# ahuang73/HemoCell

Hardware: AMD Instinct MI355X
Metric: MLUPS + cell-vertex updates/s, 256^3 pipeflow 10% Hct (higher is better)
Workload: dtype f64

## Files before the change

hemocell_amd/capi.py:

```python
import ctypes as C
import os
import subprocess

_HERE = os.path.dirname(os.path.abspath(__file__))
LIB_PATH = os.path.join(_HERE, "lib", "libhemocell_amd.so")

c_double_p = C.POINTER(C.c_double)
c_long_p = C.POINTER(C.c_long)
c_int_p = C.POINTER(C.c_int)


class HcError(RuntimeError):
    pass


class Params(C.Structure):
    _fields_ = [(n, C.c_double) for n in
                ("dx", "dt", "nu_p", "rho_p", "kBT_p", "tau", "nu_lbm", "dm", "df", "f_limit", "kBT_lbm")]


class Material(C.Structure):
    _fields_ = [("kLink", C.c_double), ("kArea", C.c_double), ("kVolume", C.c_double), ("kBend", C.c_double),
                ("eta_m", C.c_double), ("radius", C.c_double), ("min_triangles", C.c_int),
                ("aspect_ratio", C.c_double), ("inner_edges", c_long_p), ("n_inner", C.c_int)]


class WbcMaterial(C.Structure):
    _fields_ = [("kInnerRigid", C.c_double), ("kCytoskeleton", C.c_double), ("coreRadius", C.c_double),
                ("radius", C.c_double)]


class CellTypeSpec(C.Structure):
    _fields_ = [("model", C.c_int), ("shape", C.c_int), ("material", Material), ("wbc", C.POINTER(WbcMaterial)),
                ("kInnerLink", C.c_double), ("stl_path", C.c_char_p)]


VP = C.c_void_p
SIGNATURES = {
    "hc_last_error": (C.c_char_p, []),
    "hc_init": (C.c_int, [C.c_int]),
    "hc_device_count": (C.c_int, [c_int_p]),
    "hc_set_stream": (C.c_int, [VP]),
    "hc_synchronize": (C.c_int, []),
    "hc_fork": (C.c_int, []),
    "hc_route": (C.c_int, [C.c_int]),
    "hc_join": (C.c_int, []),
    "hc_side_stream": (C.c_int, [C.POINTER(VP)]),
    "hc_set_overlap": (C.c_int, [C.c_int]),
    "hc_comm_init_env": (C.c_int, []),
    "hc_comm_init": (C.c_int, [C.c_int, C.c_int, C.c_int, C.c_char_p, C.c_int, C.c_int, C.c_int]),
    "hc_comm_finalize": (C.c_int, []),
    "hc_comm_info": (C.c_int, [c_int_p, c_int_p, c_int_p]),
    "hc_comm_barrier": (C.c_int, []),
    "hc_comm_allreduce": (C.c_int, [c_double_p, C.c_int, C.c_int]),
    "hc_comm_bcast": (C.c_int, [VP, C.c_size_t, C.c_int]),
    "hc_comm_allgather": (C.c_int, [VP, C.c_size_t, VP]),
    "hc_comm_exchange_host": (C.c_int, [C.c_int, VP, C.c_size_t, VP, C.c_size_t, VP, C.c_size_t, VP, C.c_size_t]),
    "hc_slab_stats": (C.c_int, [VP, c_double_p, C.c_int]),
    "hcl_slab_refresh_halos": (C.c_int, [VP, C.c_int]),
    "hcp_slab_sync_placement": (C.c_int, [VP, c_long_p]),
    "hcp_set_envelope": (C.c_int, [VP, C.c_double, c_double_p]),
    "hcp_envelope": (C.c_int, [VP, c_double_p, c_long_p]),
    "hcp_set_deletion_mode": (C.c_int, [VP, C.c_int]),
    "hcp_delete_incomplete_cells": (C.c_int, [VP, c_long_p]),
    "hcp_deletion_counts": (C.c_int, [VP, c_long_p, c_long_p, c_long_p, c_long_p]),
    "hcp_download_alive": (C.c_int, [VP, VP]),
    "hc_profile_enable": (C.c_int, [C.c_int]),
    "hc_profile_read": (C.c_int, [C.c_char_p, c_double_p, c_long_p]),
    "hc_profile_reset": (C.c_int, []),
    "hc_build_tag": (C.c_char_p, []),
    "hc_measure_copy_bandwidth": (C.c_int, [C.c_size_t, C.c_int, c_double_p]),
    "hcl_node_counts": (C.c_int, [VP, c_long_p]),
    "hc_debug_ibm_per_vertex": (C.c_int, [C.c_int]),
    "hc_set_reproducible_spread": (C.c_int, [C.c_int]),
    "hc_debug_force_plane_padding": (C.c_int, [C.c_int]),
    "hcl_create": (C.c_int, [C.POINTER(VP), C.c_int, C.c_int, C.c_int, c_int_p, C.c_double, C.c_int, C.c_int, C.c_int]),
    "hcl_destroy": (C.c_int, [VP]),
    "hcl_set_mask": (C.c_int, [VP, VP]),
    "hcl_init_equilibrium": (C.c_int, [VP, C.c_double, c_double_p]),
    "hcl_set_body_force_regions": (C.c_int, [VP, C.c_int, C.POINTER(C.c_int), c_double_p]),
    "hcl_set_body_force": (C.c_int, [VP, c_double_p]),
    "hcl_set_wall_velocity": (C.c_int, [VP, C.c_int, c_double_p]),
    "hcl_collide_stream": (C.c_int, [VP, C.c_int]),
    "hcl_set_lees_edwards": (C.c_int, [VP, C.c_double, C.c_double]),
    "hcl_set_lees_edwards_displacement": (C.c_int, [VP, C.c_double, C.c_double]),
    "hcl_lees_edwards_apply": (C.c_int, [VP]),
    "hcl_lees_edwards_state": (C.c_int, [VP, c_double_p]),
    "hcl_open_boundary_add": (C.c_int, [VP, C.c_int, C.c_int, c_int_p, C.c_int, c_int_p]),
    "hcl_open_boundary_add_box": (C.c_int, [VP, C.c_int, C.c_int, c_int_p, c_int_p, c_int_p]),
    "hcl_open_boundary_add_axis": (C.c_int, [VP, C.c_int, C.c_int, C.c_int, c_int_p, C.c_int, c_int_p]),
    "hcl_open_boundary_add_box_axis": (C.c_int, [VP, C.c_int, C.c_int, C.c_int, c_int_p, c_int_p, c_int_p]),
    "hcl_open_boundary_axes": (C.c_int, [VP, c_int_p, C.c_int, c_int_p]),
    "hcl_open_boundary_clear": (C.c_int, [VP]),
    "hcl_open_boundary_slots": (C.c_int, [VP, c_int_p, C.c_int, c_int_p]),
    "hcl_open_boundary_set_velocity": (C.c_int, [VP, C.c_int, C.c_int, VP, C.c_int]),
    "hcl_open_boundary_set_density": (C.c_int, [VP, C.c_int, C.c_int, VP, C.c_int]),
    "hcl_open_boundary_values": (C.c_int, [VP, C.c_int, C.c_int, c_double_p]),
    "hcl_plane_velocity": (C.c_int, [VP, C.c_int, c_int_p, C.c_int, VP, C.c_int]),
    "hcl_plane_velocity_axis": (C.c_int, [VP, C.c_int, C.c_int, c_int_p, C.c_int, VP, C.c_int]),
    "hcl_preinlet_create": (C.c_int, [C.POINTER(VP), VP, VP, C.c_int, C.c_int, c_int_p, C.c_int, C.c_int]),
    "hcl_preinlet_apply": (C.c_int, [VP]),
    "hcl_preinlet_iterate": (C.c_int, [VP, C.c_int]),
    "hcl_preinlet_destroy": (C.c_int, [VP]),
    "hcl_collide_stream_part": (C.c_int, [VP, C.c_int]),
    "hcl_step_end": (C.c_int, [VP]),
    "hcl_download_populations": (C.c_int, [VP, c_double_p]),
    "hcl_upload_populations": (C.c_int, [VP, c_double_p]),
    "hcl_download_rho_u": (C.c_int, [VP, c_double_p, c_double_p]),
    "hcl_download_pi_neq": (C.c_int, [VP, c_double_p]),
    "hcl_download_ibm_force": (C.c_int, [VP, c_double_p]),
    "hcl_zero_ibm_force": (C.c_int, [VP]),
    "hcl_halo_doubles": (C.c_size_t, [VP, C.c_int]),
    "hcl_halo_pack": (C.c_int, [VP, C.c_int, C.c_int, VP]),
    "hcl_halo_unpack": (C.c_int, [VP, C.c_int, C.c_int, VP]),
    "hcl_halo_pack_next": (C.c_int, [VP, C.c_int, C.c_int, VP]),
    "hcl_face_velocity_pack": (C.c_int, [VP, C.c_int, VP]),
    "hcl_face_velocity_pack_both": (C.c_int, [VP, VP, VP]),
    "hcl_halo_pack_both": (C.c_int, [VP, VP, VP, C.c_int]),
    "hcl_halo_unpack_both": (C.c_int, [VP, VP, VP]),
    "hcl_zero_force_halos": (C.c_int, [VP]),
    "hcl_download_face_velocity": (C.c_int, [VP, C.c_int, c_double_p]),
    "hcl_dims": (C.c_int, [VP, c_int_p]),
    "hcl_mlups_bytes_per_node": (C.c_double, [VP]),
    "hcl_interior_enable": (C.c_int, [VP, C.c_int, c_double_p]),
    "hcl_interior_info": (C.c_int, [VP, c_int_p, c_double_p]),
    "hcl_interior_upload_classes": (C.c_int, [VP, VP]),
    "hcl_interior_download_classes": (C.c_int, [VP, VP]),
    "hcl_scalar_create": (C.c_int, [VP, C.c_double, C.POINTER(VP)]),
    "hcl_scalar_destroy": (C.c_int, [VP]),
    "hcl_scalar_init_equilibrium": (C.c_int, [VP, c_int_p, C.c_double]),
    "hcl_scalar_set_source_box": (C.c_int, [VP, c_int_p, C.c_double]),
    "hcl_scalar_clear_sources": (C.c_int, [VP]),
    "hcl_scalar_step": (C.c_int, [VP]),
    "hcl_scalar_download": (C.c_int, [VP, c_double_p]),
    "hcl_scalar_download_populations": (C.c_int, [VP, c_double_p]),
    "hcl_scalar_upload_populations": (C.c_int, [VP, c_double_p]),
    "hcl_scalar_download_velocity": (C.c_int, [VP, c_double_p]),
    "hcl_scalar_stats": (C.c_int, [VP, c_double_p]),
    "hcp_sample_scalar": (C.c_int, [VP, VP, c_double_p]),
    "hcp_type_set_interior_viscosity": (C.c_int, [VP, C.c_int, C.c_double]),
    "hcp_set_interior_timescales": (C.c_int, [VP, C.c_int, C.c_int]),
    "hcp_interior_find": (C.c_int, [VP]),
    "hcp_interior_membrane": (C.c_int, [VP]),
    "hcp_interior_normals": (C.c_int, [VP, C.c_int, c_double_p]),
    "hc_debug_interior_block": (C.c_int, [C.c_int]),
    "hcl_binding_populate": (C.c_int, [VP, c_int_p]),
    "hcl_binding_clear": (C.c_int, [VP]),
    "hcl_binding_download": (C.c_int, [VP, VP]),
    "hcl_binding_upload": (C.c_int, [VP, VP]),
    "hcl_download_mask": (C.c_int, [VP, VP]),
    "hcl_download_tresca": (C.c_int, [VP, c_double_p]),
    "hcl_upload_solidified_mask": (C.c_int, [VP, VP]),
    "hcp_type_set_solidify": (C.c_int, [VP, C.c_int, C.c_double, C.c_double]),
    "hcp_set_solidify_timescale": (C.c_int, [VP, C.c_int]),
    "hcp_solidify_prepare": (C.c_int, [VP]),
    "hcp_solidify_flag": (C.c_int, [VP]),
    "hcp_solidify_flags_download": (C.c_int, [VP, VP]),
    "hcp_solidify_flags_upload": (C.c_int, [VP, VP]),
    "hcp_solidify_counts": (C.c_int, [VP, c_long_p]),
    "hc_debug_solidify_block": (C.c_int, [C.c_int]),
    "hc_params_base": (C.c_int, [C.POINTER(Params)] + [C.c_double] * 5),
    "hcp_celltype_create": (C.c_int, [C.POINTER(VP), C.c_int, C.c_int, C.POINTER(Params), C.POINTER(Material)]),
    "hcp_celltype_create_wbc": (C.c_int, [C.POINTER(VP), C.c_int, C.POINTER(Params), C.POINTER(Material),
                                          C.POINTER(WbcMaterial)]),
    "hcp_celltype_wbc_constants": (C.c_int, [VP, c_double_p]),
    "hcp_celltype_create_ex": (C.c_int, [C.POINTER(VP), C.POINTER(Params), C.POINTER(CellTypeSpec)]),
    "hcp_celltype_malaria_constants": (C.c_int, [VP, c_double_p]),
    "hcp_celltype_destroy": (C.c_int, [VP]),
    "hcp_celltype_sizes": (C.c_int, [VP, c_int_p]),
    "hcp_celltype_tables": (C.c_int, [VP, c_double_p, c_long_p, c_long_p, c_double_p, c_double_p, c_double_p,
                                      c_long_p, c_double_p, c_double_p]),
    "hcp_celltype_tables2": (C.c_int, [VP, c_long_p, c_long_p, c_long_p, c_double_p, c_int_p]),
    "hcp_create": (C.c_int, [C.POINTER(VP), VP, C.POINTER(Params)]),
    "hcp_destroy": (C.c_int, [VP]),
    "hcp_add_type": (C.c_int, [VP, VP, C.c_int, c_int_p]),
    "hcp_add_cell": (C.c_int, [VP, C.c_int, C.c_long, c_double_p, c_double_p, C.c_double, c_int_p]),
    "hcp_add_cell_unchecked": (C.c_int, [VP, C.c_int, C.c_long, c_double_p, c_double_p]),
    "hcp_counts": (C.c_int, [VP, c_long_p, c_long_p, c_long_p]),
    "hcp_type_range": (C.c_int, [VP, C.c_int, c_long_p, c_long_p]),
    "hcp_download": (C.c_int, [VP, C.c_int, c_double_p]),
    "hcp_upload": (C.c_int, [VP, C.c_int, c_double_p]),
    "hcp_download_cell_ids": (C.c_int, [VP, c_long_p]),
    "hcp_download_records": (C.c_int, [VP, C.c_void_p, C.c_long]),
    "hcp_upload_records": (C.c_int, [VP, C.c_void_p, C.c_long]),
    "hcp_add_vertex_force": (C.c_int, [VP, c_long_p, C.c_int, c_double_p]),
    "hcp_set_repulsion": (C.c_int, [VP, C.c_double, C.c_double, C.c_int]),
    "hcp_repulsion": (C.c_int, [VP]),
    "hcp_download_repulsion": (C.c_int, [VP, c_double_p]),
    "hcl_fluid_stats": (C.c_int, [VP, C.c_int, c_double_p, C.POINTER(C.c_long)]),
    "hcp_vertex_stats": (C.c_int, [VP, C.c_int, c_double_p, C.POINTER(C.c_long)]),
    "hcp_set_boundary_repulsion": (C.c_int, [VP, C.c_double, C.c_double, C.c_int]),
    "hcp_boundary_repulsion": (C.c_int, [VP]),
    "hcp_spread": (C.c_int, [VP, C.c_int]),
    "hcp_interpolate": (C.c_int, [VP]),
    "hcp_interpolate_cells": (C.c_int, [VP, C.c_int, c_int_p, C.c_int]),
    "hcp_advance": (C.c_int, [VP, C.c_int]),
    "hcp_mechanics": (C.c_int, [VP, C.c_long, C.c_int]),
    "hcp_mechanics_components": (C.c_int, [VP, C.c_int, c_double_p]),
    "hc_iterate": (C.c_int, [VP, VP, c_long_p, C.c_int, C.c_int, C.c_int, C.c_int]),
    "hcp_cell_extents": (C.c_int, [VP, C.c_int, c_double_p]),
    "hcp_cell_extents_begin": (C.c_int, [VP, C.c_int]),
    "hcp_cell_extents_end": (C.c_int, [VP, C.c_int, c_double_p]),
    "hcp_record_doubles": (C.c_size_t, [VP, C.c_int]),
    "hcp_pack_cells": (C.c_int, [VP, C.c_int, c_int_p, C.c_int, C.c_double, VP]),
    "hcp_unpack_cells": (C.c_int, [VP, C.c_int, c_int_p, c_long_p, c_int_p, C.c_int, VP]),
    "hcp_remove_cells": (C.c_int, [VP, C.c_int, c_int_p, C.c_int]),
    "hcp_owned_vertices": (C.c_int, [VP, c_long_p]),
    "hcp_preinlet_create": (C.c_int, [C.POINTER(VP), VP, VP, C.c_int, C.c_int, C.c_double, C.c_double, c_double_p, C.c_long]),
    "hcp_preinlet_create_slab": (C.c_int, [C.POINTER(VP), VP, VP, C.c_int, C.c_int, C.c_double, C.c_double, c_double_p, C.c_long]),
    "hcp_preinlet_set_sink": (C.c_int, [VP, C.c_int, C.c_double]),
    "hcp_preinlet_apply": (C.c_int, [VP, c_long_p, c_long_p]),
    "hcp_preinlet_counts": (C.c_int, [VP, c_long_p]),
    "hcp_preinlet_destroy": (C.c_int, [VP]),
    "hc_preinlet_iterate": (C.c_int, [VP, VP, c_long_p, C.c_int, C.c_int, C.c_int, C.c_int, C.c_int]),
    "hcp_cell_info": (C.c_int, [VP, C.c_int, c_double_p, c_double_p, c_double_p, c_double_p]),
}

_lib = None


def build():
    subprocess.check_call(["make", "-s", "-C", os.path.join(_HERE, "csrc")])


def lib():
    global _lib
    if _lib is None:
        if not os.path.exists(LIB_PATH):
            raise HcError("libhemocell_amd.so is not built (run `python -c 'import __graft_entry__ as g; g.build()'`); "
                          "the product path has no CPU fallback")
        L = C.CDLL(LIB_PATH)
        for name, (res, args) in SIGNATURES.items():
            fn = getattr(L, name)
            fn.restype = res
            fn.argtypes = args
        _lib = L
    return _lib


def check(rc):
    if rc != 0:
        raise HcError(lib().hc_last_error().decode("utf-8", "replace"))


def dptr(a):
    return a.ctypes.data_as(c_double_p)


def lptr(a):
    return a.ctypes.data_as(c_long_p)
```

hemocell_amd/csrc/cells.h:

```cpp
#pragma once
#include "common.h"
#include "host_cells.h"
#include "mesh.h"
#include <algorithm>
#include <cmath>
#include <cstring>

using namespace hc;

struct hc_celltype {
  CellTables host;
  DevBuf<int> d_tri, d_edge, d_ebt, d_ebo, d_iedge, d_vtri, d_vtri_k, d_vedge, d_vedge_s, d_bsrc, d_vouter, d_vinner, d_vinner_s, d_ring, d_nring;
  DevBuf<double> d_tri_area_eq, d_edge_len_eq, d_edge_angle_eq, d_patch_eq, d_iedge_len_eq;
};

struct hc_cells {
  hc_lattice *L = nullptr;
  hc_params P;
  int ntypes = 0;
  hc_celltype *types[8];
  int timescale[8];
  HostCells host[8];
  bool host_dirty = false;
  long nverts = 0, cap = 0;
  long ncells[8] = {0};
  long capc[8] = {0};
  long first[8] = {0};
  long cell0[8] = {0};
  DevBuf<double> pos[3], vel[3], frc[3];
  DevBuf<int> d_tag;
  long tag_cap = 0;
  DevBuf<unsigned char> d_vdead;
  MappedBuf<int> h_ntag;
  DevBuf<int> d_ntag;
  Event ntag_ev;
  bool ntag_pending = false, maybe_tagged = false;
  int del_mode = HC_DELETE_PARTICLE;
  DevBuf<int> d_vert_cell;
  DevBuf<double> rep[3];
  int rep_enabled = 0, rep_timescale = 1; double rep_const = 0, rep_cutoff = 0;
  int brep_enabled = 0, brep_timescale = 1; double brep_const = 0, brep_cutoff = 0; DevBuf<uint8_t> d_bflag;
  bool rep_on() const { return rep_enabled || brep_enabled; }
  DevBuf<unsigned int> d_keys[2]; DevBuf<int> d_vals[2]; DevBuf<char> d_sort_tmp; long sort_cap = 0;
  Staged<int> iscratch[19];
  MappedBuf<double> h_ext[8]; long ext_n[8] = {0}; Event ext_done[8]; bool ext_pending[8] = {false};
  Staged<char> vf;
  DevBuf<unsigned int> det_keys[2]; DevBuf<int> det_vals[2]; DevBuf<double> det_val[3]; DevBuf<char> det_tmp; long det_cap = 0;
  Staged<double> stat;
  Staged<double> info;
  std::vector<long> slab_gone[8];
  double e_share = 4.0;
  MappedBuf<int> h_env_viol;
  std::vector<long> slab_rejected;
  int visc_class[8] = {0};
  int visc_every = 1, visc_grid_every = 1;
  Staged<int> visc_rank; std::vector<long> visc_ids_seen;
  bool visc_on() const { for (int t = 0; t < ntypes; t++) if (visc_class[t]) return true; return false; }
  int solid_on[8] = {0}; double solid_dist[8] = {0}, solid_shear[8] = {0};
  int solid_every = 1;
  DevBuf<unsigned char> d_sflag;
  DevBuf<int> d_solid; MappedBuf<int> h_solid;
  long solid_nodes_seen = 0;
  bool solidify_on() const { for (int t = 0; t < ntypes; t++) if (solid_on[t]) return true; return false; }
  long n_deleted = 0;
  long n_particles_deleted = 0;
};

namespace hcc {

constexpr double E_SHARE_DEFAULT = 4.0, E_SHARE_MIN = 2.0;

struct LatView {
  const uint8_t *mask;
  int nx, ny, nz; long plane; long npad;
  int x0;
  int wrap_x, halo_x;
  int per_y, per_z;
  int nx_global;
  uint8_t *dirty; uint8_t epoch;
  const uint8_t *wallbrick; int nby, nbz;
  const double *halo_u[2];
  int ny_nz;
};

inline LatView make_view(const hc_lattice *L) {
  LatView v;
  v.mask = L->mask; v.nx = L->nx; v.ny = L->ny; v.nz = L->nz; v.plane = (long)L->xs; v.npad = (long)L->npad;
  v.x0 = L->x0; v.wrap_x = (L->n_slabs == 1 && L->periodic[0]) ? 1 : 0; v.halo_x = L->n_slabs > 1 ? 1 : 0;
  v.per_y = L->periodic[1]; v.per_z = L->periodic[2]; v.nx_global = L->nx_global;
  v.dirty = L->fdirty[L->fcur]; v.epoch = L->fepoch[L->fcur];
  v.wallbrick = L->wallbrick; v.nby = L->nby; v.nbz = L->nbz;
  v.halo_u[0] = L->halo_u_valid ? L->halo_u[0] : nullptr; v.halo_u[1] = L->halo_u_valid ? L->halo_u[1] : nullptr; v.ny_nz = (int)L->plane;
  return v;
}

__device__ __forceinline__ long pmod(long a, long n) { long r = a % n; return r < 0 ? r + n : r; }

__device__ __forceinline__ double phi2(double x) { x = fabs(x); x = 1.0 - x; return x > 0.0 ? x : 0.0; }

struct Stencil {
  long node[8];
  double w[8];
  int lx[8], ly[8], lz[8];
};

__device__ __forceinline__ long nearest_node(double x) { return (long)floor(x + 0.5); }

__device__ __forceinline__ void phi2_stencil(const LatView &v, double px, double py, double pz, Stencil &s) {
  const double p[3] = {px, py, pz};
  long c[3]; int d0[3];
#pragma unroll
  for (int a = 0; a < 3; a++) { c[a] = nearest_node(p[a]); d0[a] = (p[a] < (double)c[a]) ? -1 : 0; }
  double total = 0.0;
#pragma unroll
  for (int i = 0; i < 2; i++)
#pragma unroll
    for (int j = 0; j < 2; j++)
#pragma unroll
      for (int k = 0; k < 2; k++) {
        const int idx = i * 4 + j * 2 + k;
        const long gx = c[0] + d0[0] + i, gy = c[1] + d0[1] + j, gz = c[2] + d0[2] + k;
        long lx = gx - v.x0, ly = gy, lz = gz;
        bool ok = true;
        if (v.wrap_x) lx = pmod(lx, v.nx);
        else if (v.halo_x) ok = ok && (lx >= -HALO && lx < v.nx + HALO);
        else ok = ok && (lx >= 0 && lx < v.nx);
        if (gy < 0 || gy >= v.ny) { if (v.per_y) ly = pmod(gy, v.ny); else ok = false; }
        if (gz < 0 || gz >= v.nz) { if (v.per_z) lz = pmod(gz, v.nz); else ok = false; }
        double weight = 0.0; long node = -1;
        if (ok) {
          weight = phi2(p[0] - (double)gx) * phi2(p[1] - (double)gy) * phi2(p[2] - (double)gz);
          if (weight != 0.0) {
            node = (lx + HALO) * (long)v.plane + ly * v.nz + lz;
            if (v.mask[node] != 0) node = -1;
          }
        }
        if (node >= 0) total += weight;
        s.node[idx] = node; s.w[idx] = weight; s.lx[idx] = (int)lx; s.ly[idx] = (int)ly; s.lz[idx] = (int)lz;
      }
  const double coeff = 1.0 / total;
#pragma unroll
  for (int idx = 0; idx < 8; idx++) s.w[idx] *= coeff;
}

struct VertArrays { double *p[3], *v[3], *f[3], *r[3]; unsigned char *dead; int *tag; };
struct TypeArrays : VertArrays { const int *vert_cell; int *tag_all; };

template <typename T>
inline int upload_vec(DevBuf<T> &dst, const std::vector<T> &src) {
  const int rc = dst.reserve(src.size() ? src.size() : 1); if (rc != HC_OK) return rc;
  if (src.size()) HC_HIP(hipMemcpy(dst, src.data(), src.size() * sizeof(T), hipMemcpyHostToDevice));
  return HC_OK;
}
template <size_t N>
inline std::vector<int> flatten(const std::vector<std::array<long, N>> &v) {
  std::vector<int> o; o.reserve(v.size() * N);
  for (auto &a : v) for (long x : a) o.push_back((int)x);
  return o;
}

int sync_to_device(hc_cells *C);
int sync_to_host(hc_cells *C);
int settle(hc_cells *C);
TypeArrays vert_arrays(hc_cells *C, int t);
int ensure_sflag(hc_cells *C);
int solidify_refresh_mask(hc_cells *C);
int solidify_check(hc_cells *C);
const char *solidify_refusal(const hc_lattice *L);
int ensure_rep(hc_cells *C);
int stage_ints(hc_cells *C, int which, int **d, const int *h, int n);
int stage_ints(Staged<int> &s, int **d, const int *h, int n);
int upload_xyz(DevBuf<double> dst[3], long first, const double *src, long n);
int download_xyz(double *dst, const DevBuf<double> src[3], long first, long n);
int append_cells(hc_cells *C, int type, const long *cell_ids, const int *is_new, int n, long n_new);
int interpolate_cells_staged(hc_cells *C, int type, const int *slots, int n, int which);

}
using namespace hcc;
```

hemocell_amd/csrc/cells.hip:

```cpp
#include "cells.h"
#include <cstddef>
#include <memory>
#include <unordered_map>
#include <utility>
#include <vector>

namespace {

__global__ __launch_bounds__(256) void advance_kernel(LatView v, long n, double *px, double *py, double *pz, const double *vx,
                                                      const double *vy, const double *vz, const int *vert_cell, int *tag, unsigned char *dead,
                                                      int *counters, int whole_cell) {
  const long i = (long)blockIdx.x * 256 + threadIdx.x;
  if (i >= n) return;
  const int cell = vert_cell[i];
  if (dead[i] || tag[cell] == 1) return;
  const double x = px[i] + vx[i], y = py[i] + vy[i], z = pz[i] + vz[i];
  px[i] = x; py[i] = y; pz[i] = z;
  long gx = nearest_node(x) - v.x0, gy = nearest_node(y), gz = nearest_node(z);
  bool inside = true;
  if (v.wrap_x) gx = pmod(gx, v.nx); else inside = inside && (gx >= (v.halo_x ? -HALO : 0) && gx < (v.halo_x ? v.nx + HALO : v.nx));
  if (gy < 0 || gy >= v.ny) { if (v.per_y) gy = pmod(gy, v.ny); else inside = false; }
  if (gz < 0 || gz >= v.nz) { if (v.per_z) gz = pmod(gz, v.nz); else inside = false; }
  if (inside && v.mask[(gx + HALO) * (long)v.plane + gy * v.nz + gz] != 0) {
    if (whole_cell) {
      if (atomicExch(&tag[cell], 1) != 1) atomicAdd(&counters[0], 1);
    } else {
      dead[i] = 1;
      atomicAdd(&counters[2], 1);
      if (atomicCAS(&tag[cell], 0, 2) == 0) atomicAdd(&counters[1], 1);
    }
  }
}

__global__ void publish_counters_kernel(const int *counters, int *host_view) { for (int k = 0; k < 4; k++) host_view[k] = counters[k]; }
__global__ void sub_counters_kernel(int *counters, int a, int b, int c, int d) { atomicSub(&counters[0], a); atomicSub(&counters[1], b); atomicSub(&counters[2], c); if (d) atomicSub(&counters[3], d); }

__global__ void delete_incomplete_kernel(long ncells, int *tag, int *counters) {
  const long c = (long)blockIdx.x * 256 + threadIdx.x;
  if (c >= ncells) return;
  if (tag[c] == 2) { tag[c] = 1; atomicAdd(&counters[0], 1); }
}

__global__ void add_vertex_force_kernel(int n, const long *idx, const double *f, double *fx, double *fy, double *fz) {
  const int i = blockIdx.x * 256 + threadIdx.x;
  if (i >= n) return;
  const long v = idx[i];
  fx[v] += f[3 * i]; fy[v] += f[3 * i + 1]; fz[v] += f[3 * i + 2];
}

__global__ void fill_vert_cell_kernel(long n, int nv, int cell0, long first, int *vert_cell) {
  const long i = (long)blockIdx.x * 256 + threadIdx.x;
  if (i >= n) return;
  vert_cell[first + i] = cell0 + (int)(i / nv);
}

}

namespace hcc {

static void drop_regions(hc_cells *C) {
  for (int d = 0; d < 3; d++) { C->pos[d].reset(); C->vel[d].reset(); C->frc[d].reset(); C->rep[d].reset(); }
  C->d_tag.reset(); C->d_vdead.reset(); C->d_vert_cell.reset(); C->d_sflag.reset();
  C->cap = 0; C->tag_cap = 0;
  for (int t = 0; t < 8; t++) C->capc[t] = 0;
}

int ensure_rep(hc_cells *C) {
  if (C->rep[0] || C->cap <= 0) return HC_OK;
  for (int d = 0; d < 3; d++) {
    const int rc = C->rep[d].reserve((size_t)C->cap); if (rc != HC_OK) return rc;
    HC_HIP(hipMemset(C->rep[d], 0, C->cap * sizeof(double)));
  }
  return HC_OK;
}

int upload_xyz(DevBuf<double> dst[3], long first, const double *src, long n) {
  std::vector<double> tmp((size_t)n);
  for (int d = 0; d < 3; d++) {
    for (long i = 0; i < n; i++) tmp[(size_t)i] = src[(size_t)(3 * i + d)];
    HC_HIP(hipMemcpy(dst[d] + first, tmp.data(), (size_t)n * sizeof(double), hipMemcpyHostToDevice));
  }
  return HC_OK;
}
int download_xyz(double *dst, const DevBuf<double> src[3], long first, long n) {
  std::vector<double> tmp((size_t)n);
  for (int d = 0; d < 3; d++) {
    HC_HIP(hipMemcpy(tmp.data(), src[d] + first, (size_t)n * sizeof(double), hipMemcpyDeviceToHost));
    for (long i = 0; i < n; i++) dst[(size_t)(3 * i + d)] = tmp[(size_t)i];
  }
  return HC_OK;
}

int sync_to_device(hc_cells *C) {
  if (!C->host_dirty) return HC_OK;
  bool grow = false;
  long nverts = 0;
  int rc;
  for (int t = 0; t < C->ntypes; t++) {
    C->ncells[t] = (long)C->host[t].cells();
    nverts += C->ncells[t] * C->types[t]->host.nv;
    if (C->ncells[t] > C->capc[t]) grow = true;
  }
  if (grow || C->cap == 0) {
    drop_regions(C);
    long cap = 0, capcells = 0;
    for (int t = 0; t < C->ntypes; t++) {
      C->capc[t] = C->ncells[t] + C->ncells[t] / 4 + 64;
      C->first[t] = cap; C->cell0[t] = capcells;
      cap += C->capc[t] * C->types[t]->host.nv; capcells += C->capc[t];
    }
    C->cap = cap > 0 ? cap : 1;
    for (int d = 0; d < 3; d++)
      if ((rc = C->pos[d].reserve((size_t)C->cap)) != HC_OK || (rc = C->vel[d].reserve((size_t)C->cap)) != HC_OK || (rc = C->frc[d].reserve((size_t)C->cap)) != HC_OK) return rc;
    if ((rc = C->d_vert_cell.reserve((size_t)C->cap)) != HC_OK) return rc;
    if (C->rep_on() && (rc = ensure_rep(C)) != HC_OK) return rc;
    C->tag_cap = capcells + 1;
    if ((rc = C->d_tag.reserve((size_t)C->tag_cap)) != HC_OK || (rc = C->d_vdead.reserve((size_t)C->cap)) != HC_OK) return rc;
    for (int t = 0; t < C->ntypes; t++) {
      const long n = C->capc[t] * C->types[t]->host.nv;
      hipLaunchKernelGGL(fill_vert_cell_kernel, dim3((unsigned)((n + 255) / 256)), dim3(256), 0, hc::stream(), n, C->types[t]->host.nv, (int)C->cell0[t], C->first[t], C->d_vert_cell);
      HC_HIP(hipGetLastError());
    }
  }
  if (C->solidify_on() && (rc = ensure_sflag(C)) != HC_OK) return rc;
  C->nverts = nverts;
  for (int t = 0; t < C->ntypes; t++) {
    const long n = C->ncells[t] * C->types[t]->host.nv;
    if (n == 0) continue;
    const HostCells &H = C->host[t];
    if ((rc = upload_xyz(C->pos, C->first[t], H.pos.data(), n)) != HC_OK || (rc = upload_xyz(C->vel, C->first[t], H.vel.data(), n)) != HC_OK ||
        (rc = upload_xyz(C->frc, C->first[t], H.frc.data(), n)) != HC_OK) return rc;
  }
  HC_HIP(hipMemsetAsync(C->d_tag, 0, C->tag_cap * sizeof(int), hc::stream()));
  HC_HIP(hipMemsetAsync(C->d_vdead, 0, (size_t)C->cap, hc::stream()));
  if (C->d_sflag) HC_HIP(hipMemsetAsync(C->d_sflag, 0, (size_t)C->cap, hc::stream()));
  HC_HIP(hipStreamSynchronize(hc::stream()));
  for (int t = 0; t < C->ntypes; t++) {
    const long nc = C->ncells[t], n = nc * C->types[t]->host.nv;
    if (nc == 0) continue;
    const HostCells &H = C->host[t];
    HC_HIP(hipMemcpy(C->d_tag + C->cell0[t], H.tag.data(), (size_t)nc * sizeof(int), hipMemcpyHostToDevice));
    HC_HIP(hipMemcpy(C->d_vdead + C->first[t], H.dead.data(), (size_t)n, hipMemcpyHostToDevice));
    if (C->d_sflag) HC_HIP(hipMemcpy(C->d_sflag + C->first[t], H.sflag.data(), (size_t)n, hipMemcpyHostToDevice));
    if (H.has_rep && C->rep[0] && (rc = upload_xyz(C->rep, C->first[t], H.rep.data(), n)) != HC_OK) return rc;
  }
  C->host_dirty = false;
  return HC_OK;
}

int sync_to_host(hc_cells *C) {
  if (C->host_dirty) return HC_OK;
  HC_HIP(hipStreamSynchronize(hc::stream()));
  int rc;
  for (int t = 0; t < C->ntypes; t++) {
    const long n = C->ncells[t] * C->types[t]->host.nv;
    HostCells &H = C->host[t];
    H.size_payload(C->rep[0] != nullptr);
    if (n == 0) continue;
    if ((rc = download_xyz(H.pos.data(), C->pos, C->first[t], n)) != HC_OK || (rc = download_xyz(H.vel.data(), C->vel, C->first[t], n)) != HC_OK ||
        (rc = download_xyz(H.frc.data(), C->frc, C->first[t], n)) != HC_OK) return rc;
    if (C->d_tag) {
      HC_HIP(hipMemcpy(H.tag.data(), C->d_tag + C->cell0[t], (size_t)C->ncells[t] * sizeof(int), hipMemcpyDeviceToHost));
      HC_HIP(hipMemcpy(H.dead.data(), C->d_vdead + C->first[t], (size_t)n, hipMemcpyDeviceToHost));
    }
    if (C->d_sflag) HC_HIP(hipMemcpy(H.sflag.data(), C->d_sflag + C->first[t], (size_t)n, hipMemcpyDeviceToHost));
    if (H.has_rep && (rc = download_xyz(H.rep.data(), C->rep, C->first[t], n)) != HC_OK) return rc;
  }
  return HC_OK;
}

TypeArrays vert_arrays(hc_cells *C, int t) {
  TypeArrays a;
  for (int d = 0; d < 3; d++) {
    a.p[d] = C->pos[d] + C->first[t]; a.v[d] = C->vel[d] + C->first[t]; a.f[d] = C->frc[d] + C->first[t];
    a.r[d] = C->rep[d] ? C->rep[d] + C->first[t] : nullptr;
  }
  a.dead = C->d_vdead + C->first[t]; a.tag = C->d_tag + C->cell0[t];
  a.vert_cell = C->d_vert_cell + C->first[t]; a.tag_all = C->d_tag;
  return a;
}
int stage_ints(hc_cells *C, int which, int **d, const int *h, int n) { return stage_ints(C->iscratch[which], d, h, n); }
int stage_ints(Staged<int> &s, int **d, const int *h, int n) {
  if (!s.ev) { const int rc = s.ev.create(); if (rc != HC_OK) return rc; }
  else HC_HIP(hipEventSynchronize(s.ev));
  if ((size_t)n > s.cap()) {
    HC_HIP(hipDeviceSynchronize());
    const int rc = s.reserve((size_t)n * 2 + 256); if (rc != HC_OK) return rc;
  }
  if (n > 0) {
    std::memcpy(s.h, h, (size_t)n * sizeof(int));
    HC_HIP(hipMemcpyAsync(s.d, s.h, (size_t)n * sizeof(int), hipMemcpyHostToDevice, hc::stream()));
    HC_HIP(hipEventRecord(s.ev, hc::stream()));
  }
  *d = s.d;
  return HC_OK;
}

int celltype_create(const char *fn, hc_celltype **out, const hc_params *P, const hc_celltype_spec &S) {
  if (hc::stream() == nullptr) { hc::set_error(std::string(fn) + ": hc_init() has not been called"); return HC_ERR_STATE; }
  std::unique_ptr<hc_celltype> T(new hc_celltype());
  std::string err = build_cell_tables(T->host, *P, S);
  if (!err.empty()) { hc::set_error(std::string(fn) + ": " + err); return HC_ERR_ARG; }
  const CellTables &H = T->host;
  int rc = HC_OK;
  auto up_i = [&](DevBuf<int> &d, const std::vector<int> &v) { if (rc == HC_OK) rc = upload_vec(d, v); };
  auto up_d = [&](DevBuf<double> &d, const std::vector<double> &v) { if (rc == HC_OK) rc = upload_vec(d, v); };
  up_i(T->d_tri, flatten(H.triangles)); up_i(T->d_edge, flatten(H.edges));
  up_i(T->d_ebt, flatten(H.edge_bending_triangles)); up_i(T->d_ebo, flatten(H.edge_bending_outer));
  up_i(T->d_iedge, flatten(H.inner_edges));
  up_i(T->d_vtri, H.vtri); up_i(T->d_vtri_k, H.vtri_k); up_i(T->d_vedge, H.vedge); up_i(T->d_vedge_s, H.vedge_s);
  up_i(T->d_bsrc, H.bsrc); up_i(T->d_vouter, H.vouter); up_i(T->d_vinner, H.vinner); up_i(T->d_vinner_s, H.vinner_s);
  up_i(T->d_ring, flatten(H.vertex_vertexes)); up_i(T->d_nring, H.vertex_n_vertexes);
  up_d(T->d_tri_area_eq, H.triangle_area_eq); up_d(T->d_edge_len_eq, H.edge_length_eq);
  up_d(T->d_edge_angle_eq, H.edge_angle_eq); up_d(T->d_patch_eq, H.patch_dist_eq); up_d(T->d_iedge_len_eq, H.inner_edge_length_eq);
  if (rc != HC_OK) return rc;
  *out = T.release();
  return HC_OK;
}

}

extern "C" {

int hcp_celltype_create(hc_celltype **out, int model, int shape, const hc_params *P, const hc_material *M) {
  HC_REQUIRE(out && P && M, "hcp_celltype_create: null pointer");
  HC_REQUIRE(model != HC_MODEL_WBC_HO, "hcp_celltype_create: HC_MODEL_WBC_HO needs its inner-link constants: use hcp_celltype_create_wbc or hcp_celltype_create_ex");
  HC_REQUIRE(model != HC_MODEL_RBC_MALARIA, "hcp_celltype_create: HC_MODEL_RBC_MALARIA needs kInnerLink: use hcp_celltype_create_ex");
  HC_REQUIRE(shape != HC_SHAPE_MESH_FROM_STL, "hcp_celltype_create: HC_SHAPE_MESH_FROM_STL needs the STL file: use hcp_celltype_create_ex");
  hc_celltype_spec S{};
  S.model = model; S.shape = shape; S.material = *M;
  return hcc::celltype_create("hcp_celltype_create", out, P, S);
}

int hcp_celltype_create_wbc(hc_celltype **out, int shape, const hc_params *P, const hc_material *M, const hc_wbc_material *W) {
  HC_REQUIRE(out && P && M && W, "hcp_celltype_create_wbc: null pointer");
  HC_REQUIRE(shape != HC_SHAPE_MESH_FROM_STL, "hcp_celltype_create_wbc: HC_SHAPE_MESH_FROM_STL needs the STL file: use hcp_celltype_create_ex");
  hc_celltype_spec S{};
  S.model = HC_MODEL_WBC_HO; S.shape = shape; S.material = *M; S.wbc = W;
  return hcc::celltype_create("hcp_celltype_create_wbc", out, P, S);
}

int hcp_celltype_create_ex(hc_celltype **out, const hc_params *P, const hc_celltype_spec *S) {
  HC_REQUIRE(out && P && S, "hcp_celltype_create_ex: null pointer");
  return hcc::celltype_create("hcp_celltype_create_ex", out, P, *S);
}

int hcp_celltype_malaria_constants(const hc_celltype *T, double out[1]) {
  HC_REQUIRE(T && out, "hcp_celltype_malaria_constants: null pointer");
  out[0] = T->host.k_inner_link;
  return HC_OK;
}

int hcp_celltype_wbc_constants(const hc_celltype *T, double out[4]) {
  HC_REQUIRE(T && out, "hcp_celltype_wbc_constants: null pointer");
  const CellTables &H = T->host;
  out[0] = H.k_inner_rigid; out[1] = H.k_cytoskeleton; out[2] = H.core_radius; out[3] = H.wbc_radius;
  return HC_OK;
}

int hcp_celltype_destroy(hc_celltype *T) {
  delete T;
  return HC_OK;
}

int hcp_celltype_sizes(const hc_celltype *T, int out[4]) {
  HC_REQUIRE(T && out, "hcp_celltype_sizes: null pointer");
  out[0] = T->host.nv; out[1] = T->host.nt; out[2] = T->host.ne; out[3] = T->host.nie;
  return HC_OK;
}

int hcp_celltype_tables(const hc_celltype *T, double *vertices, long *triangles, long *edges, double *edge_length_eq,
                        double *edge_angle_eq, double *triangle_area_eq, long *vertex_vertexes, double *patch_dist_eq,
                        double scalars[9]) {
  HC_REQUIRE(T, "hcp_celltype_tables: null cell type");
  const CellTables &H = T->host;
  if (vertices) for (int i = 0; i < H.nv; i++) for (int d = 0; d < 3; d++) vertices[3 * i + d] = H.vertices[i][d];
  if (triangles) for (int i = 0; i < H.nt; i++) for (int d = 0; d < 3; d++) triangles[3 * i + d] = H.triangles[i][d];
  if (edges) for (int i = 0; i < H.ne; i++) for (int d = 0; d < 2; d++) edges[2 * i + d] = H.edges[i][d];
  if (edge_length_eq) std::copy(H.edge_length_eq.begin(), H.edge_length_eq.end(), edge_length_eq);
  if (edge_angle_eq) std::copy(H.edge_angle_eq.begin(), H.edge_angle_eq.end(), edge_angle_eq);
  if (triangle_area_eq) std::copy(H.triangle_area_eq.begin(), H.triangle_area_eq.end(), triangle_area_eq);
  if (vertex_vertexes) for (int i = 0; i < H.nv; i++) for (int d = 0; d < 6; d++) vertex_vertexes[6 * i + d] = H.vertex_vertexes[i][d];
  if (patch_dist_eq) std::copy(H.patch_dist_eq.begin(), H.patch_dist_eq.end(), patch_dist_eq);
  if (scalars) {
    const double s[9] = {H.volume_eq, H.area_mean_eq, H.edge_mean_eq, H.angle_mean_eq, H.k_volume, H.k_area, H.k_link, H.k_bend, H.eta_m};
    std::copy(s, s + 9, scalars);
  }
  return HC_OK;
}

int hcp_celltype_tables2(const hc_celltype *T, long *edge_bending_triangles, long *edge_bending_outer_points, long *inner_edges,
                         double *inner_edge_length_eq, int *vertex_n_vertexes) {
  HC_REQUIRE(T, "hcp_celltype_tables2: null cell type");
  const CellTables &H = T->host;
  if (edge_bending_triangles) for (int i = 0; i < H.ne; i++) for (int d = 0; d < 2; d++) edge_bending_triangles[2 * i + d] = H.edge_bending_triangles[i][d];
  if (edge_bending_outer_points) for (int i = 0; i < H.ne; i++) for (int d = 0; d < 2; d++) edge_bending_outer_points[2 * i + d] = H.edge_bending_outer[i][d];
  if (inner_edges) for (int i = 0; i < H.nie; i++) for (int d = 0; d < 2; d++) inner_edges[2 * i + d] = H.inner_edges[i][d];
  if (inner_edge_length_eq) std::copy(H.inner_edge_length_eq.begin(), H.inner_edge_length_eq.end(), inner_edge_length_eq);
  if (vertex_n_vertexes) std::copy(H.vertex_n_vertexes.begin(), H.vertex_n_vertexes.end(), vertex_n_vertexes);
  return HC_OK;
}

int hcp_create(hc_cells **out, hc_lattice *L, const hc_params *P) {
  HC_REQUIRE(out && L && P, "hcp_create: null pointer");
  std::unique_ptr<hc_cells> C(new hc_cells());
  C->L = L; C->P = *P;
  L->ibm = 1;
  int rc;
  if ((rc = C->h_ntag.reserve(4)) != HC_OK) return rc;
  for (int k = 0; k < 4; k++) C->h_ntag[k] = 0;
  if ((rc = C->d_ntag.reserve(4)) != HC_OK) return rc;
  HC_HIP(hipMemset(C->d_ntag, 0, 4 * sizeof(int)));
  if ((rc = C->ntag_ev.create()) != HC_OK || (rc = C->h_env_viol.reserve(1)) != HC_OK) return rc;
  *C->h_env_viol = 0;
  *out = C.release();
  return HC_OK;
}

int hcp_set_envelope(hc_cells *C, double particle_envelope_lu, double *share_in_use) {
  HC_REQUIRE(C, "hcp_set_envelope: null pointer");
  HC_REQUIRE(particle_envelope_lu > 0.0 && particle_envelope_lu < 1e6, "hcp_set_envelope: the envelope must be a positive number of lattice units");
  HC_REQUIRE(C->ntypes > 0, "hcp_set_envelope: add the cell types first (the envelope is measured against the largest cell)");
  for (int t = 0; t < C->ntypes; t++) HC_REQUIRE(C->host[t].cells() == 0, "hcp_set_envelope: set the envelope before the first cell is placed (placement already uses it)");
  double dmax = 0.0;
  for (int t = 0; t < C->ntypes; t++) dmax = std::max(dmax, C->types[t]->host.diameter);
  double share = std::max(particle_envelope_lu - dmax, E_SHARE_MIN);
  const hc_lattice *L = C->L;
  if (L->n_slabs > 1) {
    const double room = 0.5 * ((double)L->nx - 2.0 * dmax);
    if (room < E_SHARE_MIN) { hc::set_error("hcp_set_envelope: a slab of " + std::to_string(L->nx) + " planes cannot hold two cell diameters (" + std::to_string(2.0 * dmax) + " lu) and a particle envelope"); return HC_ERR_ARG; }
    share = std::min(share, std::floor(room * 16.0) / 16.0);
  }
  C->e_share = share;
  if (share_in_use) *share_in_use = share;
  return HC_OK;
}

int hcp_envelope(const hc_cells *C, double *share_in_use, long *late_copies) {
  HC_REQUIRE(C, "hcp_envelope: null pointer");
  if (share_in_use) *share_in_use = C->e_share;
  if (late_copies) *late_copies = C->h_env_viol ? (long)*C->h_env_viol : 0;
  return HC_OK;
}

int hcp_destroy(hc_cells *C) {
  if (!C) return HC_OK;
  (void)hipStreamSynchronize(hc::stream());
  delete C;
  return HC_OK;
}

int hcp_add_type(hc_cells *C, hc_celltype *T, int material_timescale, int *type_index) {
  HC_REQUIRE(C && T, "hcp_add_type: null pointer");
  HC_REQUIRE(C->ntypes < 8, "hcp_add_type: at most 8 cell types");
  HC_REQUIRE(material_timescale >= 1, "hcp_add_type: material timescale must be >= 1");
  C->types[C->ntypes] = T; C->timescale[C->ntypes] = material_timescale; C->host[C->ntypes].nv = T->host.nv;
  if (type_index) *type_index = C->ntypes;
  C->ntypes++;
  return HC_OK;
}

int hcp_add_cell(hc_cells *C, int type, long cell_id, const double centre_lu[3], const double angles[3], double min_dist_um, int *placed) {
  HC_REQUIRE(C && centre_lu && angles, "hcp_add_cell: null pointer");
  HC_REQUIRE(type >= 0 && type < C->ntypes, "hcp_add_cell: unknown cell type");
  int rc = settle(C); if (rc != HC_OK) return rc;
  rc = sync_to_host(C); if (rc != HC_OK) return rc;
  const CellTables &T = C->types[type]->host;
  const hc_lattice *L = C->L;
  const int nv = T.nv;
  auto bbox_centre = [&](const std::vector<Vec3> &v) {
    Vec3 lo = v[0], hi = v[0];
    for (auto &p : v) for (int d = 0; d < 3; d++) { lo[d] = std::min(lo[d], p[d]); hi[d] = std::max(hi[d], p[d]); }
    return Vec3{(hi[0] + lo[0]) * 0.5, (hi[1] + lo[1]) * 0.5, (hi[2] + lo[2]) * 0.5};
  };
  std::vector<Vec3> m = T.vertices;
  const Vec3 c0 = bbox_centre(m);
  for (auto &p : m) for (int d = 0; d < 3; d++) p[d] -= c0[d];
  const Vec3 mc = bbox_centre(m);
  double R[3][3];
  rotation_matrix_xyz(angles[0], angles[1], angles[2], R);
  for (auto &p : m) {
    const Vec3 x{p[0] + -1.0 * mc[0], p[1] + -1.0 * mc[1], p[2] + -1.0 * mc[2]};
    for (int a = 0; a < 3; a++) { double s = 0; for (int b = 0; b < 3; b++) s += R[a][b] * x[b]; p[a] = s + mc[a]; }
  }
  const std::vector<uint8_t> &mask = L->hmask;
  auto is_boundary = [&](long gx, long gy, long gz) -> bool {
    long lx = gx - L->x0, ly = gy, lz = gz;
    if (L->n_slabs == 1) { if (lx < 0 || lx >= L->nx) { if (L->periodic[0]) lx = ((lx % L->nx) + L->nx) % L->nx; else return false; } }
    else if (lx < -HALO || lx >= L->nx + HALO) return false;
    if (ly < 0 || ly >= L->ny) { if (L->periodic[1]) ly = ((ly % L->ny) + L->ny) % L->ny; else return false; }
    if (lz < 0 || lz >= L->nz) { if (L->periodic[2]) lz = ((lz % L->nz) + L->nz) % L->nz; else return false; }
    return mask[(size_t)(lx + HALO) * L->xs + (size_t)ly * L->nz + lz] != 0;
  };
  double cx = centre_lu[0];
  if (L->n_slabs > 1) {
    const double x0 = (double)L->x0, x1 = (double)(L->x0 + L->nx);
    const double shifts[3] = {0.0, -(double)L->nx_global, (double)L->nx_global};
    bool mine = false;
    for (int k = 0; k < (L->periodic[0] ? 3 : 1) && !mine; k++) {
      double lo = 1e300, hi = -1e300; bool own = false;
      for (int i = 0; i < nv; i++) {
        const double x = centre_lu[0] + shifts[k] + m[i][0];
        lo = std::min(lo, x); hi = std::max(hi, x);
        const double g = std::floor(x + 0.5);
        own = own || (g >= x0 && g < x1);
      }
      if (own || (hi >= x0 - C->e_share && lo < x1 + C->e_share)) { mine = true; cx = centre_lu[0] + shifts[k]; }
    }
    if (!mine) { if (placed) *placed = 0; return HC_OK; }
  }
  const int deny = (int)((min_dist_um * 1e-6) / C->P.dx);
  bool ok = true;
  for (int i = 0; i < nv && ok; i++) {
    const double v[3] = {cx + m[i][0], centre_lu[1] + m[i][1], centre_lu[2] + m[i][2]};
    const long n[3] = {(long)std::floor(v[0] + 0.5), (long)std::floor(v[1] + 0.5), (long)std::floor(v[2] + 0.5)};
    if (is_boundary(n[0], n[1], n[2])) { ok = false; break; }
    for (int a = -deny; a <= deny && ok; a++) for (int b = -deny; b <= deny && ok; b++) for (int c = -deny; c <= deny; c++)
      if (is_boundary(n[0] + a, n[1] + b, n[2] + c)) { ok = false; break; }
  }
  if (placed) *placed = ok ? 1 : 0;
  if (!ok) {
    if (L->n_slabs > 1) { C->slab_rejected.push_back(type); C->slab_rejected.push_back(cell_id); }
    return HC_OK;
  }
  double *p = C->host[type].append(cell_id, C->rep_on());
  for (int i = 0; i < nv; i++) { p[3 * i] = cx + m[i][0]; p[3 * i + 1] = centre_lu[1] + m[i][1]; p[3 * i + 2] = centre_lu[2] + m[i][2]; }
  C->host_dirty = true;
  return HC_OK;
}

int hcp_add_cell_unchecked(hc_cells *C, int type, long cell_id, const double centre_lu[3], const double angles[3]) {
  HC_REQUIRE(C && centre_lu && angles, "hcp_add_cell_unchecked: null pointer");
  HC_REQUIRE(type >= 0 && type < C->ntypes, "hcp_add_cell_unchecked: unknown cell type");
  int rc = settle(C); if (rc != HC_OK) return rc;
  rc = sync_to_host(C); if (rc != HC_OK) return rc;
  const CellTables &T = C->types[type]->host;
  (void)angles;
// ... 375 lines not shown
```

hemocell_amd/csrc/common.h:

```cpp
#pragma once
#include <hip/hip_runtime.h>
#include <stdint.h>
#include <string>
#include <utility>
#include <vector>
#include <type_traits>
#include "../../include/hemocell_amd.h"
#include "d3q19.h"

namespace hc {

void set_error(const std::string &msg);
int hip_fail(hipError_t e, const char *what, const char *file, int line);
hipStream_t stream();
hipStream_t comm_stream();
int fork();
void route(int side);
int join();
bool forked();

#define HC_HIP(call)                                                         \
  do {                                                                       \
    hipError_t e__ = (call);                                                 \
    if (e__ != hipSuccess) return hc::hip_fail(e__, #call, __FILE__, __LINE__); \
  } while (0)

#define HC_REQUIRE(cond, msg)                 \
  do {                                        \
    if (!(cond)) {                            \
      hc::set_error(std::string(msg));        \
      return HC_ERR_ARG;                      \
    }                                         \
  } while (0)

template <class T> struct DevBuf {
  T *p = nullptr; size_t cap = 0;
  DevBuf() = default;
  DevBuf(DevBuf &&o) noexcept { swap(o); }
  DevBuf &operator=(DevBuf &&o) noexcept { swap(o); return *this; }
  ~DevBuf() { reset(); }
  void swap(DevBuf &o) { std::swap(p, o.p); std::swap(cap, o.cap); }
  void reset() { if (p) (void)hipFree(p); p = nullptr; cap = 0; }
  operator T *() const { return p; }
  int reserve(size_t n) {
    if (n <= cap) return HC_OK;
    reset();
    const hipError_t e = hipMalloc((void **)&p, n * sizeof(T));
    if (e != hipSuccess) { p = nullptr; return hip_fail(e, "hipMalloc", __FILE__, __LINE__); }
    cap = n;
    return HC_OK;
  }
};
template <class T> struct PinBuf {
  T *p = nullptr, *dev = nullptr; size_t cap = 0; unsigned flags;
  explicit PinBuf(unsigned f = hipHostMallocDefault) : flags(f) {}
  PinBuf(PinBuf &&o) noexcept : flags(o.flags) { swap(o); }
  PinBuf &operator=(PinBuf &&o) noexcept { swap(o); return *this; }
  ~PinBuf() { reset(); }
  void swap(PinBuf &o) { std::swap(p, o.p); std::swap(dev, o.dev); std::swap(cap, o.cap); std::swap(flags, o.flags); }
  void reset() { if (p) (void)hipHostFree(p); p = dev = nullptr; cap = 0; }
  operator T *() const { return p; }
  int reserve(size_t n) {
    if (n <= cap) return HC_OK;
    reset();
    hipError_t e = hipHostMalloc((void **)&p, n * sizeof(T), flags);
    if (e != hipSuccess) p = nullptr;
    else if (flags & hipHostMallocMapped) e = hipHostGetDevicePointer((void **)&dev, p, 0);
    if (e != hipSuccess) { reset(); return hip_fail(e, "hipHostMalloc", __FILE__, __LINE__); }
    cap = n;
    return HC_OK;
  }
};
template <class T> struct MappedBuf : PinBuf<T> { MappedBuf() : PinBuf<T>(hipHostMallocMapped) {} };
struct Event {
  hipEvent_t e = nullptr;
  Event() = default;
  Event(Event &&o) noexcept { std::swap(e, o.e); }
  Event &operator=(Event &&o) noexcept { std::swap(e, o.e); return *this; }
  ~Event() { if (e) (void)hipEventDestroy(e); }
  operator hipEvent_t() const { return e; }
  int create() {
    if (e) return HC_OK;
    const hipError_t r = hipEventCreateWithFlags(&e, hipEventDisableTiming);
    if (r != hipSuccess) { e = nullptr; return hip_fail(r, "hipEventCreateWithFlags", __FILE__, __LINE__); }
    return HC_OK;
  }
};
template <class T> struct Staged {
  DevBuf<T> d; PinBuf<T> h; Event ev;
  size_t cap() const { return d.cap < h.cap ? d.cap : h.cap; }
  int reserve(size_t n) { const int rc = d.reserve(n); return rc != HC_OK ? rc : h.reserve(n); }
};

enum ProfKernel { PK_COLLIDE = 0, PK_SPREAD, PK_INTERP, PK_ADVANCE, PK_MECH, PK_COLLIDE_BESIDE, PK_LEES_EDWARDS, PK_COLLIDE_VISC, PK_INTERIOR_FIND, PK_INTERIOR_MEMBRANE, PK_SCALAR, PK_SOLIDIFY_PREPARE, PK_SOLIDIFY_FLAG, PK_COUNT };
void prof_count(int kernel);
struct ProfScope {
  int k; bool on;
  hipEvent_t a, b;
  explicit ProfScope(int kernel);
  ~ProfScope();
};

constexpr int HALO = 2;

constexpr int STAT_BLOCKS = 512;
struct StatAcc { double mn, mx, sum; long n; };
__device__ __forceinline__ void stat_add(StatAcc &a, double v) { a.mn = v < a.mn ? v : a.mn; a.mx = v > a.mx ? v : a.mx; a.sum += v; a.n++; }
__device__ __forceinline__ void stat_block_store(StatAcc a, double *partial ) {
  __shared__ double s_red[4][4];
#pragma unroll
  for (int off = 32; off > 0; off >>= 1) {
    const double mn = __shfl_xor(a.mn, off), mx = __shfl_xor(a.mx, off), sm = __shfl_xor(a.sum, off);
    const long n = __shfl_xor(a.n, off);
    a.mn = mn < a.mn ? mn : a.mn; a.mx = mx > a.mx ? mx : a.mx; a.sum += sm; a.n += n;
  }
  const int w = threadIdx.x >> 6;
  if ((threadIdx.x & 63) == 0) { s_red[w][0] = a.mn; s_red[w][1] = a.mx; s_red[w][2] = a.sum; s_red[w][3] = (double)a.n; }
  __syncthreads();
  if (threadIdx.x == 0) {
    double mn = s_red[0][0], mx = s_red[0][1], sm = s_red[0][2], n = s_red[0][3];
    for (int k = 1; k < (int)(blockDim.x >> 6); k++) { mn = s_red[k][0] < mn ? s_red[k][0] : mn; mx = s_red[k][1] > mx ? s_red[k][1] : mx; sm += s_red[k][2]; n += s_red[k][3]; }
    double *o = partial + 4 * blockIdx.x;
    o[0] = mn; o[1] = mx; o[2] = sm; o[3] = n;
  }
}
int stat_finish(const double *d_partial, double out[3], long *n, double *h_pinned = nullptr);

}

namespace hc {
struct BodyRegions { int n; int box[HC_MAX_FORCE_REGIONS][6]; double f[HC_MAX_FORCE_REGIONS][3]; };
#ifdef __HIPCC__
__device__ __forceinline__ void region_force(const BodyRegions &r, int xg, int y, int z, double &bx, double &by, double &bz) {
  for (int k = 0; k < r.n; k++) {
    const int *b = r.box[k];
    if (xg >= b[0] && xg <= b[1] && y >= b[2] && y <= b[3] && z >= b[4] && z <= b[5]) { bx = r.f[k][0]; by = r.f[k][1]; bz = r.f[k][2]; }
  }
}

constexpr int HC_OB_AXIS_SHIFT = 29;
constexpr int HC_OB_MAX_SLOTS = 1 << 27;
constexpr int ob_axis(int code) { return code >> HC_OB_AXIS_SHIFT; }
constexpr int ob_slot(int code) { return (code & ((1 << HC_OB_AXIS_SHIFT) - 1)) >> 2; }
constexpr bool ob_is_pressure(int code) { return (code & 2) != 0; }
__host__ __device__ constexpr int zh_perm(int axis, int i) {
  const int x = axis == 1 ? HC_CY[i] : axis == 2 ? HC_CZ[i] : HC_CX[i];
  const int y = axis == 1 ? HC_CX[i] : HC_CY[i];
  const int z = axis == 2 ? HC_CX[i] : HC_CZ[i];
  for (int j = 0; j < HC_Q; j++) if (HC_CX[j] == x && HC_CY[j] == y && HC_CZ[j] == z) return j;
  return -1;
}
template <int AXIS, int I> inline constexpr int ZH = zh_perm(AXIS, I);
static_assert(ZH<0, 7> == 7 && ZH<1, 1> == 2 && ZH<1, 5> == 14 && ZH<1, 15> == 17 && ZH<2, 1> == 3 && ZH<2, 7> == 16 && ZH<2, 13> == 17, "zh_perm");

template <int AXIS>
__device__ __forceinline__ void zou_he(double f[HC_Q], int code, const double *__restrict__ val) {
#define G(I) f[ZH<AXIS, I>]
  const int kind = code & 3;
  const long slot = code >> 2;
  const double s0 = G(0) + G(2) + G(3) + G(8) + G(9) + G(11) + G(12) + G(17) + G(18);
  const double sm = G(1) + G(4) + G(5) + G(6) + G(7);
  const double sp = G(10) + G(13) + G(14) + G(15) + G(16);
  const bool neg = (kind & 1) == 0;
  const double s_out = neg ? sm : sp;
  const double known = s0 + 2.0 * s_out + 1.0;
  double rho, ux, uy, uz;
  if (kind < 2) {
    ux = val[4 * slot + AXIS]; uy = val[4 * slot + (AXIS == 1 ? 0 : 1)]; uz = val[4 * slot + (AXIS == 2 ? 0 : 2)];
    rho = neg ? known / (1.0 - ux) : known / (1.0 + ux);
  } else {
    rho = val[4 * slot + 3];
    ux = neg ? 1.0 - known / rho : known / rho - 1.0;
    uy = 0.0; uz = 0.0;
  }
  const double ny = 0.5 * ((G(11) + G(17) + G(18)) - (G(2) + G(8) + G(9))) - rho * uy / 3.0;
  const double nz = 0.5 * ((G(12) + G(9) + G(17)) - (G(3) + G(8) + G(18))) - rho * uz / 3.0;
  if (neg) {
    G(10) = G(1) + rho * ux / 3.0;
    G(13) = G(4) + rho * (ux + uy) / 6.0 - ny;
    G(14) = G(5) + rho * (ux - uy) / 6.0 + ny;
    G(15) = G(6) + rho * (ux + uz) / 6.0 - nz;
    G(16) = G(7) + rho * (ux - uz) / 6.0 + nz;
  } else {
    G(1) = G(10) - rho * ux / 3.0;
    G(4) = G(13) - rho * (ux + uy) / 6.0 + ny;
    G(5) = G(14) - rho * (ux - uy) / 6.0 - ny;
    G(6) = G(15) - rho * (ux + uz) / 6.0 + nz;
    G(7) = G(16) - rho * (ux - uz) / 6.0 - nz;
  }
#undef G
}

__device__ __forceinline__ void zou_he_node(double f[HC_Q], int code, const double *__restrict__ val) {
  switch (code >> HC_OB_AXIS_SHIFT) {
    case 0: zou_he<0>(f, code, val); break;
    case 1: zou_he<1>(f, code & ((1 << HC_OB_AXIS_SHIFT) - 1), val); break;
    default: zou_he<2>(f, code & ((1 << HC_OB_AXIS_SHIFT) - 1), val); break;
  }
}
#endif
}

struct hc_lattice {
  int nx, ny, nz;
  int periodic[3];
  int x0, nx_global, n_slabs;
  double omega;
  size_t plane;
  size_t xs;
  size_t npad;
  size_t qstride;
  hc::DevBuf<double> f[2];
  int cur;
  hc::DevBuf<double> force[3];
  int fcur;
  int ibm;
  hc::DevBuf<uint8_t> fdirty[3];
  uint8_t fepoch[3];
  hc::DevBuf<uint8_t> wallbrick; int nbx, nby, nbz;
  hc::DevBuf<uint8_t> mask;
  std::vector<uint8_t> hmask;
  double body[3];
  hc::BodyRegions regions;
  double wall_u[4][3];
  hc::DevBuf<int> row_z0, row_cum, blk_row;
  int nblk, max_active;
  hc::DevBuf<double> scratch;
  hc::DevBuf<double> halo_u[2];
  bool halo_u_valid = false;
  bool le_on = false;
  double le_D = 0.0, le_d = 0.0, le_v_top = 0.0, le_v_bottom = 0.0;
  hc::DevBuf<double> le_buf;
  hc::DevBuf<int> ob_code;
  std::vector<int> ob_hcode;
  hc::DevBuf<double> ob_val;
  int ob_n = 0, ob_cap = 0;
  long ob_epoch = 0;
  hc::DevBuf<uint8_t> visc_class;
  int visc_n = 0; double visc_omega[HC_MAX_VISC_CLASSES];
  hc::DevBuf<unsigned long long> visc_vote;
  hc_scalar *scalar = nullptr;
  hc::DevBuf<uint8_t> binding;
  hc::DevBuf<int> ob_list;
  hc::DevBuf<double> ob_out;
};

namespace hc {
template <class Plain, class Launch>
inline void launch_open(const hc_lattice *L, const Plain &plain, Launch launch) {
  if (L->ob_n > 0) launch(std::true_type{}, open_of(L, plain));
  else launch(std::false_type{}, plain);
}
}

namespace hc {
int lees_edwards_step(hc_lattice *L);
void scalar_lattice_destroyed(hc_lattice *L);
void preinlet_pair_add(const void *owner, const hc_lattice *L);
void preinlet_pair_remove(const void *owner);
void preinlet_pair_forget(const hc_lattice *L);
bool in_preinlet_pair(const hc_lattice *L);
}

namespace hcs {
int iterate_slab(hc_lattice *L, hc_cells *C, long *iter, int n, int particle_timescale, int force_limit);
int collide_stream_slab(hc_lattice *L, int nsteps);
void lattice_destroyed(hc_lattice *L);
void halos_stale(hc_lattice *L);
void set_overlap(int on);
}
```

hemocell_amd/csrc/ibm.hip:

```cpp
#include "cells.h"
#include <type_traits>
#include <hipcub/hipcub.hpp>
#include <cstdlib>
#include <cstring>
#include <numeric>

namespace {

__global__ __launch_bounds__(256) void ibm_spread_kernel(LatView v, long n, const double *px, const double *py, const double *pz,
                                                         double *fx, double *fy, double *fz, const double *rx, const double *ry, const double *rz,
                                                         double *F, int limit_on, double f_limit, const int *vert_cell, const int *tag, const unsigned char *dead) {
  const long i = (long)blockIdx.x * 256 + threadIdx.x;
  if (i >= n) return;
  if (dead[i] || tag[vert_cell[i]] == 1) return;
  double f0 = fx[i], f1 = fy[i], f2 = fz[i];
  if (limit_on) {
    const double mag = sqrt((f0 * f0 + f1 * f1) + f2 * f2);
    if (mag > f_limit) {
      const double sc = f_limit / mag;
      f0 *= sc; f1 *= sc; f2 *= sc;
      fx[i] = f0; fy[i] = f1; fz[i] = f2;
    }
  }
  Stencil s;
  phi2_stencil(v, px[i], py[i], pz[i], s);
#pragma unroll
  for (int k = 0; k < 8; k++) {
    if (s.node[k] < 0) continue;
    v.dirty[s.node[k] >> 4] = v.epoch;
    double *Fn = F + 3 * s.node[k];
    unsafeAtomicAdd(Fn, ((rx ? rx[i] : 0.0) + f0) * s.w[k]);
    unsafeAtomicAdd(Fn + 1, ((ry ? ry[i] : 0.0) + f1) * s.w[k]);
    unsafeAtomicAdd(Fn + 2, ((rz ? rz[i] : 0.0) + f2) * s.w[k]);
  }
}

__global__ __launch_bounds__(256) void spread_emit_kernel(LatView v, int nv, long n, const int *order, long ebase, const double *px, const double *py,
                                                          const double *pz, double *fx, double *fy, double *fz, const double *rx, const double *ry,
                                                          const double *rz, int limit_on, double f_limit, const int *tag, const unsigned char *dead,
                                                          unsigned int *keys, int *vals, double *c0, double *c1, double *c2) {
  const long g = (long)blockIdx.x * 256 + threadIdx.x;
  if (g >= n) return;
  const int cell = order[g / nv];
  const long i = (long)cell * nv + (g % nv);
  const long e0 = (ebase + g) * 8;
  const bool live = tag[cell] != 1 && !dead[i];
  Stencil s;
  double f0 = 0.0, f1 = 0.0, f2 = 0.0;
  if (live) {
    f0 = fx[i]; f1 = fy[i]; f2 = fz[i];
    if (limit_on) {
      const double mag = sqrt((f0 * f0 + f1 * f1) + f2 * f2);
      if (mag > f_limit) { const double sc = f_limit / mag; f0 *= sc; f1 *= sc; f2 *= sc; fx[i] = f0; fy[i] = f1; fz[i] = f2; }
    }
    if (rx) { f0 = rx[i] + f0; f1 = ry[i] + f1; f2 = rz[i] + f2; }
    phi2_stencil(v, px[i], py[i], pz[i], s);
  }
#pragma unroll
  for (int k = 0; k < 8; k++) {
    const bool adm = live && s.node[k] >= 0;
    keys[e0 + k] = adm ? (unsigned int)s.node[k] : 0xffffffffu;
    vals[e0 + k] = (int)(e0 + k);
    c0[e0 + k] = adm ? f0 * s.w[k] : 0.0; c1[e0 + k] = adm ? f1 * s.w[k] : 0.0; c2[e0 + k] = adm ? f2 * s.w[k] : 0.0;
  }
}

__global__ __launch_bounds__(256) void spread_gather_kernel(LatView v, long n, const unsigned int *keys, const int *vals, const double *c0, const double *c1,
                                                            const double *c2, double *F) {
  const long s = (long)blockIdx.x * 256 + threadIdx.x;
  if (s >= n) return;
  const unsigned int key = keys[s];
  if (key == 0xffffffffu || (s > 0 && keys[s - 1] == key)) return;
  double a0 = 0.0, a1 = 0.0, a2 = 0.0;
  for (long q = s; q < n && keys[q] == key; q++) { const int e = vals[q]; a0 += c0[e]; a1 += c1[e]; a2 += c2[e]; }
  v.dirty[key >> 4] = v.epoch;
  double *Fn = F + 3 * (long)key;
  Fn[0] += a0; Fn[1] += a1; Fn[2] += a2;
}

struct PopView {
  const double *f; const double *F; double bx, by, bz; long qs;
  hc::BodyRegions reg;
};
struct OpenPopView : PopView { const int *ob_code; const double *ob_val; };
template <bool OPEN> using Pops = std::conditional_t<OPEN, OpenPopView, PopView>;

template <bool OPEN = false>
__device__ __forceinline__ void node_velocity(const LatView &v, const Pops<OPEN> &pv, int lx, int ly, int lz, long node, double u[3]) {
  if (v.halo_x && (lx <= -HALO || lx >= v.nx + HALO - 1)) { u[0] = u[1] = u[2] = 0.0; return; }
  if (v.halo_x && (lx == -1 || lx == v.nx)) {
    const double *hu = v.halo_u[lx < 0 ? 0 : 1];
    if (hu) { const long k = (long)ly * v.nz + lz; u[0] = hu[k]; u[1] = hu[v.ny_nz + k]; u[2] = hu[2L * v.ny_nz + k]; return; }
  }
  const hc::Nbr nb = hc::neighbours(v, v.plane, lx, ly, lz);
  double r = 0.0, jx = 0.0, jy = 0.0, jz = 0.0;
  [[maybe_unused]] double f[OPEN ? HC_Q : 1];
#define M(Q, CX, CY, CZ)                                                              \
  {                                                                                   \
    bool ok; const long off = hc::src_off<CX, CY, CZ>(nb, ok);                        \
    const double fq = ok ? pv.f[(long)Q * pv.qs + node + off] : 0.0;                 \
    if constexpr (OPEN) f[Q] = fq;                                                    \
    else {                                                                            \
      r += fq;                                                                        \
      if (CX == 1) jx += fq; else if (CX == -1) jx += -fq;                            \
      if (CY == 1) jy += fq; else if (CY == -1) jy += -fq;                            \
      if (CZ == 1) jz += fq; else if (CZ == -1) jz += -fq;                            \
    }                                                                                 \
  }
  FOR_Q(M)
#undef M
  if constexpr (OPEN) {
    if (v.mask[node] == 0) {
      const int code = pv.ob_code[node];
      if (code >= 0) hc::zou_he_node(f, code, pv.ob_val);
    }
    hc::moments(f, r, jx, jy, jz);
  }
  const double invRho = 1.0 / (1.0 + r);
  double bx = pv.bx, by = pv.by, bz = pv.bz;
  if (pv.reg.n) {
    int xg = v.x0 + lx;
    if (xg < 0) xg += v.nx_global; else if (xg >= v.nx_global) xg -= v.nx_global;
    region_force(pv.reg, xg, ly, lz, bx, by, bz);
  }
  u[0] = jx * invRho + (bx + pv.F[3 * node]) / 2.0;
  u[1] = jy * invRho + (by + pv.F[3 * node + 1]) / 2.0;
  u[2] = jz * invRho + (bz + pv.F[3 * node + 2]) / 2.0;
}

template <bool OPEN = false>
__global__ __launch_bounds__(256) void face_velocity_kernel(LatView v, Pops<OPEN> pv, int lx0, double *out0, int lx1, double *out1) {
  const int k = blockIdx.x * 256 + threadIdx.x;
  if (k >= v.ny_nz) return;
  const int lx = blockIdx.y ? lx1 : lx0;
  double *out = blockIdx.y ? out1 : out0;
  const int ly = k / v.nz, lz = k - ly * v.nz;
  const long node = (long)(lx + HALO) * v.plane + (long)ly * v.nz + lz;
  double u[3] = {0.0, 0.0, 0.0};
  if (v.mask[node] == 0) node_velocity<OPEN>(v, pv, lx, ly, lz, node, u);
  out[k] = u[0]; out[v.ny_nz + k] = u[1]; out[2L * v.ny_nz + k] = u[2];
}

template <bool OPEN = false>
__global__ __launch_bounds__(256) void ibm_interpolate_kernel(LatView v, Pops<OPEN> pv, long n, const double *px, const double *py,
                                                              const double *pz, double *vx, double *vy, double *vz, const int *vert_cell, const int *tag,
                                                              const unsigned char *dead) {
  const long i = (long)blockIdx.x * 256 + threadIdx.x;
  if (i >= n) return;
  if (dead[i] || tag[vert_cell[i]] == 1) return;
  Stencil s;
  phi2_stencil(v, px[i], py[i], pz[i], s);
  double a0 = 0.0, a1 = 0.0, a2 = 0.0;
#pragma unroll
  for (int k = 0; k < 8; k++) {
    if (s.node[k] < 0) continue;
    double u[3];
    node_velocity<OPEN>(v, pv, s.lx[k], s.ly[k], s.lz[k], s.node[k], u);
    a0 += (u[0] * s.w[k]); a1 += (u[1] * s.w[k]); a2 += (u[2] * s.w[k]);
  }
  vx[i] = a0; vy[i] = a1; vz[i] = a2;
}


constexpr int TILE_CAP = 5832;
constexpr int NODE_CAP = 1536;

struct Tile { int o[3]; int e[3]; int vol; int ow[3]; float r1, r2; };

__device__ __forceinline__ void tile_decode(const Tile &t, int i, int &tx, int &ty, int &tz) {
  const int q = (int)(((float)i + 0.5f) * t.r2);
  tz = i - q * t.e[2];
  tx = (int)(((float)q + 0.5f) * t.r1);
  ty = q - tx * t.e[1];
}

__device__ __forceinline__ int stencil_base(const LatView &v, double px, double py, double pz, int b[3]) {
  const double p[3] = {px, py, pz};
#pragma unroll
  for (int a = 0; a < 3; a++) { const long c = nearest_node(p[a]); b[a] = (int)c + ((p[a] < (double)c) ? -1 : 0); }
  return 0;
}

__device__ __forceinline__ long tile_node(const LatView &v, const Tile &t, int i, int &lx, int &ly, int &lz) {
  int tx, ty, tz;
  tile_decode(t, i, tx, ty, tz);
  lx = t.ow[0] + tx; ly = t.ow[1] + ty; lz = t.ow[2] + tz;
  if (v.wrap_x && lx >= v.nx) lx -= v.nx;
  if (v.per_y && ly >= v.ny) ly -= v.ny;
  if (v.per_z && lz >= v.nz) lz -= v.nz;
  return (long)(lx + HALO) * v.plane + ly * v.nz + lz;
}

__device__ __forceinline__ int xcd_contiguous(int b, int n) {
  const int per = n >> 3;
  const int main_n = per << 3;
  if (b >= main_n) return b;
  return (b & 7) * per + (b >> 3);
}

struct VStencil { double w[8]; int base; unsigned adm; };

constexpr int NVPT = 3;
constexpr int MAXW = 4;

#ifdef HC_IBM_PHASE_TIMES
__device__ unsigned long long g_phase[32];
#define PH_PARAM , long long &ph_last
#define PH_ARG , ph_last
#define PH_INIT long long ph_last = clock64();
#define STAMP(k) do { if (threadIdx.x == 0) { const long long ph_now = clock64(); atomicAdd(&g_phase[k], (unsigned long long)(ph_now - ph_last)); ph_last = ph_now; } } while (0)
#else
#define PH_PARAM
#define PH_ARG
#define PH_INIT
#define STAMP(k) do {} while (0)
#endif

__device__ __forceinline__ void block_bbox(int lo[3], int hi[3], int *s_red, Tile &t) {
  const int tid = threadIdx.x;
#pragma unroll
  for (int a = 0; a < 3; a++)
#pragma unroll
    for (int off = 32; off > 0; off >>= 1) { lo[a] = min(lo[a], __shfl_xor(lo[a], off)); hi[a] = max(hi[a], __shfl_xor(hi[a], off)); }
  if ((tid & 63) == 0) {
#pragma unroll
    for (int a = 0; a < 3; a++) { s_red[(tid >> 6) * 6 + a] = lo[a]; s_red[(tid >> 6) * 6 + 3 + a] = hi[a]; }
  }
  __syncthreads();
  const int nw = (blockDim.x + 63) >> 6;
#pragma unroll
  for (int a = 0; a < 3; a++) {
    int l = s_red[a], h = s_red[3 + a];
    for (int w = 1; w < nw; w++) { l = min(l, s_red[w * 6 + a]); h = max(h, s_red[w * 6 + 3 + a]); }
    t.o[a] = l; t.e[a] = h >= l ? h - l + 1 : 0;
  }
  const long vol = (long)t.e[0] * t.e[1] * t.e[2];
  t.vol = vol > 0x7fffffff ? 0x7fffffff : (int)vol;
}

__device__ __forceinline__ bool tile_finish(const LatView &v, Tile &t) {
  if (t.vol > TILE_CAP) return false;
  if ((v.wrap_x && t.e[0] > v.nx) || (v.per_y && t.e[1] > v.ny) || (v.per_z && t.e[2] > v.nz)) return false;
  t.ow[0] = v.wrap_x ? (int)pmod((long)t.o[0] - v.x0, v.nx) : t.o[0] - v.x0;
  t.ow[1] = v.per_y ? (int)pmod(t.o[1], v.ny) : t.o[1];
  t.ow[2] = v.per_z ? (int)pmod(t.o[2], v.nz) : t.o[2];
  t.r1 = 1.0f / (float)t.e[1]; t.r2 = 1.0f / (float)t.e[2];
  return true;
}

__device__ __forceinline__ unsigned char tile_mask(const LatView &v, const Tile &t, int i) {
  int tx, ty, tz;
  tile_decode(t, i, tx, ty, tz);
  int lx = t.ow[0] + tx, ly = t.ow[1] + ty, lz = t.ow[2] + tz;
  if (v.wrap_x) { if (lx >= v.nx) lx -= v.nx; }
  else if (v.halo_x) { if (lx < -HALO || lx >= v.nx + HALO) return 3; }
  else if (lx < 0 || lx >= v.nx) return 3;
  if (v.per_y) { if (ly >= v.ny) ly -= v.ny; } else if (ly < 0 || ly >= v.ny) return 3;
  if (v.per_z) { if (lz >= v.nz) lz -= v.nz; } else if (lz < 0 || lz >= v.nz) return 3;
  return v.mask[(long)(lx + HALO) * v.plane + ly * v.nz + lz];
}

__device__ __forceinline__ void tile_stencil(const Tile &t, const unsigned char *mt, double px, double py, double pz, const int b[3], VStencil &o) {
  const int sy = t.e[2], sx = t.e[1] * t.e[2];
  o.base = ((b[0] - t.o[0]) * t.e[1] + (b[1] - t.o[1])) * t.e[2] + (b[2] - t.o[2]);
  o.adm = 0;
  double total = 0.0;
#pragma unroll
  for (int i = 0; i < 2; i++)
#pragma unroll
    for (int j = 0; j < 2; j++)
#pragma unroll
      for (int k = 0; k < 2; k++) {
        const int idx = i * 4 + j * 2 + k;
        const double weight = phi2(px - (double)(b[0] + i)) * phi2(py - (double)(b[1] + j)) * phi2(pz - (double)(b[2] + k));
        const bool adm = (weight != 0.0) && (!mt || mt[o.base + i * sx + j * sy + k] == 0);
        if (adm) { total += weight; o.adm |= 1u << idx; }
        o.w[idx] = adm ? weight : 0.0;
      }
  const double coeff = 1.0 / total;
#pragma unroll
  for (int idx = 0; idx < 8; idx++) o.w[idx] *= coeff;
}

__device__ __forceinline__ bool tile_is_clear(const LatView &v, const Tile &t, int *s_near) {
  const int n[3] = {v.nx, v.ny, v.nz};
  bool inside = v.wallbrick != nullptr;
  int b0[3], nb[3];
#pragma unroll
  for (int a = 0; a < 3; a++) {
    const int lo = a == 0 ? t.ow[0] + HALO : t.ow[a], hi = lo + t.e[a] - 1, lim = a == 0 ? v.nx + 2 * HALO : n[a];
    inside = inside && lo >= 0 && hi < lim && (a != 0 || !v.wrap_x || (t.ow[0] >= 0 && t.ow[0] + t.e[0] <= v.nx));
    b0[a] = lo >> 3; nb[a] = (hi >> 3) - b0[a] + 1;
  }
  if (!inside) return false;
  if (nb[0] * nb[1] * nb[2] > 64) return false;
  if (threadIdx.x < 64) {
    const int l = threadIdx.x;
    bool near = false;
    if (l < nb[0] * nb[1] * nb[2]) {
      const int bz = l % nb[2], by = (l / nb[2]) % nb[1], bx = l / (nb[2] * nb[1]);
      near = v.wallbrick[((long)(b0[0] + bx) * v.nby + (b0[1] + by)) * v.nbz + (b0[2] + bz)] != 0;
    }
    const unsigned long long any = __ballot(near);
    if (l == 0) *s_near = any != 0ull;
  }
  __syncthreads();
  return *s_near == 0;
}

__device__ __forceinline__ bool cell_prologue(const LatView &v, int nv, long base, const double *px, const double *py, const double *pz,
                                              const unsigned char *dead, int *s_red, int *s_near, unsigned char *mt, Tile &t, VStencil vs[NVPT] PH_PARAM) {
  const int tid = threadIdx.x, nth = blockDim.x;
  double p[NVPT][3]; int b[NVPT][3]; bool live[NVPT];
  int lo[3] = {0x7fffffff, 0x7fffffff, 0x7fffffff}, hi[3] = {-0x7fffffff, -0x7fffffff, -0x7fffffff};
#pragma unroll
  for (int j = 0; j < NVPT; j++) {
    const int i = tid + j * nth;
    live[j] = i < nv && !(dead && dead[base + i]);
    if (live[j]) {
      p[j][0] = px[base + i]; p[j][1] = py[base + i]; p[j][2] = pz[base + i];
      stencil_base(v, p[j][0], p[j][1], p[j][2], b[j]);
#pragma unroll
      for (int a = 0; a < 3; a++) { lo[a] = min(lo[a], b[j][a]); hi[a] = max(hi[a], b[j][a] + 1); }
    }
  }
  block_bbox(lo, hi, s_red, t);
  STAMP(1);
  if (!tile_finish(v, t) || nv > NVPT * nth) return false;
  const bool clear = tile_is_clear(v, t, s_near);
  STAMP(2);
  if (!clear) {
#pragma unroll 4
    for (int i = tid; i < t.vol; i += nth) mt[i] = tile_mask(v, t, i);
    __syncthreads();
  }
  STAMP(3);
#pragma unroll
  for (int j = 0; j < NVPT; j++) {
    vs[j].adm = 0; vs[j].base = 0;
    if (live[j]) tile_stencil(t, clear ? nullptr : mt, p[j][0], p[j][1], p[j][2], b[j], vs[j]);
  }
  STAMP(4);
  return true;
}

constexpr unsigned short SLOT_FREE = 0xFFFF, SLOT_MARK = 0xFFFE;
__device__ __forceinline__ int compact_nodes(const Tile &t, const VStencil vs[NVPT], unsigned short *slot, unsigned short *list, int *s_count) {
  const int tid = threadIdx.x, nth = blockDim.x;
  const int sy = t.e[2], sx = t.e[1] * t.e[2];
  for (int i = tid; i < t.vol; i += nth) slot[i] = SLOT_FREE;
  if (tid == 0) *s_count = 0;
  __syncthreads();
#pragma unroll
  for (int j = 0; j < NVPT; j++)
#pragma unroll
    for (int k = 0; k < 8; k++) if (vs[j].adm & (1u << k)) slot[vs[j].base + (k >> 2) * sx + ((k >> 1) & 1) * sy + (k & 1)] = SLOT_MARK;
  __syncthreads();
  for (int i0 = 0; i0 < t.vol; i0 += nth) {
    const int i = i0 + tid;
    const bool marked = i < t.vol && slot[i] == SLOT_MARK;
    const unsigned long long b = __ballot(marked);
    int first = 0;
    if ((tid & 63) == 0 && b) first = atomicAdd(s_count, (int)__popcll(b));
    first = __shfl(first, 0);
    if (marked) {
      const int n = first + (int)__popcll(b & ((1ull << (tid & 63)) - 1ull));
      if (n < NODE_CAP) { slot[i] = (unsigned short)n; list[n] = (unsigned short)i; }
    }
  }
  __syncthreads();
  return *s_count;
}

__device__ void spread_direct(const LatView &v, int nv, long base, const double *px, const double *py, const double *pz, const double *fx,
                              const double *fy, const double *fz, const double *rx, const double *ry, const double *rz, double *F,
                              const unsigned char *dead) {
  for (int i = threadIdx.x; i < nv; i += blockDim.x) {
    if (dead && dead[base + i]) continue;
    Stencil s;
    phi2_stencil(v, px[base + i], py[base + i], pz[base + i], s);
    const double f0 = (rx ? rx[base + i] : 0.0) + fx[base + i], f1 = (ry ? ry[base + i] : 0.0) + fy[base + i], f2 = (rz ? rz[base + i] : 0.0) + fz[base + i];
#pragma unroll
    for (int k = 0; k < 8; k++) {
      if (s.node[k] < 0) continue;
      v.dirty[s.node[k] >> 4] = v.epoch;
      double *Fn = F + 3 * s.node[k];
      unsafeAtomicAdd(Fn, f0 * s.w[k]);
      unsafeAtomicAdd(Fn + 1, f1 * s.w[k]);
      unsafeAtomicAdd(Fn + 2, f2 * s.w[k]);
    }
  }
}

__global__ __launch_bounds__(256) void ibm_spread_cell_kernel(LatView v, int nv, const double *px, const double *py, const double *pz,
                                                              double *fx, double *fy, double *fz, const double *rx, const double *ry, const double *rz,
                                                              double *F, int limit_on, double f_limit, int xcd_ranges, const int *tag, const unsigned char *vdead) {
  __shared__ unsigned short slot[TILE_CAP];
  __shared__ __attribute__((aligned(16))) unsigned char raw[TILE_CAP > 2 * NODE_CAP ? TILE_CAP : 2 * NODE_CAP];
  unsigned char *mt = raw; unsigned short *list = reinterpret_cast<unsigned short *>(raw);
  __shared__ double acc[3 * NODE_CAP];
  __shared__ int s_red[6 * MAXW], s_count, s_near;
  const int tid = threadIdx.x, nth = blockDim.x;
  PH_INIT
  const int cell = xcd_ranges ? xcd_contiguous((int)blockIdx.x, (int)gridDim.x) : (int)blockIdx.x;
  const int state = tag[cell];
  if (state == 1) return;
  STAMP(0);
  const unsigned char *dead = state == 2 ? vdead : nullptr;
  const long base = (long)cell * nv;
  const bool in_regs = nv <= NVPT * nth;
  double f[NVPT][3];
  if (in_regs) {
#pragma unroll
    for (int j = 0; j < NVPT; j++) {
      const int i = tid + j * nth;
      f[j][0] = f[j][1] = f[j][2] = 0.0;
      if (i < nv) { f[j][0] = fx[base + i]; f[j][1] = fy[base + i]; f[j][2] = fz[base + i]; }
    }
  }
  Tile t; VStencil vs[NVPT];
  bool tiled = cell_prologue(v, nv, base, px, py, pz, dead, s_red, &s_near, mt, t, vs PH_ARG);
  if (limit_on) {
    if (in_regs) {
#pragma unroll
      for (int j = 0; j < NVPT; j++) {
        const int i = tid + j * nth;
        if (i < nv && !(dead && dead[base + i])) {
          const double mag = sqrt((f[j][0] * f[j][0] + f[j][1] * f[j][1]) + f[j][2] * f[j][2]);
          if (mag > f_limit) { const double sc = f_limit / mag; f[j][0] *= sc; f[j][1] *= sc; f[j][2] *= sc; fx[base + i] = f[j][0]; fy[base + i] = f[j][1]; fz[base + i] = f[j][2]; }
        }
      }
    } else {
      for (int i = tid; i < nv; i += nth) {
        if (dead && dead[base + i]) continue;
        const double f0 = fx[base + i], f1 = fy[base + i], f2 = fz[base + i];
        const double mag = sqrt((f0 * f0 + f1 * f1) + f2 * f2);
        if (mag > f_limit) { const double sc = f_limit / mag; fx[base + i] = f0 * sc; fy[base + i] = f1 * sc; fz[base + i] = f2 * sc; }
      }
    }
  }
  const int n = tiled ? compact_nodes(t, vs, slot, list, &s_count) : 0;
  STAMP(5);
  if (!tiled || n > NODE_CAP) { spread_direct(v, nv, base, px, py, pz, fx, fy, fz, rx, ry, rz, F, dead); return; }
  const int sy = t.e[2], sx = t.e[1] * t.e[2];
  for (int k = tid; k < 3 * n; k += nth) acc[k] = 0.0;
  __syncthreads();
#pragma unroll
  for (int j = 0; j < NVPT; j++) {
    const int i = tid + j * nth;
    if (i >= nv || !vs[j].adm) continue;
    double fv[3];
    fv[0] = (rx ? rx[base + i] : 0.0) + f[j][0]; fv[1] = (ry ? ry[base + i] : 0.0) + f[j][1]; fv[2] = (rz ? rz[base + i] : 0.0) + f[j][2];
#pragma unroll
    for (int k = 0; k < 8; k++) {
      if (!(vs[j].adm & (1u << k))) continue;
      double *a = &acc[3 * slot[vs[j].base + (k >> 2) * sx + ((k >> 1) & 1) * sy + (k & 1)]];
      atomicAdd(a, fv[0] * vs[j].w[k]); atomicAdd(a + 1, fv[1] * vs[j].w[k]); atomicAdd(a + 2, fv[2] * vs[j].w[k]);
    }
  }
  __syncthreads();
  STAMP(6);
  for (int k = tid; k < 3 * n; k += nth) {
    const double val = acc[k];
    if (val != 0.0) {
      const int q = k / 3;
      int lx, ly, lz; const long node = tile_node(v, t, list[q], lx, ly, lz); v.dirty[node >> 4] = v.epoch;
      unsafeAtomicAdd(&F[3 * node + (k - 3 * q)], val);
    }
  }
  STAMP(7);
}

template <bool OPEN = false>
__global__ __launch_bounds__(256) void ibm_interpolate_cell_kernel(LatView v, Pops<OPEN> pv, int nv, const double *px, const double *py,
                                                                   const double *pz, double *vx, double *vy, double *vz, const int *slots, int xcd_ranges,
                                                                   const int *tag, const unsigned char *vdead) {
  __shared__ unsigned short slot[TILE_CAP];
  __shared__ __attribute__((aligned(16))) unsigned char raw[TILE_CAP > 2 * NODE_CAP ? TILE_CAP : 2 * NODE_CAP];
  unsigned char *mt = raw; unsigned short *list = reinterpret_cast<unsigned short *>(raw);
  __shared__ double ux[NODE_CAP], uy[NODE_CAP], uz[NODE_CAP];
  __shared__ int s_red[6 * MAXW], s_count, s_near;
  const int tid = threadIdx.x, nth = blockDim.x;
  const int cell = slots ? slots[blockIdx.x] : (xcd_ranges ? xcd_contiguous((int)blockIdx.x, (int)gridDim.x) : (int)blockIdx.x);
  const int state = tag[cell];
  if (state == 1) return;
  const unsigned char *dead = state == 2 ? vdead : nullptr;
  const long base = (long)cell * nv;
  Tile t; VStencil vs[NVPT];
  PH_INIT
  bool tiled = cell_prologue(v, nv, base, px, py, pz, dead, s_red, &s_near, mt, t, vs PH_ARG);
  const int sy = t.e[2], sx = t.e[1] * t.e[2];
  if (tiled) {
    if (compact_nodes(t, vs, slot, list, &s_count) > NODE_CAP) tiled = false;
    STAMP(12);
  }
  if (tiled) {
    const int n = s_count;
    for (int k = tid; k < n; k += nth) {
      int lx, ly, lz;
      const long node = tile_node(v, t, list[k], lx, ly, lz);
      double u[3];
      node_velocity<OPEN>(v, pv, lx, ly, lz, node, u);
      ux[k] = u[0]; uy[k] = u[1]; uz[k] = u[2];
    }
    __syncthreads();
    STAMP(13);
#pragma unroll
    for (int j = 0; j < NVPT; j++) {
      const int i = tid + j * nth;
      if (i >= nv || (dead && dead[base + i])) continue;
      double a0 = 0.0, a1 = 0.0, a2 = 0.0;
#pragma unroll
      for (int k = 0; k < 8; k++) {
        if (!(vs[j].adm & (1u << k))) continue;
        const int q = slot[vs[j].base + (k >> 2) * sx + ((k >> 1) & 1) * sy + (k & 1)];
        a0 += (ux[q] * vs[j].w[k]); a1 += (uy[q] * vs[j].w[k]); a2 += (uz[q] * vs[j].w[k]);
      }
      vx[base + i] = a0; vy[base + i] = a1; vz[base + i] = a2;
    }
    STAMP(14);
    return;
  }
  for (int i = tid; i < nv; i += nth) {
    if (dead && dead[base + i]) continue;
    Stencil s;
    phi2_stencil(v, px[base + i], py[base + i], pz[base + i], s);
    double a0 = 0.0, a1 = 0.0, a2 = 0.0;
#pragma unroll
    for (int k = 0; k < 8; k++) {
      if (s.node[k] < 0) continue;
      double u[3];
      node_velocity<OPEN>(v, pv, s.lx[k], s.ly[k], s.lz[k], s.node[k], u);
      a0 += (u[0] * s.w[k]); a1 += (u[1] * s.w[k]); a2 += (u[2] * s.w[k]);
    }
    vx[base + i] = a0; vy[base + i] = a1; vz[base + i] = a2;
  }
}

PopView make_pops(const hc_lattice *L) {
  return PopView{L->f[L->cur], L->force[(L->fcur + 2) % 3], L->body[0], L->body[1], L->body[2], (long)L->qstride, L->regions};
}
OpenPopView open_of(const hc_lattice *L, const PopView &pv) {
  OpenPopView o;
  static_cast<PopView &>(o) = pv;
  o.ob_code = L->ob_code; o.ob_val = L->ob_val;
  return o;
}

}

#define HC_LAUNCH_POPS(K, grid, block, v, pv, ...)                                                                      \
  hc::launch_open(L, pv, [&](auto open, const auto &pops) {                                                             \
    hipLaunchKernelGGL(K<decltype(open)::value>, grid, block, 0, hc::stream(), v, pops, __VA_ARGS__);                   \
  })

static int g_ibm_per_vertex = 0;
extern "C" int hc_debug_ibm_per_vertex(int on) { g_ibm_per_vertex = on; return HC_OK; }
static int g_reproducible = -1;
static bool reproducible() {
  if (g_reproducible < 0) { const char *e = std::getenv("HEMOCELL_REPRODUCIBLE_SPREAD"); g_reproducible = (e && *e && *e != '0') ? 1 : 0; }
  return g_reproducible == 1;
}
extern "C" int hc_set_reproducible_spread(int on) { g_reproducible = on ? 1 : 0; return HC_OK; }

static int spread_reproducible(hc_cells *C, int force_limit) {
  const LatView v = make_view(C->L);
  HC_REQUIRE(v.npad * 3 < 0xffffffffL && C->nverts * 8 < 0x7fffffffL, "reproducible spread: lattice or vertex count beyond its 32-bit keys");
  const long n_e = C->nverts * 8;
  int rc;
  if (n_e > C->det_cap) {
    HC_HIP(hipDeviceSynchronize());
    const long cap = n_e + n_e / 4 + 4096;
    C->det_cap = 0;
    for (int k = 0; k < 2; k++) if ((rc = C->det_keys[k].reserve((size_t)cap)) != HC_OK || (rc = C->det_vals[k].reserve((size_t)cap)) != HC_OK) return rc;
    for (int k = 0; k < 3; k++) if ((rc = C->det_val[k].reserve((size_t)cap)) != HC_OK) return rc;
    size_t tmp_bytes = 0;
    HC_HIP(hipcub::DeviceRadixSort::SortPairs(nullptr, tmp_bytes, C->det_keys[0].p, C->det_keys[1].p, C->det_vals[0].p, C->det_vals[1].p, (int)cap, 0, 32, hc::stream()));
    if ((rc = C->det_tmp.reserve(tmp_bytes)) != HC_OK) return rc;
    C->det_cap = cap;
  }
  std::vector<int> order((size_t)0);
  std::vector<long> obase((size_t)C->ntypes, 0);
  for (int t = 0; t < C->ntypes; t++) {
    const size_t nc = (size_t)C->ncells[t], o = order.size();
    obase[(size_t)t] = (long)o;
    order.resize(o + nc);
    std::iota(order.begin() + (long)o, order.end(), 0);
    const std::vector<long> &ids = C->host[t].ids;
    std::stable_sort(order.begin() + (long)o, order.end(), [&](int a, int b) { return ids[(size_t)a] < ids[(size_t)b]; });
  }
  int *d_order = nullptr;
  rc = stage_ints(C, 2, &d_order, order.data(), (int)order.size()); if (rc != HC_OK) return rc;
  long ebase = 0;
  for (int t = 0; t < C->ntypes; t++) {
    const int nv = C->types[t]->host.nv;
    const long n = C->ncells[t] * nv;
    if (n == 0) continue;
    const TypeArrays a = vert_arrays(C, t);
    hipLaunchKernelGGL(spread_emit_kernel, dim3((unsigned)((n + 255) / 256)), dim3(256), 0, hc::stream(), v, nv, n, (const int *)(d_order + obase[(size_t)t]), ebase,
                       a.p[0], a.p[1], a.p[2], a.f[0], a.f[1], a.f[2], a.r[0], a.r[1], a.r[2], force_limit, C->P.f_limit, a.tag, a.dead, C->det_keys[0], C->det_vals[0],
                       C->det_val[0], C->det_val[1], C->det_val[2]);
    HC_HIP(hipGetLastError());
    ebase += n;
  }
  int bits = 1;
  while (bits < 32 && (1L << bits) <= v.npad) bits++;
  size_t tmp = C->det_tmp.cap;
  HC_HIP(hipcub::DeviceRadixSort::SortPairs(C->det_tmp.p, tmp, C->det_keys[0].p, C->det_keys[1].p, C->det_vals[0].p, C->det_vals[1].p, (int)n_e, 0, bits, hc::stream()));
  hipLaunchKernelGGL(spread_gather_kernel, dim3((unsigned)((n_e + 255) / 256)), dim3(256), 0, hc::stream(), v, n_e, (const unsigned int *)C->det_keys[1],
                     (const int *)C->det_vals[1], (const double *)C->det_val[0], (const double *)C->det_val[1], (const double *)C->det_val[2], C->L->force[C->L->fcur]);
  HC_HIP(hipGetLastError());
  return HC_OK;
}
#ifdef HC_IBM_PHASE_TIMES
extern "C" int hc_debug_phase_times(double *out) {
  unsigned long long h[32];
  if (hipMemcpyFromSymbol(h, HIP_SYMBOL(g_phase), sizeof(h)) != hipSuccess) return HC_ERR_HIP;
  for (int k = 0; k < 32; k++) out[k] = (double)h[k];
  std::memset(h, 0, sizeof(h));
  if (hipMemcpyToSymbol(HIP_SYMBOL(g_phase), h, sizeof(h)) != hipSuccess) return HC_ERR_HIP;
  return HC_OK;
}
#endif

extern "C" {

int hcp_spread(hc_cells *C, int force_limit) {
  HC_REQUIRE(C, "hcp_spread: null pointer");
  int rc = sync_to_device(C); if (rc != HC_OK) return rc;
  if (C->nverts == 0) return HC_OK;
  hc::ProfScope prof(hc::PK_SPREAD);
  if (reproducible()) return spread_reproducible(C, force_limit);
  const LatView v = make_view(C->L);
  for (int t = 0; t < C->ntypes; t++) {
    const long n = C->ncells[t] * C->types[t]->host.nv;
    if (n == 0) continue;
    const int nv = C->types[t]->host.nv;
    const TypeArrays a = vert_arrays(C, t);
    if (g_ibm_per_vertex)
      hipLaunchKernelGGL(ibm_spread_kernel, dim3((unsigned)((n + 255) / 256)), dim3(256), 0, hc::stream(), v, n, a.p[0], a.p[1], a.p[2], a.f[0], a.f[1], a.f[2],
                         a.r[0], a.r[1], a.r[2], C->L->force[C->L->fcur], force_limit, C->P.f_limit, a.vert_cell, a.tag_all, a.dead);
    else
      hipLaunchKernelGGL(ibm_spread_cell_kernel, dim3((unsigned)C->ncells[t]), dim3(nv > 128 ? 256 : 128), 0, hc::stream(), v, nv, a.p[0], a.p[1], a.p[2],
                         a.f[0], a.f[1], a.f[2], a.r[0], a.r[1], a.r[2], C->L->force[C->L->fcur], force_limit, C->P.f_limit, 1, a.tag, a.dead);
    HC_HIP(hipGetLastError());
  }
  return HC_OK;
}

int hcp_interpolate(hc_cells *C) {
  HC_REQUIRE(C, "hcp_interpolate: null pointer");
  int rc = sync_to_device(C); if (rc != HC_OK) return rc;
  if (C->nverts == 0) return HC_OK;
  hc::ProfScope prof(hc::PK_INTERP);
  const hc_lattice *L = C->L;
  const LatView v = make_view(L);
  const PopView pv = make_pops(L);
  for (int t = 0; t < C->ntypes; t++) {
    const long n = C->ncells[t] * C->types[t]->host.nv;
    if (n == 0) continue;
    const int nv = C->types[t]->host.nv;
    const TypeArrays a = vert_arrays(C, t);
    if (g_ibm_per_vertex)
      HC_LAUNCH_POPS(ibm_interpolate_kernel, dim3((unsigned)((n + 255) / 256)), dim3(256), v, pv, n, a.p[0], a.p[1], a.p[2], a.v[0], a.v[1], a.v[2],
                     a.vert_cell, a.tag_all, a.dead);
    else
      HC_LAUNCH_POPS(ibm_interpolate_cell_kernel, dim3((unsigned)C->ncells[t]), dim3(nv > 128 ? 256 : 128), v, pv, nv, a.p[0], a.p[1], a.p[2], a.v[0], a.v[1], a.v[2],
                     (const int *)nullptr, 1, a.tag, a.dead);
    HC_HIP(hipGetLastError());
  }
  return HC_OK;
}

int hcl_face_velocity_pack(hc_lattice *L, int side, double *dev_buf) {
  HC_REQUIRE(L && dev_buf && (side == 0 || side == 1), "hcl_face_velocity_pack: bad arguments");
  LatView v = make_view(L);
  v.halo_u[0] = v.halo_u[1] = nullptr;
  const PopView pv = make_pops(L);
  HC_LAUNCH_POPS(face_velocity_kernel, dim3((unsigned)((L->plane + 255) / 256), 1, 1), dim3(256), v, pv, side == 0 ? 0 : L->nx - 1, dev_buf, 0, (double *)nullptr);
  HC_HIP(hipGetLastError());
  return HC_OK;
}
int hcl_face_velocity_pack_both(hc_lattice *L, double *dev_lo, double *dev_hi) {
  HC_REQUIRE(L, "hcl_face_velocity_pack_both: null lattice");
  if (!dev_lo && !dev_hi) return HC_OK;
  if (!dev_lo || !dev_hi) return hcl_face_velocity_pack(L, dev_lo ? 0 : 1, dev_lo ? dev_lo : dev_hi);
  LatView v = make_view(L);
  v.halo_u[0] = v.halo_u[1] = nullptr;
  const PopView pv = make_pops(L);
  HC_LAUNCH_POPS(face_velocity_kernel, dim3((unsigned)((L->plane + 255) / 256), 2, 1), dim3(256), v, pv, 0, dev_lo, L->nx - 1, dev_hi);
  HC_HIP(hipGetLastError());
  return HC_OK;
}

int hcl_download_face_velocity(hc_lattice *L, int side, double *host_u) {
  HC_REQUIRE(L && host_u && (side == 0 || side == 1), "hcl_download_face_velocity: bad arguments");
  hc::DevBuf<double> d;
  int rc = d.reserve(3 * L->plane); if (rc != HC_OK) return rc;
  rc = hcl_face_velocity_pack(L, side, d);
  if (rc == HC_OK && hipMemcpyAsync(host_u, d, 3 * L->plane * sizeof(double), hipMemcpyDeviceToHost, hc::stream()) != hipSuccess) { hc::set_error("hcl_download_face_velocity: copy failed"); rc = HC_ERR_HIP; }
  if (rc == HC_OK && hipStreamSynchronize(hc::stream()) != hipSuccess) { hc::set_error("hcl_download_face_velocity: synchronise failed"); rc = HC_ERR_HIP; }
  return rc;
}

int hcp_interpolate_cells(hc_cells *C, int type, const int *slots, int n) { return hcc::interpolate_cells_staged(C, type, slots, n, 1); }

}

int hcc::interpolate_cells_staged(hc_cells *C, int type, const int *slots, int n, int which) {
  HC_REQUIRE(C && type >= 0 && type < C->ntypes && n >= 0 && which >= 0 && which < 19, "hcp_interpolate_cells: bad arguments");
  if (n == 0) return HC_OK;
  HC_REQUIRE(slots, "hcp_interpolate_cells: null pointer");
  int rc = sync_to_device(C); if (rc != HC_OK) return rc;
  for (int i = 0; i < n; i++) HC_REQUIRE(slots[i] >= 0 && slots[i] < C->ncells[type], "hcp_interpolate_cells: slot out of range");
  int *d_slots = nullptr;
  rc = stage_ints(C, which, &d_slots, slots, n); if (rc != HC_OK) return rc;
  hc::ProfScope prof(hc::PK_INTERP);
  const hc_lattice *L = C->L;
  const LatView v = make_view(L);
  const PopView pv = make_pops(L);
  const TypeArrays a = vert_arrays(C, type);
  const int nv = C->types[type]->host.nv;
  HC_LAUNCH_POPS(ibm_interpolate_cell_kernel, dim3((unsigned)n), dim3(nv > 128 ? 256 : 128), v, pv, nv, a.p[0], a.p[1], a.p[2], a.v[0], a.v[1], a.v[2],
                 (const int *)d_slots, 0, a.tag, a.dead);
  HC_HIP(hipGetLastError());
  return HC_OK;
}
```

hemocell_amd/csrc/mechanics.hip:

```cpp
#include "cells.h"

namespace {

struct MechArgs {
  int model, nv, nt, ne, nie;
  const int *tri, *edge, *ebt, *ebo, *iedge;
  const int *vtri, *vtri_k, *vedge, *vedge_s, *bsrc, *vouter, *vinner, *vinner_s, *ring, *nring;
  const double *tri_area_eq, *edge_len_eq, *edge_angle_eq, *patch_eq, *iedge_len_eq;
  double volume_eq, area_mean_eq, edge_mean_eq;
  double k_volume, k_area, k_link, k_bend, eta_m;
  const double *px, *py, *pz, *vx, *vy, *vz;
  double *fx, *fy, *fz;
  double *comp;
  long ncv;
  const int *tag;
  double k_inner_rigid, k_cytoskeleton, core_radius, radius;
  double k_inner_link;
};

#define MaxCellVolumetricChange 0.01
#define MaxCellSurfaceAreaChange 0.09
#define MaxCellBendingAngle 0.0555
#define MaxPLTBendingAngle 2.467
#define MaxCellPersistenceLength 9.0
// ... 62 lines not shown
    for (int t = 0; t < nt; t++) volume += tV[t];
    volume *= (1.0 / 6.0);
    const double vf = (volume - m.volume_eq) / m.volume_eq;
    s_volume_force = -m.k_volume * vf / fabs(MaxCellVolumetricChange - vf * vf);
  }

  if (!PLT) {
    double *Bx = ex, *By = ex + nv, *Bz = ex + 2 * nv;
    for (int i = tid; i < nv; i += nth) {
      const int nn = m.nring[i];
      const double x = xs[i], y = ys[i], z = zs[i];
      double sx = 0., sy = 0., sz = 0.;
      for (int j = 0; j < nn; j++) { const int r = m.ring[6 * i + j]; sx += xs[r]; sy += ys[r]; sz += zs[r]; }
      const double dvx = sx / nn - x, dvy = sy / nn - y, dvz = sz / nn - z;
      double pnx = 0., pny = 0., pnz = 0.;
      for (int j = 0; j < nn; j++) {
        const int ra = m.ring[6 * i + j], rb = m.ring[6 * i + (j + 1 == nn ? 0 : j + 1)];
        const double ax = xs[ra] - x, ay = ys[ra] - y, az = zs[ra] - z, bx = xs[rb] - x, by = ys[rb] - y, bz = zs[rb] - z;
        double cx = ay * bz - az * by, cy = az * bx - ax * bz, cz = ax * by - ay * bx;
        const double l = norm3(cx, cy, cz);
        cx /= l; cy /= l; cz /= l;
        pnx += cx; pny += cy; pnz += cz;
      }
      const double l = norm3(pnx, pny, pnz);
      pnx /= l; pny /= l; pnz /= l;
      const double ndev = dot3(pnx, pny, pnz, dvx, dvy, dvz);
      const double dDev = (ndev - m.patch_eq[i]) / m.edge_mean_eq;
      const double mag = m.k_bend * (dDev + dDev / fabs(MaxCellBendingAngle - dDev * dDev));
      Bx[i] = mag * pnx; By[i] = mag * pny; Bz[i] = mag * pnz;
    }
  } else {
    double *Lx = ex, *Ly = ex + ne, *Lz = ex + 2 * ne, *Vx = ex + 3 * ne, *Vy = ex + 4 * ne, *Vz = ex + 5 * ne,
           *Gx = ex + 6 * ne, *Gy = ex + 7 * ne, *Gz = ex + 8 * ne;
    for (int e = tid; e < ne; e += nth) {
      const int e0 = m.edge[2 * e], e1 = m.edge[2 * e + 1];
      const double evx = xs[e1] - xs[e0], evy = ys[e1] - ys[e0], evz = zs[e1] - zs[e0];
      const double el = sqrt(evx * evx + evy * evy + evz * evz);
      const double ux = evx / el, uy = evy / el, uz = evz / el;
      const double leq = m.edge_len_eq[e];
      const double ef = (el - leq) / leq;
      const double fs = m.k_link * (ef + ef / fabs(MaxCellPersistenceLength - ef * ef));
      Lx[e] = ux * fs; Ly[e] = uy * fs; Lz[e] = uz * fs;
      const double rvx = m.vx[base + e1] - m.vx[base + e0], rvy = m.vy[base + e1] - m.vy[base + e0], rvz = m.vz[base + e1] - m.vz[base + e0];
      const double pr = dot3(rvx, rvy, rvz, ux, uy, uz);
      double wx = m.eta_m * (pr * ux), wy = m.eta_m * (pr * uy), wz = m.eta_m * (pr * uz);
      const double wm = norm3(wx, wy, wz);
      if (wm > FORCE_LIMIT_PN / 4.0) { const double sc = (FORCE_LIMIT_PN / 4.0) / wm; wx *= sc; wy *= sc; wz *= sc; }
      Vx[e] = wx; Vy[e] = wy; Vz[e] = wz;
      const int b0 = m.ebt[2 * e], b1 = m.ebt[2 * e + 1];
      const double a = tNx[b0] + tNx[b1], b = tNy[b0] + tNy[b1], c = tNz[b0] + tNz[b1];
      const double crx = tNy[b0] * tNz[b1] - tNz[b0] * tNy[b1], cry = tNz[b0] * tNx[b1] - tNx[b0] * tNz[b1], crz = tNx[b0] * tNy[b1] - tNy[b0] * tNx[b1];
      const double angle = atan2(dot3(crx, cry, crz, ux, uy, uz), dot3(tNx[b0], tNy[b0], tNz[b0], tNx[b1], tNy[b1], tNz[b1]));
      const double af = angle - m.edge_angle_eq[e];
      const double fm = m.k_bend * (af + af / fabs(MaxPLTBendingAngle - af * af));
      Gx[e] = (fm * a) * 0.5; Gy[e] = (fm * b) * 0.5; Gz[e] = (fm * c) * 0.5;
    }
  }
  __syncthreads();
  const double volume_force = s_volume_force;

  for (int i = tid; i < nv; i += nth) {
    double acc[SEPARATE ? 6 : 1][3];
#pragma unroll
    for (int c = 0; c < (SEPARATE ? 6 : 1); c++) acc[c][0] = acc[c][1] = acc[c][2] = 0.0;
#define ACC(C) acc[SEPARATE ? (C) : 0]
    const double x = xs[i], y = ys[i], z = zs[i];
    for (int k = 0; k < MD; k++) {
      const int t = m.vtri[MD * i + k];
      if (t < 0) break;
      const int i0 = m.tri[3 * t], i1 = m.tri[3 * t + 1], i2 = m.tri[3 * t + 2];
      const double cx = (xs[i0] + xs[i1] + xs[i2]) / 3.0, cy = (ys[i0] + ys[i1] + ys[i2]) / 3.0, cz = (zs[i0] + zs[i1] + zs[i2]) / 3.0;
      double afm;
      if (PLT) afm = tAfm[t];
      else {
        const TriGeom g = tri_geom(xs, ys, zs, i0, i1, i2);
        const double aeq = m.tri_area_eq[t];
        const double areaRatio = (g.area - aeq) / aeq;
        afm = m.k_area * (areaRatio + areaRatio / fabs(MaxCellSurfaceAreaChange - areaRatio * areaRatio));
      }
      ACC(1)[0] += afm * (cx - x); ACC(1)[1] += afm * (cy - y); ACC(1)[2] += afm * (cz - z);
    }
    for (int k = 0; k < MD; k++) {
      const int t = m.vtri[MD * i + k];
      if (t < 0) break;
      TriGeom g;
      if (PLT) { g.area = tA[t]; g.nx = tNx[t]; g.ny = tNy[t]; g.nz = tNz[t]; }
      else g = tri_geom(xs, ys, zs, m.tri[3 * t], m.tri[3 * t + 1], m.tri[3 * t + 2]);
      const double sc = g.area / m.area_mean_eq;
      ACC(0)[0] += (volume_force * g.nx) * sc; ACC(0)[1] += (volume_force * g.ny) * sc; ACC(0)[2] += (volume_force * g.nz) * sc;
    }
    if (!PLT) {
      const double *Bx = ex, *By = ex + nv, *Bz = ex + 2 * nv;
      for (int k = 0; k < MD; k++) {
        const int src = m.bsrc[MD * i + k];
        if (src < 0) break;
        if (src == i) { ACC(2)[0] += Bx[i]; ACC(2)[1] += By[i]; ACC(2)[2] += Bz[i]; }
        else { const int nn = m.nring[src]; ACC(2)[0] += -Bx[src] / nn; ACC(2)[1] += -By[src] / nn; ACC(2)[2] += -Bz[src] / nn; }
      }
      for (int k = 0; k < MD; k++) {
        const int e = m.vedge[MD * i + k];
        if (e < 0) break;
        const int e0 = m.edge[2 * e], e1 = m.edge[2 * e + 1];
        const double evx = xs[e1] - xs[e0], evy = ys[e1] - ys[e0], evz = zs[e1] - zs[e0];
        const double el = norm3(evx, evy, evz);
        const double ux = evx / el, uy = evy / el, uz = evz / el;
        const double leq = m.edge_len_eq[e];
        const double ef = (el - leq) / leq;
        const double fs = m.k_link * (ef + ef / fabs(MaxCellPersistenceLength - ef * ef));
        const double frx = ux * fs, fry = uy * fs, frz = uz * fs;
        const bool first = m.vedge_s[MD * i + k] > 0;
        if (first) { ACC(3)[0] += frx; ACC(3)[1] += fry; ACC(3)[2] += frz; } else { ACC(3)[0] -= frx; ACC(3)[1] -= fry; ACC(3)[2] -= frz; }
        if (WBC || MAL || m.eta_m != 0.0) {
          const double rvx = m.vx[base + e1] - m.vx[base + e0], rvy = m.vy[base + e1] - m.vy[base + e0], rvz = m.vz[base + e1] - m.vz[base + e0];
          const double pr = dot3(rvx, rvy, rvz, ux, uy, uz);
          double wx = m.eta_m * (pr * ux), wy = m.eta_m * (pr * uy), wz = m.eta_m * (pr * uz);
          const double wm = norm3(wx, wy, wz);
          if (wm > FORCE_LIMIT_PN / 4.0) { const double sc = (FORCE_LIMIT_PN / 4.0) / wm; wx *= sc; wy *= sc; wz *= sc; }
          if (first) { ACC(4)[0] += wx; ACC(4)[1] += wy; ACC(4)[2] += wz; } else { ACC(4)[0] -= wx; ACC(4)[1] -= wy; ACC(4)[2] -= wz; }
        }
      }
      if (WBC) {
        const double d_cyto = 2 * m.radius, d_core = 2 * m.core_radius;
        for (int k = 0; k < MD; k++) {
          const int e = m.vinner[MD * i + k];
          if (e < 0) break;
          const int e0 = m.iedge[2 * e], e1 = m.iedge[2 * e + 1];
          const double evx = xs[e1] - xs[e0], evy = ys[e1] - ys[e0], evz = zs[e1] - zs[e0];
          const double el = norm3(evx, evy, evz);
          const double ux = evx / el, uy = evy / el, uz = evz / el;
          const bool first = m.vinner_s[MD * i + k] > 0;
          for (int term = 0; term < 2; term++) {
            const double d = term == 0 ? d_cyto : d_core, kk = term == 0 ? m.k_cytoskeleton : m.k_inner_rigid;
            if (!(el < d)) continue;
            const double s = 1.0 - (el / d);
            const double frx = (ux * s) * kk, fry = (uy * s) * kk, frz = (uz * s) * kk;
            if (first) { ACC(5)[0] -= frx; ACC(5)[1] -= fry; ACC(5)[2] -= frz; } else { ACC(5)[0] += frx; ACC(5)[1] += fry; ACC(5)[2] += frz; }
          }
        }
      }
      if (MAL) {
        for (int k = 0; k < MD; k++) {
          const int e = m.vinner[MD * i + k];
          if (e < 0) break;
          const int e0 = m.iedge[2 * e], e1 = m.iedge[2 * e + 1];
          const double evx = xs[e1] - xs[e0], evy = ys[e1] - ys[e0], evz = zs[e1] - zs[e0];
          const double el = sqrt(evx * evx + evy * evy + evz * evz);
          const double ux = evx / el, uy = evy / el, uz = evz / el;
          const double leq = m.iedge_len_eq[e];
          const double ef = (el - leq) / leq;
          const double fs = m.k_inner_link * 5.0 * ef;
          if (m.vinner_s[MD * i + k] > 0) { ACC(5)[0] += ux * fs; ACC(5)[1] += uy * fs; ACC(5)[2] += uz * fs; }
          else { ACC(5)[0] -= ux * fs; ACC(5)[1] -= uy * fs; ACC(5)[2] -= uz * fs; }
        }
      }
    } else {
      const double *Lx = ex, *Ly = ex + ne, *Lz = ex + 2 * ne, *Vx = ex + 3 * ne, *Vy = ex + 4 * ne, *Vz = ex + 5 * ne,
                   *Gx = ex + 6 * ne, *Gy = ex + 7 * ne, *Gz = ex + 8 * ne;
      int ka = 0, kb = 0;
      while (true) {
        const int ea = ka < MD ? m.vedge[MD * i + ka] : -1, eb = kb < MD ? m.vouter[MD * i + kb] : -1;
        if (ea < 0 && eb < 0) break;
        if (eb < 0 || (ea >= 0 && ea < eb)) {
          const bool first = m.vedge_s[MD * i + ka] > 0;
          if (first) { ACC(3)[0] += Lx[ea]; ACC(3)[1] += Ly[ea]; ACC(3)[2] += Lz[ea]; ACC(4)[0] += Vx[ea]; ACC(4)[1] += Vy[ea]; ACC(4)[2] += Vz[ea]; }
          else { ACC(3)[0] -= Lx[ea]; ACC(3)[1] -= Ly[ea]; ACC(3)[2] -= Lz[ea]; ACC(4)[0] -= Vx[ea]; ACC(4)[1] -= Vy[ea]; ACC(4)[2] -= Vz[ea]; }
          ACC(2)[0] += Gx[ea]; ACC(2)[1] += Gy[ea]; ACC(2)[2] += Gz[ea];
          ka++;
        } else {
          ACC(2)[0] -= Gx[eb]; ACC(2)[1] -= Gy[eb]; ACC(2)[2] -= Gz[eb];
          kb++;
        }
      }
      for (int k = 0; k < MD; k++) {
        const int e = m.vinner[MD * i + k];
        if (e < 0) break;
        const int e0 = m.iedge[2 * e], e1 = m.iedge[2 * e + 1];
        const double evx = xs[e1] - xs[e0], evy = ys[e1] - ys[e0], evz = zs[e1] - zs[e0];
        const double el = sqrt(evx * evx + evy * evy + evz * evz);
        const double ux = evx / el, uy = evy / el, uz = evz / el;
        const double leq = m.iedge_len_eq[e];
        const double ef = (el - leq) / leq;
        const double fs = m.k_link * 5.0 * ef;
        if (m.vinner_s[MD * i + k] > 0) { ACC(5)[0] += ux * fs; ACC(5)[1] += uy * fs; ACC(5)[2] += uz * fs; }
        else { ACC(5)[0] -= ux * fs; ACC(5)[1] -= uy * fs; ACC(5)[2] -= uz * fs; }
      }
    }
#undef ACC
    if (SEPARATE) {
#pragma unroll
      for (int c = 0; c < 6; c++)
        for (int d = 0; d < 3; d++) m.comp[((long)c * m.ncv + base + i) * 3 + d] = acc[c][d];
    } else {
      m.fx[base + i] = acc[0][0]; m.fy[base + i] = acc[0][1]; m.fz[base + i] = acc[0][2];
    }
  }
}

__global__ __launch_bounds__(256) void cell_info_kernel(int nv, int nt, const int *tri, const double *px, const double *py, const double *pz,
                                                        const int *tag, const unsigned char *dead, double *volume, double *area, double *bbox,
                                                        double *centroid) {
  __shared__ double red[256][12];
  const int tid = threadIdx.x;
  const long base = (long)blockIdx.x * nv;
  const bool incomplete = tag[blockIdx.x] == 2;
  double vol = 0, ar = 0, lo[3] = {1e300, 1e300, 1e300}, hi[3] = {-1e300, -1e300, -1e300}, cs[3] = {0, 0, 0}, cnt = 0;
  for (int t = tid; t < nt; t += 256) {
    const long i0 = base + tri[3 * t], i1 = base + tri[3 * t + 1], i2 = base + tri[3 * t + 2];
    const double v0x = px[i0], v0y = py[i0], v0z = pz[i0], v1x = px[i1], v1y = py[i1], v1z = pz[i1], v2x = px[i2], v2y = py[i2], v2z = pz[i2];
    vol += (-v2x * v1y * v0z + v1x * v2y * v0z + v2x * v0y * v1z - v0x * v2y * v1z - v1x * v0y * v2z + v0x * v1y * v2z);
    const double e1x = v1x - v0x, e1y = v1y - v0y, e1z = v1z - v0z, e2x = v2x - v0x, e2y = v2y - v0y, e2z = v2z - v0z;
    const double nx = e1y * e2z - e1z * e2y, ny = e1z * e2x - e1x * e2z, nz = e1x * e2y - e1y * e2x;
    ar += 0.5 * sqrt(nx * nx + ny * ny + nz * nz);
  }
  for (int i = tid; i < nv; i += 256) {
    if (incomplete && dead[base + i]) continue;
    const double p[3] = {px[base + i], py[base + i], pz[base + i]};
    for (int d = 0; d < 3; d++) { lo[d] = fmin(lo[d], p[d]); hi[d] = fmax(hi[d], p[d]); cs[d] += p[d]; }
    cnt += 1.0;
  }
  red[tid][0] = vol; red[tid][1] = ar; red[tid][11] = cnt;
  for (int d = 0; d < 3; d++) { red[tid][2 + d] = lo[d]; red[tid][5 + d] = hi[d]; red[tid][8 + d] = cs[d]; }
  __syncthreads();
  for (int s = 128; s > 0; s >>= 1) {
    if (tid < s) {
      red[tid][0] += red[tid + s][0]; red[tid][1] += red[tid + s][1]; red[tid][11] += red[tid + s][11];
      for (int d = 0; d < 3; d++) {
        red[tid][2 + d] = fmin(red[tid][2 + d], red[tid + s][2 + d]);
        red[tid][5 + d] = fmax(red[tid][5 + d], red[tid + s][5 + d]);
        red[tid][8 + d] += red[tid + s][8 + d];
      }
    }
    __syncthreads();
  }
  if (tid == 0) {
    const long c = blockIdx.x;
    volume[c] = red[0][0] / 6.0; area[c] = red[0][1];
    for (int d = 0; d < 3; d++) { bbox[6 * c + 2 * d] = red[0][2 + d]; bbox[6 * c + 2 * d + 1] = red[0][5 + d]; centroid[3 * c + d] = red[0][8 + d] / red[0][11]; }
  }
}

}

static MechArgs mech_args(const hc_cells *C, int t) {
  const hc_celltype *T = C->types[t];
  MechArgs m;
  m.model = T->host.model; m.nv = T->host.nv; m.nt = T->host.nt; m.ne = T->host.ne; m.nie = T->host.nie;
  m.tri = T->d_tri; m.edge = T->d_edge; m.ebt = T->d_ebt; m.ebo = T->d_ebo; m.iedge = T->d_iedge;
  m.vtri = T->d_vtri; m.vtri_k = T->d_vtri_k; m.vedge = T->d_vedge; m.vedge_s = T->d_vedge_s; m.bsrc = T->d_bsrc;
  m.vouter = T->d_vouter; m.vinner = T->d_vinner; m.vinner_s = T->d_vinner_s; m.ring = T->d_ring; m.nring = T->d_nring;
  m.tri_area_eq = T->d_tri_area_eq; m.edge_len_eq = T->d_edge_len_eq; m.edge_angle_eq = T->d_edge_angle_eq;
  m.patch_eq = T->d_patch_eq; m.iedge_len_eq = T->d_iedge_len_eq;
  m.volume_eq = T->host.volume_eq; m.area_mean_eq = T->host.area_mean_eq; m.edge_mean_eq = T->host.edge_mean_eq;
  m.k_volume = T->host.k_volume; m.k_area = T->host.k_area; m.k_link = T->host.k_link; m.k_bend = T->host.k_bend; m.eta_m = T->host.eta_m;
  const long f = C->first[t];
  m.px = C->pos[0] + f; m.py = C->pos[1] + f; m.pz = C->pos[2] + f;
  m.vx = C->vel[0] + f; m.vy = C->vel[1] + f; m.vz = C->vel[2] + f;
  m.fx = C->frc[0] + f; m.fy = C->frc[1] + f; m.fz = C->frc[2] + f;
  m.comp = nullptr; m.ncv = C->ncells[t] * T->host.nv;
  m.tag = C->d_tag + C->cell0[t];
  m.k_inner_rigid = T->host.k_inner_rigid; m.k_cytoskeleton = T->host.k_cytoskeleton; m.core_radius = T->host.core_radius; m.radius = T->host.wbc_radius;
  m.k_inner_link = T->host.k_inner_link;
  return m;
}

static size_t mech_lds_bytes(const CellTables &T) {
  if (T.model != HC_MODEL_PLT_SIMPLE) return (6 * (size_t)T.nv + (size_t)T.nt) * sizeof(double);
  return (3 * (size_t)T.nv + 6 * (size_t)T.nt + 9 * (size_t)T.ne) * sizeof(double);
}

static int launch_mechanics(hc_cells *C, int t, double *comp) {
  if (C->ncells[t] == 0) return HC_OK;
  MechArgs m = mech_args(C, t);
  m.comp = comp;
  const CellTables &T = C->types[t]->host;
  const size_t lds = mech_lds_bytes(T);
  HC_REQUIRE(lds <= 160 * 1024 - 64, "mechanics: cell type does not fit the 160 KiB LDS of a CU");
  const int threads = T.nv > 128 ? 256 : 128;
  const dim3 grid((unsigned)C->ncells[t]);
  HC_REQUIRE(T.md == CellTables::MAXD || T.md == CellTables::MAXD_WIDE, "mechanics: unsupported per-vertex table width");
#define LAUNCH1(MODEL, SEP, W)                                                                                    \
  do {                                                                                                            \
    HC_HIP(hipFuncSetAttribute((const void *)mechanics_kernel<MODEL, SEP, W>, hipFuncAttributeMaxDynamicSharedMemorySize, (int)lds)); \
    hipLaunchKernelGGL((mechanics_kernel<MODEL, SEP, W>), grid, dim3(threads), lds, hc::stream(), m);             \
  } while (0)
#define LAUNCH(MODEL, SEP)                                                                                        \
  do {                                                                                                            \
    if (T.md == CellTables::MAXD) LAUNCH1(MODEL, SEP, CellTables::MAXD); else LAUNCH1(MODEL, SEP, CellTables::MAXD_WIDE); \
  } while (0)
  if (T.model == HC_MODEL_RBC_HO) { if (comp) LAUNCH(HC_MODEL_RBC_HO, true); else LAUNCH(HC_MODEL_RBC_HO, false); }
  else if (T.model == HC_MODEL_WBC_HO) { if (comp) LAUNCH(HC_MODEL_WBC_HO, true); else LAUNCH(HC_MODEL_WBC_HO, false); }
  else if (T.model == HC_MODEL_RBC_MALARIA) { if (comp) LAUNCH(HC_MODEL_RBC_MALARIA, true); else LAUNCH(HC_MODEL_RBC_MALARIA, false); }
  else { if (comp) LAUNCH(HC_MODEL_PLT_SIMPLE, true); else LAUNCH(HC_MODEL_PLT_SIMPLE, false); }
#undef LAUNCH
#undef LAUNCH1
  HC_HIP(hipGetLastError());
  return HC_OK;
}

extern "C" {

int hcp_mechanics(hc_cells *C, long iter, int forced) {
  HC_REQUIRE(C, "hcp_mechanics: null pointer");
  int rc = sync_to_device(C); if (rc != HC_OK) return rc;
  hc::ProfScope prof(hc::PK_MECH);
  for (int t = 0; t < C->ntypes; t++) {
    if (!(iter % C->timescale[t] == 0 || forced)) continue;
    rc = launch_mechanics(C, t, nullptr);
    if (rc != HC_OK) return rc;
  }
  return HC_OK;
}

static int info_scratch(hc_cells *C, size_t doubles) {
  if (C->info.cap() >= doubles) return HC_OK;
  HC_HIP(hipStreamSynchronize(hc::stream()));
  return C->info.reserve(doubles + doubles / 4 + 1024);
}

int hcp_mechanics_components(hc_cells *C, int type, double *comp) {
  HC_REQUIRE(C && comp && type >= 0 && type < C->ntypes, "hcp_mechanics_components: bad arguments");
  int rc = settle(C); if (rc != HC_OK) return rc;
  rc = sync_to_device(C); if (rc != HC_OK) return rc;
  const long n = C->ncells[type] * C->types[type]->host.nv;
  if (n == 0) return HC_OK;
  rc = info_scratch(C, (size_t)(18 * n)); if (rc != HC_OK) return rc;
  rc = launch_mechanics(C, type, C->info.d); if (rc != HC_OK) return rc;
  HC_HIP(hipMemcpyAsync(C->info.h, C->info.d, (size_t)(18 * n) * sizeof(double), hipMemcpyDeviceToHost, hc::stream()));
  HC_HIP(hipStreamSynchronize(hc::stream()));
  std::memcpy(comp, C->info.h, (size_t)(18 * n) * sizeof(double));
  return HC_OK;
}

int hcp_cell_info(hc_cells *C, int type, double *volume, double *area, double *bbox, double *centroid) {
  HC_REQUIRE(C && volume && area && bbox && centroid && type >= 0 && type < C->ntypes, "hcp_cell_info: bad arguments");
  int rc = settle(C); if (rc != HC_OK) return rc;
  rc = sync_to_device(C); if (rc != HC_OK) return rc;
  const long nc = C->ncells[type];
  if (nc == 0) return HC_OK;
  const CellTables &T = C->types[type]->host;
  rc = info_scratch(C, (size_t)(11 * nc)); if (rc != HC_OK) return rc;
  double *d = C->info.d;
  const double *h = C->info.h;
  const TypeArrays a = vert_arrays(C, type);
  hipLaunchKernelGGL(cell_info_kernel, dim3((unsigned)nc), dim3(256), 0, hc::stream(), T.nv, T.nt, C->types[type]->d_tri, a.p[0], a.p[1], a.p[2], a.tag, a.dead,
                     d, d + nc, d + 2 * nc, d + 8 * nc);
  HC_HIP(hipGetLastError());
  HC_HIP(hipMemcpyAsync(C->info.h, d, (size_t)(11 * nc) * sizeof(double), hipMemcpyDeviceToHost, hc::stream()));
  HC_HIP(hipStreamSynchronize(hc::stream()));
  std::memcpy(volume, h, (size_t)nc * sizeof(double));
  std::memcpy(area, h + nc, (size_t)nc * sizeof(double));
  std::memcpy(bbox, h + 2 * nc, (size_t)(6 * nc) * sizeof(double));
  std::memcpy(centroid, h + 8 * nc, (size_t)(3 * nc) * sizeof(double));
  return HC_OK;
}

}
```

hemocell_amd/csrc/solidify.hip:

```cpp
#include "raycast.h"
#include <memory>

namespace {

__global__ __launch_bounds__(256) void binding_populate_kernel(LatView v, uint8_t *binding, int x0, int y0, int z0, int ex, int ey, int ez) {
  const long k = (long)blockIdx.x * 256 + threadIdx.x;
  if (k >= (long)ex * ey * ez) return;
  const int ix = (int)(k / ((long)ey * ez)), r = (int)(k - (long)ix * ey * ez), iy = r / ez, iz = r - iy * ez;
  const long gx = (long)v.x0 + x0 + ix, gy = y0 + iy, gz = z0 + iz;
  const long node = lattice_node(v, gx, gy, gz);
  if (node < 0 || v.mask[node] == 0) return;
  for (int a = -1; a <= 1; a++)
    for (int b = -1; b <= 1; b++)
      for (int c = -1; c <= 1; c++) {
        const long nb = lattice_node(v, gx + a, gy + b, gz + c);
        if (nb >= 0 && v.mask[nb] == 0) { binding[node] = 1; return; }
      }
}

__device__ __forceinline__ void jacobi_rotate(double &app, double &aqq, double &apq, double &arp, double &arq) {
  if (apq == 0.0) return;
  const double theta = (aqq - app) / (2.0 * apq);
  double t;
  if (fabs(theta) > 1.0e150) t = 0.5 / theta;
  else { t = 1.0 / (fabs(theta) + sqrt(theta * theta + 1.0)); if (theta < 0.0) t = -t; }
  const double c = 1.0 / sqrt(t * t + 1.0), s = t * c;
  app = app - t * apq; aqq = aqq + t * apq; apq = 0.0;
  const double rp = c * arp - s * arq, rq = s * arp + c * arq;
  arp = rp; arq = rq;
}

constexpr int JACOBI_SWEEPS = 6;
__device__ __forceinline__ double tresca_of(double xx, double xy, double xz, double yy, double yz, double zz) {
#pragma unroll 1
  for (int sweep = 0; sweep < JACOBI_SWEEPS; sweep++) {
    jacobi_rotate(xx, yy, xy, xz, yz);
    jacobi_rotate(xx, zz, xz, xy, yz);
    jacobi_rotate(yy, zz, yz, xy, xz);
  }
  const double hi = fmax(xx, fmax(yy, zz)), lo = fmin(xx, fmin(yy, zz));
  return (hi - lo) / 2.0;
}

__device__ __forceinline__ double tresca_at(const LatView &v, const double *__restrict__ fin, long qs, double omega, int lx, int ly, int lz, long node) {
  double f[HC_Q];
  pull(fin, qs, node, hc::neighbours(v, v.plane, lx, ly, lz), f);
  double rhoBar, j0, j1, j2;
  moments(f, rhoBar, j0, j1, j2);
  const double invRho = 1.0 / (1.0 + rhoBar);
  double xx = 0, xy = 0, xz = 0, yy = 0, yz = 0, zz = 0;
#define M(Q, CX, CY, CZ)                       \
  if (CX * CX) xx += f[Q];                     \
  if (CX * CY == 1) xy += f[Q]; else if (CX * CY == -1) xy += -f[Q]; \
  if (CX * CZ == 1) xz += f[Q]; else if (CX * CZ == -1) xz += -f[Q]; \
  if (CY * CY) yy += f[Q];                     \
  if (CY * CZ == 1) yz += f[Q]; else if (CY * CZ == -1) yz += -f[Q]; \
  if (CZ * CZ) zz += f[Q];
  FOR_Q(M)
#undef M
  const double cs2 = 1.0 / 3.0;
  const double pre = (-omega * 3.0) / (2.0 * (1.0 + rhoBar));
  return tresca_of(pre * (xx - invRho * j0 * j0 - cs2 * rhoBar), pre * (xy - invRho * j0 * j1), pre * (xz - invRho * j0 * j2),
                   pre * (yy - invRho * j1 * j1 - cs2 * rhoBar), pre * (yz - invRho * j1 * j2), pre * (zz - invRho * j2 * j2 - cs2 * rhoBar));
}

__global__ __launch_bounds__(256) void tresca_kernel(LatView v, const double *fin, long qs, double omega, double *out) {
  const int p = blockIdx.x * 256 + threadIdx.x;
  const int ny_nz = v.ny * v.nz;
  if (p >= ny_nz) return;
  const int x = blockIdx.y, y = p / v.nz, z = p - y * v.nz;
  const long node = (long)(x + HALO) * v.plane + p;
  out[(long)x * ny_nz + p] = v.mask[node] == 0 ? tresca_at(v, fin, qs, omega, x, y, z, node) : 0.0;
}

struct PrepareArgs {
  LatView v;
  uint8_t *mask, *binding, *wallbrick;
  int nv, nt;
  const int *tri;
  const double *px, *py, *pz;
  int *tag;
  const unsigned char *sflag;
  int *ntag;
  int *solid;
};

__global__ void solidify_prepare_kernel(PrepareArgs a) {
  extern __shared__ double lds[];
  __shared__ int s_any;
  const int nv = a.nv;
  double *xs = lds, *ys = xs + nv, *zs = ys + nv;
  if (a.tag[blockIdx.x] != 0) return;
  if (threadIdx.x == 0) s_any = 0;
  int lo[3], hi[3];
  stage_cell(a, xs, ys, zs, lo, hi);
  const long base = (long)blockIdx.x * nv;
  bool any = false;
  for (int i = threadIdx.x; i < nv; i += blockDim.x) any = any || a.sflag[base + i] != 0;
  if (any) s_any = 1;
  __syncthreads();
  if (!s_any) return;
  int converted = 0;
  const bool sweep = !(hi[0] < lo[0] || hi[1] < lo[1] || hi[2] < lo[2]) &&
                     !((long)hi[0] - lo[0] >= 4L * a.v.nx || (long)hi[1] - lo[1] >= 4L * a.v.ny || (long)hi[2] - lo[2] >= 4L * a.v.nz);
  if (sweep) {
    const long ey = (long)hi[1] - lo[1] + 1, ez = (long)hi[2] - lo[2] + 1;
    const long count = ((long)hi[0] - lo[0] + 1) * ey * ez;
    for (long k = threadIdx.x; k < count; k += blockDim.x) {
      const long ix = k / (ey * ez), r = k - ix * ey * ez, iy = r / ez, iz = r - iy * ez;
      const long gx = lo[0] + ix, gy = lo[1] + iy, gz = lo[2] + iz;
      const long node = lattice_node(a.v, gx, gy, gz);
      if (node < 0 || a.mask[node] != 0) continue;
      if (ray_crossings(xs, ys, zs, a.tri, a.nt, (double)gx, (double)gy, (double)gz) % 2 == 0) continue;
      const unsigned bit = 1u << (8 * (unsigned)(node & 3));
      const unsigned old = atomicOr(reinterpret_cast<unsigned *>(a.mask + (node & ~3L)), bit);
      if (((old >> (8 * (unsigned)(node & 3))) & 0xffu) == 0) converted++;
      a.binding[node] = 1;
      const long xp = node / a.v.plane, rem = node - xp * a.v.plane;
      const long y = rem / a.v.nz, z = rem - y * a.v.nz;
      a.wallbrick[((xp >> 3) * a.v.nby + (y >> 3)) * a.v.nbz + (z >> 3)] = 1;
    }
  }
  if (converted) atomicAdd(&a.solid[1], converted);
  if (threadIdx.x == 0 && atomicExch(&a.tag[blockIdx.x], 1) != 1) {
    atomicAdd(&a.ntag[0], 1); atomicAdd(&a.ntag[3], 1);
    atomicAdd(&a.solid[0], 1);
  }
}

__global__ __launch_bounds__(256) void solidify_flag_kernel(LatView v, long n, const uint8_t *binding, const double *fin, long qs, double omega,
                                                            const double *px, const double *py, const double *pz, unsigned char *sflag,
                                                            const int *vert_cell, const int *tag, const unsigned char *dead, double dist_max, double shear_min) {
  const long i = (long)blockIdx.x * 256 + threadIdx.x;
  if (i >= n) return;
  if (dead[i] || tag[vert_cell[i]] == 1) return;
  const double x = px[i], y = py[i], z = pz[i];
  const long cx = nearest_node(x), cy = nearest_node(y), cz = nearest_node(z);
  const long node = lattice_node(v, cx, cy, cz);
  if (node < 0) return;
  bool near = false;
  for (int dx = -1; dx <= 1; dx++)
    for (int dy = -1; dy <= 1; dy++)
      for (int dz = -1; dz <= 1; dz++) {
        const long gx = cx + dx, gy = cy + dy, gz = cz + dz;
        const long b = lattice_node(v, gx, gy, gz);
        if (b < 0 || !binding[b]) continue;
        const double d0 = x - (double)gx, d1 = y - (double)gy, d2 = z - (double)gz;
        if (sqrt(d0 * d0 + d1 * d1 + d2 * d2) <= dist_max) near = true;
      }
  if (!near || v.mask[node] != 0) return;
  const long xp = node / v.plane, rem = node - xp * v.plane;
  const int ly = (int)(rem / v.nz), lz = (int)(rem - (long)ly * v.nz);
  const double tresca = tresca_at(v, fin, qs, omega, (int)xp - HALO, ly, lz, node);
  if (fabs(tresca / 1e-7) > shear_min) sflag[i] = 1;
}

__global__ __launch_bounds__(256) void add_walls_kernel(LatView v, long npad, const uint8_t *add, uint8_t *mask, uint8_t *wallbrick) {
  const long node = (long)blockIdx.x * 256 + threadIdx.x;
  if (node >= npad || !add[node] || mask[node] != 0) return;
  mask[node] = 1;
  const long xp = node / v.plane, rem = node - xp * v.plane;
  const long y = rem / v.nz, z = rem - y * v.nz;
  wallbrick[((xp >> 3) * v.nby + (y >> 3)) * v.nbz + (z >> 3)] = 1;
}

__global__ void publish_solid_kernel(const int *solid, int *host_view) { host_view[0] = solid[0]; host_view[1] = solid[1]; }

int g_block = 256;

int ensure_binding(hc_lattice *L) {
  if (L->binding) return HC_OK;
  const int rc = L->binding.reserve(L->npad); if (rc != HC_OK) return rc;
  HC_HIP(hipMemsetAsync(L->binding, 0, L->npad, hc::stream()));
  return HC_OK;
}

void to_bulk(const hc_lattice *L, const std::vector<uint8_t> &pad, uint8_t *out) {
  for (int x = 0; x < L->nx; x++) std::memcpy(out + (size_t)x * L->plane, pad.data() + (size_t)(x + HALO) * L->xs, L->plane);
}

int refuse(const char *who, const hc_lattice *L) {
  const char *why = solidify_refusal(L);
  if (!why) return HC_OK;
  hc::set_error(std::string(who) + ": " + why);
  return HC_ERR_ARG;
}

}

namespace hcc {

const char *solidify_refusal(const hc_lattice *L) {
  if (L->n_slabs > 1) return "solidify mechanics run on one domain (n_slabs = 1)";
  if (L->ob_n > 0) return "solidify mechanics do not combine with open boundaries";
  if (L->le_on) return "solidify mechanics do not combine with a Lees-Edwards boundary";
  if (L->visc_n > 0) return "solidify mechanics do not combine with interior viscosity";
  if (hc::in_preinlet_pair(L)) return "solidify mechanics do not combine with a pre-inlet";
  return nullptr;
}

int ensure_sflag(hc_cells *C) {
  if (C->d_sflag || C->cap <= 0) return HC_OK;
  const int rc = C->d_sflag.reserve((size_t)C->cap); if (rc != HC_OK) return rc;
  HC_HIP(hipMemset(C->d_sflag, 0, (size_t)C->cap));
  return HC_OK;
}

static int launch_prepare(hc_cells *C) {
  hc_lattice *L = C->L;
  hc::ProfScope prof(hc::PK_SOLIDIFY_PREPARE);
  for (int t = 0; t < C->ntypes; t++) {
    if (!C->solid_on[t] || C->ncells[t] == 0) continue;
    const hc_celltype *T = C->types[t];
    const TypeArrays va = vert_arrays(C, t);
    PrepareArgs a;
    a.v = make_view(L);
    a.mask = L->mask; a.binding = L->binding; a.wallbrick = L->wallbrick;
    a.nv = T->host.nv; a.nt = T->host.nt; a.tri = T->d_tri;
    a.px = va.p[0]; a.py = va.p[1]; a.pz = va.p[2]; a.tag = va.tag;
    a.sflag = C->d_sflag + C->first[t];
    a.ntag = C->d_ntag; a.solid = C->d_solid;
    hipLaunchKernelGGL(solidify_prepare_kernel, dim3((unsigned)C->ncells[t]), dim3(g_block), 3 * (size_t)T->host.nv * sizeof(double), hc::stream(), a);
    HC_HIP(hipGetLastError());
  }
  C->maybe_tagged = true;
  return HC_OK;
}

static int launch_flag(hc_cells *C) {
  hc_lattice *L = C->L;
  hc::ProfScope prof(hc::PK_SOLIDIFY_FLAG);
  const LatView v = make_view(L);
  for (int t = 0; t < C->ntypes; t++) {
    const long n = C->ncells[t] * C->types[t]->host.nv;
    if (!C->solid_on[t] || n == 0) continue;
    const TypeArrays a = vert_arrays(C, t);
    hipLaunchKernelGGL(solidify_flag_kernel, dim3((unsigned)((n + 255) / 256)), dim3(256), 0, hc::stream(), v, n, (const uint8_t *)L->binding,
                       (const double *)L->f[L->cur], (long)L->qstride, L->omega, a.p[0], a.p[1], a.p[2], C->d_sflag + C->first[t], a.vert_cell,
                       (const int *)a.tag_all, (const unsigned char *)a.dead, C->solid_dist[t], C->solid_shear[t]);
    HC_HIP(hipGetLastError());
  }
  return HC_OK;
}

static int ready(hc_cells *C, const char *who) {
  if (!C->solidify_on()) { hc::set_error(std::string(who) + ": no cell type has solidify mechanics (hcp_type_set_solidify)"); return HC_ERR_STATE; }
  int rc = refuse(who, C->L); if (rc != HC_OK) return rc;
  if ((rc = sync_to_device(C)) != HC_OK || (rc = ensure_binding(C->L)) != HC_OK) return rc;
  return ensure_sflag(C);
}

int solidify_check(hc_cells *C) {
  int rc = ready(C, "hc_iterate"); if (rc != HC_OK) return rc;
  if (C->nverts == 0) return HC_OK;
  if ((rc = launch_prepare(C)) != HC_OK) return rc;
  return launch_flag(C);
}

int solidify_refresh_mask(hc_cells *C) {
  hc_lattice *L = C->L;
  if (!C->d_solid) return HC_OK;
  hipLaunchKernelGGL(publish_solid_kernel, dim3(1), dim3(1), 0, hc::stream(), (const int *)C->d_solid, C->h_solid.dev);
  HC_HIP(hipGetLastError());
  HC_HIP(hipStreamSynchronize(hc::stream()));
  if ((long)C->h_solid[1] == C->solid_nodes_seen) return HC_OK;
  HC_HIP(hipMemcpy(L->hmask.data(), L->mask, L->npad, hipMemcpyDeviceToHost));
  C->solid_nodes_seen = (long)C->h_solid[1];
  return HC_OK;
}

}

extern "C" {

int hc_debug_solidify_block(int threads) {
  HC_REQUIRE(threads == 64 || threads == 128 || threads == 256 || threads == 512, "hc_debug_solidify_block: 64, 128, 256 or 512 threads");
  g_block = threads;
  return HC_OK;
}

int hcl_binding_populate(hc_lattice *L, const int box[6]) {
  HC_REQUIRE(L && box, "hcl_binding_populate: null pointer");
  int rc = refuse("hcl_binding_populate", L); if (rc != HC_OK) return rc;
  if ((rc = ensure_binding(L)) != HC_OK) return rc;
  const int b[6] = {std::max(box[0], 0), std::min(box[1], L->nx - 1), std::max(box[2], 0), std::min(box[3], L->ny - 1), std::max(box[4], 0), std::min(box[5], L->nz - 1)};
  if (b[0] > b[1] || b[2] > b[3] || b[4] > b[5]) return HC_OK;
  const int ex = b[1] - b[0] + 1, ey = b[3] - b[2] + 1, ez = b[5] - b[4] + 1;
  const long n = (long)ex * ey * ez;
  hipLaunchKernelGGL(binding_populate_kernel, dim3((unsigned)((n + 255) / 256)), dim3(256), 0, hc::stream(), make_view(L), L->binding.p, b[0], b[2], b[4], ex, ey, ez);
  HC_HIP(hipGetLastError());
  return HC_OK;
}

int hcl_binding_clear(hc_lattice *L) {
  HC_REQUIRE(L, "hcl_binding_clear: null pointer");
  int rc = refuse("hcl_binding_clear", L); if (rc != HC_OK) return rc;
  if (!L->binding) return ensure_binding(L);
  HC_HIP(hipMemsetAsync(L->binding, 0, L->npad, hc::stream()));
  return HC_OK;
}

int hcl_binding_download(hc_lattice *L, uint8_t *out) {
  HC_REQUIRE(L && out, "hcl_binding_download: null pointer");
  if (!L->binding) { std::memset(out, 0, (size_t)L->nx * L->plane); return HC_OK; }
  std::vector<uint8_t> pad(L->npad);
  HC_HIP(hipMemcpyAsync(pad.data(), L->binding, L->npad, hipMemcpyDeviceToHost, hc::stream()));
  HC_HIP(hipStreamSynchronize(hc::stream()));
  to_bulk(L, pad, out);
  return HC_OK;
}

int hcl_binding_upload(hc_lattice *L, const uint8_t *in) {
  HC_REQUIRE(L && in, "hcl_binding_upload: null pointer");
  int rc = refuse("hcl_binding_upload", L); if (rc != HC_OK) return rc;
  if ((rc = ensure_binding(L)) != HC_OK) return rc;
  std::vector<uint8_t> pad(L->npad, 0);
  for (int x = 0; x < L->nx; x++)
    for (size_t p = 0; p < L->plane; p++) pad[(size_t)(x + HALO) * L->xs + p] = in[(size_t)x * L->plane + p] ? 1 : 0;
  HC_HIP(hipMemcpyAsync(L->binding, pad.data(), L->npad, hipMemcpyHostToDevice, hc::stream()));
  HC_HIP(hipStreamSynchronize(hc::stream()));
  return HC_OK;
}

int hcl_download_mask(hc_lattice *L, uint8_t *out) {
  HC_REQUIRE(L && out, "hcl_download_mask: null pointer");
  std::vector<uint8_t> pad(L->npad);
  HC_HIP(hipMemcpyAsync(pad.data(), L->mask, L->npad, hipMemcpyDeviceToHost, hc::stream()));
  HC_HIP(hipStreamSynchronize(hc::stream()));
  to_bulk(L, pad, out);
  return HC_OK;
}

int hcl_upload_solidified_mask(hc_lattice *L, const uint8_t *in) {
  HC_REQUIRE(L && in, "hcl_upload_solidified_mask: null pointer");
  int rc = refuse("hcl_upload_solidified_mask", L); if (rc != HC_OK) return rc;
  std::vector<uint8_t> pad(L->npad, 0);
  for (int x = 0; x < L->nx; x++)
    for (size_t p = 0; p < L->plane; p++) pad[(size_t)(x + HALO) * L->xs + p] = in[(size_t)x * L->plane + p] ? 1 : 0;
  hc::DevBuf<uint8_t> d;
  if ((rc = d.reserve(L->npad)) != HC_OK) return rc;
  HC_HIP(hipMemcpyAsync(d, pad.data(), L->npad, hipMemcpyHostToDevice, hc::stream()));
  hipLaunchKernelGGL(add_walls_kernel, dim3((unsigned)((L->npad + 255) / 256)), dim3(256), 0, hc::stream(), make_view(L), (long)L->npad, (const uint8_t *)d.p, L->mask.p, L->wallbrick.p);
  HC_HIP(hipGetLastError());
  HC_HIP(hipMemcpyAsync(L->hmask.data(), L->mask, L->npad, hipMemcpyDeviceToHost, hc::stream()));
  HC_HIP(hipStreamSynchronize(hc::stream()));
  return HC_OK;
}

int hcl_download_tresca(hc_lattice *L, double *out) {
  HC_REQUIRE(L && out, "hcl_download_tresca: null pointer");
  HC_REQUIRE(L->n_slabs == 1 && L->ob_n == 0 && L->visc_n == 0, "hcl_download_tresca: one domain without open boundaries and without interior viscosity (the value is formed with the lattice's one omega)");
  const size_t n = (size_t)L->nx * L->plane;
  int rc = L->scratch.reserve(n); if (rc != HC_OK) return rc;
  hipLaunchKernelGGL(tresca_kernel, dim3((unsigned)((L->plane + 255) / 256), (unsigned)L->nx), dim3(256), 0, hc::stream(), make_view(L),
                     (const double *)L->f[L->cur], (long)L->qstride, L->omega, L->scratch.p);
  HC_HIP(hipGetLastError());
  HC_HIP(hipMemcpyAsync(out, L->scratch, n * sizeof(double), hipMemcpyDeviceToHost, hc::stream()));
  HC_HIP(hipStreamSynchronize(hc::stream()));
  return HC_OK;
}

int hcp_type_set_solidify(hc_cells *C, int type, double distance_threshold_lu, double shear_threshold) {
  HC_REQUIRE(C && type >= 0 && type < C->ntypes, "hcp_type_set_solidify: unknown cell type");
  HC_REQUIRE(C->types[type]->host.model == HC_MODEL_PLT_SIMPLE, "hcp_type_set_solidify: only HC_MODEL_PLT_SIMPLE (PltSimpleModel) implements solidifyMechanics");
  HC_REQUIRE(distance_threshold_lu >= 0.0 && shear_threshold >= 0.0, "hcp_type_set_solidify: the thresholds must not be negative");
  HC_REQUIRE(3 * (size_t)C->types[type]->host.nv * sizeof(double) <= 60 * 1024, "hcp_type_set_solidify: the positions of one cell of the type exceed 60 KiB of LDS");
  int rc = refuse("hcp_type_set_solidify", C->L); if (rc != HC_OK) return rc;
  if (!C->d_solid) {
    std::unique_ptr<int[]> zero(new int[2]());
    if ((rc = C->d_solid.reserve(2)) != HC_OK || (rc = C->h_solid.reserve(2)) != HC_OK) return rc;
    HC_HIP(hipMemcpy(C->d_solid, zero.get(), 2 * sizeof(int), hipMemcpyHostToDevice));
    C->h_solid[0] = C->h_solid[1] = 0;
  }
  C->solid_on[type] = 1; C->solid_dist[type] = distance_threshold_lu; C->solid_shear[type] = shear_threshold;
  if (!C->host_dirty) return ensure_sflag(C);
  return HC_OK;
}

int hcp_set_solidify_timescale(hc_cells *C, int every) {
  HC_REQUIRE(C && every >= 1, "hcp_set_solidify_timescale: the timescale must be >= 1");
  C->solid_every = every;
  return HC_OK;
}

int hcp_solidify_prepare(hc_cells *C) {
  HC_REQUIRE(C, "hcp_solidify_prepare: null pointer");
  int rc = ready(C, "hcp_solidify_prepare"); if (rc != HC_OK) return rc;
  if (C->nverts > 0 && (rc = launch_prepare(C)) != HC_OK) return rc;
  return solidify_refresh_mask(C);
}

int hcp_solidify_flag(hc_cells *C) {
  HC_REQUIRE(C, "hcp_solidify_flag: null pointer");
  int rc = ready(C, "hcp_solidify_flag"); if (rc != HC_OK) return rc;
  if (C->nverts > 0 && (rc = launch_flag(C)) != HC_OK) return rc;
  return solidify_refresh_mask(C);
}

int hcp_solidify_flags_download(hc_cells *C, unsigned char *out) {
  HC_REQUIRE(C && out, "hcp_solidify_flags_download: null pointer");
  int rc = settle(C); if (rc != HC_OK) return rc;
  rc = sync_to_host(C); if (rc != HC_OK) return rc;
  size_t o = 0;
  for (int t = 0; t < C->ntypes; t++) { const std::vector<unsigned char> &f = C->host[t].sflag; std::copy(f.begin(), f.end(), out + o); o += f.size(); }
  return HC_OK;
}

int hcp_solidify_flags_upload(hc_cells *C, const unsigned char *in) {
  HC_REQUIRE(C && in, "hcp_solidify_flags_upload: null pointer");
  if (!C->solidify_on()) { hc::set_error("hcp_solidify_flags_upload: no cell type has solidify mechanics (hcp_type_set_solidify)"); return HC_ERR_STATE; }
  int rc = settle(C); if (rc != HC_OK) return rc;
  rc = sync_to_host(C); if (rc != HC_OK) return rc;
  size_t o = 0;
  for (int t = 0; t < C->ntypes; t++) {
    std::vector<unsigned char> &f = C->host[t].sflag;
    for (size_t i = 0; i < f.size(); i++) f[i] = in[o + i] ? 1 : 0;
    o += f.size();
  }
  C->host_dirty = true;
  return HC_OK;
}

int hcp_solidify_counts(hc_cells *C, long out[3]) {
  HC_REQUIRE(C && out, "hcp_solidify_counts: null pointer");
  int rc = settle(C); if (rc != HC_OK) return rc;
  rc = sync_to_host(C); if (rc != HC_OK) return rc;
  if ((rc = solidify_refresh_mask(C)) != HC_OK) return rc;
  out[0] = C->d_solid ? (long)C->h_solid[0] : 0; out[1] = C->d_solid ? (long)C->h_solid[1] : 0; out[2] = 0;
  for (int t = 0; t < C->ntypes; t++) for (unsigned char f : C->host[t].sflag) out[2] += f ? 1 : 0;
  return HC_OK;
}

}
```

hemocell_amd/host.py:

```python
import ctypes as C
import math
import os
import xml.etree.ElementTree as ET

import numpy as np

from . import capi
from .capi import CellTypeSpec, HcError, Material, Params, WbcMaterial, check, dptr, lptr

HALO = 2

MODEL_RBC_HO = 0
MODEL_PLT_SIMPLE = 1
MODEL_WBC_HO = 2
MODEL_RBC_MALARIA = 3
WBC_SPHERE = 0
RBC_FROM_SPHERE = 1
MESH_FROM_STL = 2
ELLIPSOID_FROM_SPHERE = 6

WBC_HO_XML = os.path.join(os.path.dirname(os.path.dirname(os.path.abspath(__file__))), "tests", "golden", "wbc_case",
                          "WBC_HO.xml")
MALARIA_XML = os.path.join(os.path.dirname(os.path.dirname(os.path.abspath(__file__))), "tests", "golden", "malaria_case",
                           "RBC_MALARIA.xml")

PLT_INNER_EDGES = np.array([[60, 65], [62, 64], [37, 42], [54, 56], [34, 40], [25, 46], [50, 59], [29, 47],
                            [61, 63], [26, 45], [33, 43], [27, 35], [32, 39], [49, 51], [0, 4], [48, 52],
                            [6, 10], [53, 55], [19, 21], [57, 58], [15, 13]], dtype=np.int64)

_initialised = False


def _iptr(array):
    return array.ctypes.data_as(C.POINTER(C.c_int))


def read_material(path):
    mm = ET.parse(path).getroot().find("MaterialModel")
    if mm is None:
        raise HcError("%s has no <MaterialModel>" % path)
    out = {}
    for el in mm:
        if el.tag == "InnerEdges":
            out["inner_edges"] = np.array([[int(v) for v in e.text.split()] for e in el.iter("Edge")], np.int64).reshape(-1, 2)
            continue
        try:
            out[el.tag] = float(el.text)
        except (TypeError, ValueError):
            pass
    return out


def read_stl_file_tag(path):
    el = ET.parse(path).getroot().find("MaterialModel/StlFile")
    return None if el is None or not (el.text or "").strip() else el.text.strip()


def init(device=0):
    global _initialised
    check(capi.lib().hc_init(device))
    _initialised = True


def ensure_init():
    if not _initialised:
        init(0)


def base_parameters(dx=5e-7, dt=1e-7, nuP=1.1e-6, rhoP=1025.0, kBT=4.100531391e-21):
    P = Params()
    check(capi.lib().hc_params_base(C.byref(P), dx, dt, nuP, rhoP, kBT))
    return P


class Lattice:

    def __init__(self, nx, ny, nz, periodic=(False, False, False), omega=1.0, x0=0, nx_global=None, n_slabs=1):
        ensure_init()
        self.lib = capi.lib()
        self.nx, self.ny, self.nz = int(nx), int(ny), int(nz)
        self.x0 = int(x0)
        self.nx_global = int(nx_global if nx_global is not None else nx)
        self.n_slabs = int(n_slabs)
        self.periodic = tuple(bool(p) for p in periodic)
        per = (C.c_int * 3)(*[int(p) for p in periodic])
        self.ptr = C.c_void_p()
        check(self.lib.hcl_create(C.byref(self.ptr), self.nx, self.ny, self.nz, per, float(omega),
                                  self.x0, self.nx_global, self.n_slabs))
        self.n = self.nx * self.ny * self.nz

    def defineBounceBack(self, mask_global):
        m = np.ascontiguousarray(mask_global, dtype=np.uint8)
        if m.shape != (self.nx_global, self.ny, self.nz):
            raise HcError("mask must have the global shape %s, got %s" % ((self.nx_global, self.ny, self.nz), m.shape))
        xs = np.arange(self.x0 - HALO, self.x0 + self.nx + HALO)
        if self.periodic[0]:
            local = m[np.mod(xs, self.nx_global)]
        else:
            local = np.ones((len(xs), self.ny, self.nz), np.uint8)
            ok = (xs >= 0) & (xs < self.nx_global)
            local[ok] = m[xs[ok]]
        local = np.ascontiguousarray(local)
        check(self.lib.hcl_set_mask(self.ptr, local.ctypes.data))

    def latticeEquilibrium(self, rho=1.0, u=(0.0, 0.0, 0.0)):
        uu = np.array(u, dtype=np.float64)
        check(self.lib.hcl_init_equilibrium(self.ptr, float(rho), dptr(uu)))

    def setExternalVector(self, F):
        ff = np.array(F, dtype=np.float64)
        check(self.lib.hcl_set_body_force(self.ptr, dptr(ff)))

    def setExternalVectorBoxes(self, boxes, forces):
        bb = np.ascontiguousarray(boxes, dtype=np.int32).reshape(-1, 6)
        ff = np.ascontiguousarray(forces, dtype=np.float64).reshape(-1, 3)
        assert len(bb) == len(ff)
        check(self.lib.hcl_set_body_force_regions(self.ptr, len(bb), _iptr(bb), dptr(ff)))

    def setBoundaryVelocity(self, wall_class, u):
        if isinstance(wall_class, (int, np.integer)):
            uu = np.array(u, dtype=np.float64)
            check(self.lib.hcl_set_wall_velocity(self.ptr, int(wall_class), dptr(uu)))
            return
        self._set_open(wall_class, u, 3, self.lib.hcl_open_boundary_set_velocity)

    def setBoundaryDensity(self, where, rho):
        self._set_open(where, rho, 1, self.lib.hcl_open_boundary_set_density)

    def addVelocityBoundary0N(self, box):
        return self._add_open_box(0, -1, box)

    def addVelocityBoundary0P(self, box):
        return self._add_open_box(0, 1, box)

    def addPressureBoundary0N(self, box):
        return self._add_open_box(1, -1, box)

    def addPressureBoundary0P(self, box):
        return self._add_open_box(1, 1, box)

    def addVelocityBoundary1N(self, box):
        return self._add_open_box(0, -1, box, 1)

    def addVelocityBoundary1P(self, box):
        return self._add_open_box(0, 1, box, 1)

    def addPressureBoundary1N(self, box):
        return self._add_open_box(1, -1, box, 1)

    def addPressureBoundary1P(self, box):
        return self._add_open_box(1, 1, box, 1)

    def addVelocityBoundary2N(self, box):
        return self._add_open_box(0, -1, box, 2)

    def addVelocityBoundary2P(self, box):
        return self._add_open_box(0, 1, box, 2)

    def addPressureBoundary2N(self, box):
        return self._add_open_box(1, -1, box, 2)

    def addPressureBoundary2P(self, box):
        return self._add_open_box(1, 1, box, 2)

    def addOpenBoundaryNodes(self, kind, orientation, nodes, axis=0):
        nn = np.ascontiguousarray(nodes, dtype=np.int32).reshape(-1, 3)
        first = C.c_int()
        check(self.lib.hcl_open_boundary_add_axis(self.ptr, int(kind), int(axis), int(orientation),
                                                  _iptr(nn), len(nn), C.byref(first)))
        return first.value

    def openBoundaryAxes(self, nodes):
        nn = np.ascontiguousarray(nodes, dtype=np.int32).reshape(-1, 3)
        out = np.empty(len(nn), np.int32)
        check(self.lib.hcl_open_boundary_axes(self.ptr, _iptr(nn), len(nn), _iptr(out)))
        return out

    def clearOpenBoundaries(self):
        check(self.lib.hcl_open_boundary_clear(self.ptr))

    def openBoundarySlots(self, nodes):
        nn = np.ascontiguousarray(nodes, dtype=np.int32).reshape(-1, 3)
        out = np.empty(len(nn), np.int32)
        check(self.lib.hcl_open_boundary_slots(self.ptr, _iptr(nn), len(nn), _iptr(out)))
        return out

    def setOpenBoundaryVelocitySlots(self, first_slot, u):
        uu = np.ascontiguousarray(u, dtype=np.float64).reshape(-1, 3)
        check(self.lib.hcl_open_boundary_set_velocity(self.ptr, int(first_slot), len(uu), uu.ctypes.data, 0))

    def setOpenBoundaryDensitySlots(self, first_slot, rho):
        rr = np.ascontiguousarray(rho, dtype=np.float64).reshape(-1)
        check(self.lib.hcl_open_boundary_set_density(self.ptr, int(first_slot), len(rr), rr.ctypes.data, 0))

    def openBoundaryValues(self, first_slot, n):
        out = np.empty((int(n), 4))
        check(self.lib.hcl_open_boundary_values(self.ptr, int(first_slot), int(n), dptr(out)))
        return out

    def planeVelocity(self, x, yz):
        ii = np.ascontiguousarray(yz, dtype=np.int32).reshape(-1)
        out = np.empty((len(ii), 3))
        check(self.lib.hcl_plane_velocity(self.ptr, int(x), _iptr(ii), len(ii), out.ctypes.data, 0))
        return out

    def planeVelocityAxis(self, axis, plane, idx):
        ii = np.ascontiguousarray(idx, dtype=np.int32).reshape(-1)
        out = np.empty((len(ii), 3))
        check(self.lib.hcl_plane_velocity_axis(self.ptr, int(axis), int(plane), _iptr(ii), len(ii),
                                               out.ctypes.data, 0))
        return out

    def _add_open_box(self, kind, orientation, box, axis=0):
        bb = (C.c_int * 6)(*[int(v) for v in box])
        first, n = C.c_int(), C.c_int()
        check(self.lib.hcl_open_boundary_add_box_axis(self.ptr, int(kind), int(axis), int(orientation), bb, C.byref(first), C.byref(n)))
        return first.value, n.value

    def _set_open(self, where, values, nc, fn):
        w = np.asarray(where)
        if w.shape == (6,):
            x0, x1, y0, y1, z0, z1 = [int(v) for v in w]
            g = np.mgrid[x0:x1 + 1, y0:y1 + 1, z0:z1 + 1].reshape(3, -1).T
        else:
            g = w.reshape(-1, 3)
        slots = self.openBoundarySlots(g)
        if (slots < 0).any():
            raise HcError("node %s is not an open-boundary node" % (tuple(g[np.argmax(slots < 0)]),))
        v = np.asarray(values, dtype=np.float64)
        v = np.broadcast_to(v.reshape(-1, nc) if v.size != nc else v.reshape(1, nc), (len(g), nc))
        order = np.argsort(slots, kind="stable")
        s, vv = slots[order], np.ascontiguousarray(v[order])
        cut = np.flatnonzero(np.diff(s) != 1) + 1
        for a, b in zip(np.r_[0, cut], np.r_[cut, len(s)]):
            blk = np.ascontiguousarray(vv[a:b])
            check(fn(self.ptr, int(s[a]), int(b - a), blk.ctypes.data, 0))

    def collideAndStream(self, steps=1):
        check(self.lib.hcl_collide_stream(self.ptr, int(steps)))

    def setLeesEdwards(self, v_top, v_bottom):
        check(self.lib.hcl_set_lees_edwards(self.ptr, float(v_top), float(v_bottom)))

    def setLeesEdwardsDisplacement(self, D, d_per_iteration=0.0):
        check(self.lib.hcl_set_lees_edwards_displacement(self.ptr, float(D), float(d_per_iteration)))

    def applyLeesEdwards(self):
        check(self.lib.hcl_lees_edwards_apply(self.ptr))

    def leesEdwardsState(self):
        o = np.zeros(4)
        check(self.lib.hcl_lees_edwards_state(self.ptr, dptr(o)))
        return tuple(float(v) for v in o)

    def collide_part(self, part):
        check(self.lib.hcl_collide_stream_part(self.ptr, int(part)))

    def fluid_stats(self, what=0):
        o = np.zeros(3); n = C.c_long()
        check(self.lib.hcl_fluid_stats(self.ptr, int(what), dptr(o), C.byref(n)))
        return o[0], o[1], (o[2] / n.value if n.value else 0.0), n.value

    def step_end(self):
        check(self.lib.hcl_step_end(self.ptr))

    def populations(self):
        out = np.empty((self.n, 19), dtype=np.float64)
        check(self.lib.hcl_download_populations(self.ptr, dptr(out)))
        return out

    def set_populations(self, f):
        f = np.ascontiguousarray(f, dtype=np.float64)
        if f.shape != (self.n, 19):
            raise HcError("populations must have shape (%d, 19), got %s" % (self.n, f.shape))
        check(self.lib.hcl_upload_populations(self.ptr, dptr(f)))

    def rho_u(self):
        rho = np.empty(self.n, dtype=np.float64)
        u = np.empty((self.n, 3), dtype=np.float64)
        check(self.lib.hcl_download_rho_u(self.ptr, dptr(rho), dptr(u)))
        return rho, u

    def pi_neq(self):
        pi = np.empty((self.n, 6), dtype=np.float64)
        check(self.lib.hcl_download_pi_neq(self.ptr, dptr(pi)))
        return pi

    def ibm_force(self):
        F = np.empty((self.n, 3), dtype=np.float64)
        check(self.lib.hcl_download_ibm_force(self.ptr, dptr(F)))
        return F

    def halo_doubles(self, width):
        return int(self.lib.hcl_halo_doubles(self.ptr, int(width)))

    def halo_pack(self, side, width, dev_ptr, next=False):
        fn = self.lib.hcl_halo_pack_next if next else self.lib.hcl_halo_pack
        check(fn(self.ptr, int(side), int(width), C.c_void_p(dev_ptr)))

    def halo_unpack(self, side, width, dev_ptr):
        check(self.lib.hcl_halo_unpack(self.ptr, int(side), int(width), C.c_void_p(dev_ptr)))

    def bytes_per_node(self):
        return float(self.lib.hcl_mlups_bytes_per_node(self.ptr))

    def enableInteriorViscosity(self, omegas):
        oo = np.ascontiguousarray(omegas, dtype=np.float64).reshape(-1)
        check(self.lib.hcl_interior_enable(self.ptr, len(oo), dptr(oo)))

    def interiorViscosityOmegas(self):
        n = C.c_int()
        oo = np.zeros(7)
        check(self.lib.hcl_interior_info(self.ptr, C.byref(n), dptr(oo)))
        return oo[:n.value].copy()

    def setInteriorClasses(self, classes):
        cc = np.ascontiguousarray(classes, dtype=np.uint8)
        if cc.size != self.n:
            raise HcError("classes must have %d entries, got %d" % (self.n, cc.size))
        check(self.lib.hcl_interior_upload_classes(self.ptr, cc.ctypes.data))

    def interiorClasses(self):
        out = np.empty((self.nx, self.ny, self.nz), dtype=np.uint8)
        check(self.lib.hcl_interior_download_classes(self.ptr, out.ctypes.data))
        return out

    def populateBindingSites(self, box):
        b = [int(v) for v in box]
        if len(b) != 6:
            raise HcError("a box is (x0, x1, y0, y1, z0, z1), got %r" % (box,))
        check(self.lib.hcl_binding_populate(self.ptr, (C.c_int * 6)(*b)))

    def bindingSites(self):
        out = np.empty((self.nx, self.ny, self.nz), dtype=np.uint8)
        check(self.lib.hcl_binding_download(self.ptr, out.ctypes.data))
        return out

    def setBindingSites(self, sites):
        ss = np.ascontiguousarray(sites, dtype=np.uint8)
        if ss.size != self.n:
            raise HcError("the binding field must have %d entries, got %d" % (self.n, ss.size))
        check(self.lib.hcl_binding_upload(self.ptr, ss.ctypes.data))

    def clearBindingSites(self):
        check(self.lib.hcl_binding_clear(self.ptr))

    def mask(self):
        out = np.empty((self.nx, self.ny, self.nz), dtype=np.uint8)
        check(self.lib.hcl_download_mask(self.ptr, out.ctypes.data))
        return out

    def node_counts(self):
        o = (C.c_long * 3)()
        check(self.lib.hcl_node_counts(self.ptr, o))
        return tuple(int(v) for v in o)

    def tresca(self):
        out = np.empty(self.n, dtype=np.float64)
        check(self.lib.hcl_download_tresca(self.ptr, dptr(out)))
        return out

    def createCEPACfield(self, tau):
        if not tau > 0.0:
            raise HcError("createCEPACfield: tau must be positive, got %r" % (tau,))
        self.scalar = Scalar(self, 1.0 / float(tau))
        return self.scalar

    def destroy(self):
        if self.ptr:
# ... 640 lines not shown
```

include/hemocell_amd.h:

```cpp
#ifndef HEMOCELL_AMD_H
#define HEMOCELL_AMD_H

#include <stddef.h>
#include <stdint.h>

#ifdef __cplusplus
extern "C" {
#endif

#define HC_OK 0
#define HC_ERR_HIP 1
#define HC_ERR_ARG 2
#define HC_ERR_STATE 3

#define HC_Q 19

typedef struct hc_lattice hc_lattice;
typedef struct hc_celltype hc_celltype;
typedef struct hc_cells hc_cells;

const char *hc_last_error(void);
int hc_init(int device);
int hc_device_count(int *count);
int hc_set_stream(void *hip_stream);
int hc_synchronize(void);
int hc_fork(void);
int hc_route(int side);
int hc_join(void);
int hc_side_stream(void **hip_stream);
int hc_set_overlap(int on);
int hc_profile_enable(int on);
int hc_profile_read(const char *kernel, double *total_ms, long *launches);
int hc_profile_reset(void);
const char *hc_build_tag(void);
int hc_measure_copy_bandwidth(size_t bytes, int repeats, double *gbytes_per_s);
int hc_set_reproducible_spread(int on);
int hc_debug_ibm_per_vertex(int on);
int hc_debug_force_plane_padding(int on);

#define HC_TRANSPORT_NONE 0
#define HC_TRANSPORT_RCCL 1
#define HC_TRANSPORT_TCP 2
#define HC_TRANSPORT_AUTO 3
int hc_comm_init_env(void);
int hc_comm_init(int rank, int world, int local_rank, const char *master_addr, int port, int transport, int init_device);
int hc_comm_finalize(void);
int hc_comm_info(int *rank, int *world, int *transport);
int hc_comm_barrier(void);
int hc_comm_allreduce(double *v, int n, int op);
int hc_comm_bcast(void *buf, size_t bytes, int root);
int hc_comm_allgather(const void *mine, size_t bytes, void *all);
int hc_comm_exchange_host(int periodic, const void *send_lo, size_t n_lo, const void *send_hi, size_t n_hi,
                          void *recv_lo, size_t m_lo, void *recv_hi, size_t m_hi);
int hc_slab_stats(hc_lattice *L, double out[8], int reset);

int hcl_create(hc_lattice **out, int nx, int ny, int nz, const int periodic[3], double omega,
               int x0, int nx_global, int n_slabs);
int hcl_destroy(hc_lattice *L);
int hcl_set_mask(hc_lattice *L, const uint8_t *mask_with_halo);
int hcl_init_equilibrium(hc_lattice *L, double rho, const double u[3]);
int hcl_set_body_force(hc_lattice *L, const double F[3]);
#define HC_MAX_FORCE_REGIONS 4
int hcl_set_body_force_regions(hc_lattice *L, int n, const int *boxes, const double *forces);
int hcl_set_wall_velocity(hc_lattice *L, int wall_class, const double u[3]);
int hcl_collide_stream(hc_lattice *L, int nsteps);
int hcl_set_lees_edwards(hc_lattice *L, double v_top, double v_bottom);
int hcl_set_lees_edwards_displacement(hc_lattice *L, double D, double d_per_iteration);
int hcl_lees_edwards_apply(hc_lattice *L);
int hcl_lees_edwards_state(const hc_lattice *L, double out[4]);
#define HC_OB_VELOCITY 0
#define HC_OB_PRESSURE 1
int hcl_open_boundary_add(hc_lattice *L, int kind, int orientation, const int *nodes, int n, int *first_slot);
int hcl_open_boundary_add_box(hc_lattice *L, int kind, int orientation, const int box[6], int *first_slot, int *n_nodes);
int hcl_open_boundary_add_axis(hc_lattice *L, int kind, int axis, int orientation, const int *nodes, int n, int *first_slot);
int hcl_open_boundary_add_box_axis(hc_lattice *L, int kind, int axis, int orientation, const int box[6], int *first_slot, int *n_nodes);
int hcl_open_boundary_clear(hc_lattice *L);
int hcl_open_boundary_slots(const hc_lattice *L, const int *nodes, int n, int *slots);
int hcl_open_boundary_axes(const hc_lattice *L, const int *nodes, int n, int *axes);
int hcl_open_boundary_set_velocity(hc_lattice *L, int first_slot, int n, const double *u, int on_device);
int hcl_open_boundary_set_density(hc_lattice *L, int first_slot, int n, const double *rho, int on_device);
int hcl_open_boundary_values(hc_lattice *L, int first_slot, int n, double *out);
int hcl_plane_velocity(hc_lattice *L, int x, const int *yz, int n, double *out, int on_device);
int hcl_plane_velocity_axis(hc_lattice *L, int axis, int plane, const int *idx, int n, double *out, int on_device);
typedef struct hc_preinlet hc_preinlet;
int hcl_preinlet_create(hc_preinlet **out, hc_lattice *pre, hc_lattice *domain, int axis, int pre_plane,
                        const int *pre_idx, int n, int domain_first_slot);
int hcl_preinlet_apply(hc_preinlet *P);
int hcl_preinlet_iterate(hc_preinlet *P, int n);
int hcl_preinlet_destroy(hc_preinlet *P);
int hcl_slab_refresh_halos(hc_lattice *L, int width);
int hcl_collide_stream_part(hc_lattice *L, int part);
int hcl_zero_force_halos(hc_lattice *L);
int hcl_step_end(hc_lattice *L);
int hcl_download_populations(hc_lattice *L, double *f_aos);
int hcl_upload_populations(hc_lattice *L, const double *f_aos);
int hcl_download_rho_u(hc_lattice *L, double *rho, double *u);
int hcl_download_pi_neq(hc_lattice *L, double *pi);
int hcl_fluid_stats(hc_lattice *L, int what, double out[3], long *n_nodes);
int hcl_download_ibm_force(hc_lattice *L, double *F);
int hcl_zero_ibm_force(hc_lattice *L);
size_t hcl_halo_doubles(const hc_lattice *L, int width);
int hcl_halo_pack(hc_lattice *L, int side, int width, double *dev_buf);
int hcl_halo_unpack(hc_lattice *L, int side, int width, const double *dev_buf);
int hcl_halo_pack_next(hc_lattice *L, int side, int width, double *dev_buf);
int hcl_halo_pack_both(hc_lattice *L, double *dev_lo, double *dev_hi, int next);
int hcl_halo_unpack_both(hc_lattice *L, const double *dev_lo, const double *dev_hi);
int hcl_face_velocity_pack(hc_lattice *L, int side, double *dev_buf);
int hcl_face_velocity_pack_both(hc_lattice *L, double *dev_lo, double *dev_hi);
int hcl_download_face_velocity(hc_lattice *L, int side, double *host_u );
int hcl_dims(const hc_lattice *L, int dims[3]);
int hcl_node_counts(const hc_lattice *L, long counts[3]);
double hcl_mlups_bytes_per_node(const hc_lattice *L);
#define HC_MAX_VISC_CLASSES 7
int hcl_interior_enable(hc_lattice *L, int n_classes, const double *omega );
int hcl_interior_info(const hc_lattice *L, int *n_classes , double *omega );
int hcl_interior_upload_classes(hc_lattice *L, const uint8_t *classes);
int hcl_interior_download_classes(hc_lattice *L, uint8_t *classes);

typedef struct hc_scalar hc_scalar;
#define HC_MAX_SCALAR_SOURCES 8
int hcl_scalar_create(hc_lattice *L, double omega, hc_scalar **out);
int hcl_scalar_destroy(hc_scalar *S);
int hcl_scalar_init_equilibrium(hc_scalar *S, const int box[6] , double C);
int hcl_scalar_set_source_box(hc_scalar *S, const int box[6], double C);
int hcl_scalar_clear_sources(hc_scalar *S);
int hcl_scalar_step(hc_scalar *S);
int hcl_scalar_download(hc_scalar *S, double *C_out);
int hcl_scalar_download_populations(hc_scalar *S, double *g_aos);
int hcl_scalar_upload_populations(hc_scalar *S, const double *g_aos);
int hcl_scalar_download_velocity(hc_scalar *S, double *u_out);
int hcl_scalar_stats(hc_scalar *S, double out3[3]);
int hcp_sample_scalar(hc_cells *C, hc_scalar *S, double *out_per_vertex);

#define HC_MODEL_RBC_HO 0
#define HC_MODEL_PLT_SIMPLE 1
#define HC_MODEL_WBC_HO 2
#define HC_MODEL_RBC_MALARIA 3
#define HC_SHAPE_WBC_SPHERE 0
#define HC_SHAPE_RBC_FROM_SPHERE 1
#define HC_SHAPE_MESH_FROM_STL 2
#define HC_SHAPE_ELLIPSOID_FROM_SPHERE 6

typedef struct hc_params {
  double dx, dt, nu_p, rho_p, kBT_p;
  double tau, nu_lbm, dm, df, f_limit, kBT_lbm;
} hc_params;
int hc_params_base(hc_params *P, double dx, double dt, double nu_p, double rho_p, double kBT_p);

typedef struct hc_material {
  double kLink, kArea, kVolume, kBend, eta_m;
  double radius;
  int min_triangles;
  double aspect_ratio;
  const long *inner_edges;
  int n_inner;
} hc_material;

int hcp_celltype_create(hc_celltype **out, int model, int shape, const hc_params *P, const hc_material *M);

typedef struct hc_wbc_material {
  double kInnerRigid;
  double kCytoskeleton;
  double coreRadius;
  double radius;
} hc_wbc_material;
int hcp_celltype_create_wbc(hc_celltype **out, int shape, const hc_params *P, const hc_material *M, const hc_wbc_material *W);
int hcp_celltype_wbc_constants(const hc_celltype *T, double out[4]);

typedef struct hc_celltype_spec {
  int model;
  int shape;
  hc_material material;
  const hc_wbc_material *wbc;
  double kInnerLink;
  const char *stl_path;
} hc_celltype_spec;
int hcp_celltype_create_ex(hc_celltype **out, const hc_params *P, const hc_celltype_spec *S);
int hcp_celltype_malaria_constants(const hc_celltype *T, double out[1]);
int hcp_celltype_destroy(hc_celltype *T);
int hcp_celltype_sizes(const hc_celltype *T, int out[4]);
int hcp_celltype_tables(const hc_celltype *T, double *vertices , long *triangles ,
                        long *edges , double *edge_length_eq, double *edge_angle_eq,
                        double *triangle_area_eq, long *vertex_vertexes , double *patch_dist_eq,
                        double scalars[9] );

int hcp_celltype_tables2(const hc_celltype *T, long *edge_bending_triangles , long *edge_bending_outer_points ,
                         long *inner_edges , double *inner_edge_length_eq , int *vertex_n_vertexes );

int hcp_create(hc_cells **out, hc_lattice *L, const hc_params *P);
int hcp_destroy(hc_cells *C);
int hcp_add_type(hc_cells *C, hc_celltype *T, int material_timescale , int *type_index);
int hcp_add_cell(hc_cells *C, int type, long cell_id, const double centre_lu[3], const double angles[3],
                 double min_dist_um, int *placed);
int hcp_add_cell_unchecked(hc_cells *C, int type, long cell_id, const double centre_lu[3], const double angles[3]);
int hcp_slab_sync_placement(hc_cells *C, long *global_cells_per_type );
int hcp_set_envelope(hc_cells *C, double particle_envelope_lu, double *share_in_use);
int hcp_envelope(const hc_cells *C, double *share_in_use, long *late_copies);
int hcp_counts(hc_cells *C, long *n_vertices, long *n_cells, long *n_deleted);
int hcp_type_range(hc_cells *C, int type, long *first_vertex, long *n_cells);
#define HC_DELETE_PARTICLE 0
#define HC_DELETE_CELL 1
int hcp_set_deletion_mode(hc_cells *C, int mode);
int hcp_delete_incomplete_cells(hc_cells *C, long *n_cells_removed);
int hcp_deletion_counts(hc_cells *C, long *cells_removed, long *particles_removed, long *incomplete_cells, long *missing_particles);
int hcp_download_alive(hc_cells *C, unsigned char *alive);
int hcp_download(hc_cells *C, int what, double *out);
int hcp_upload(hc_cells *C, int what, const double *in);
int hcp_download_cell_ids(hc_cells *C, long *ids);
int hcp_download_records(hc_cells *C, void *records, long n_records);
int hcp_upload_records(hc_cells *C, const void *records, long n_records);
int hcp_add_vertex_force(hc_cells *C, const long *vertex_index, int n, const double *f );
int hcp_vertex_stats(hc_cells *C, int what, double out[3], long *n);
int hcp_set_repulsion(hc_cells *C, double r_const, double r_cutoff_lu, int timescale);
int hcp_repulsion(hc_cells *C);
int hcp_download_repulsion(hc_cells *C, double *out );
int hcp_set_boundary_repulsion(hc_cells *C, double br_const, double br_cutoff_lu, int timescale);
int hcp_boundary_repulsion(hc_cells *C);
int hcp_spread(hc_cells *C, int force_limit);
int hcp_interpolate(hc_cells *C);
int hcp_interpolate_cells(hc_cells *C, int type, const int *slots, int n);
int hcp_advance(hc_cells *C, int check_deletions);
int hcp_mechanics(hc_cells *C, long iter, int forced);
int hcp_mechanics_components(hc_cells *C, int type, double *comp);
int hcp_type_set_interior_viscosity(hc_cells *C, int type, double tau_int);
int hcp_set_interior_timescales(hc_cells *C, int membrane_every, int entire_grid_every);
int hcp_interior_find(hc_cells *C);
int hcp_interior_membrane(hc_cells *C);
int hcp_interior_normals(hc_cells *C, int type, double *out);
int hc_debug_interior_block(int threads);
int hcl_binding_populate(hc_lattice *L, const int box[6]);
int hcl_binding_clear(hc_lattice *L);
int hcl_binding_download(hc_lattice *L, uint8_t *out);
int hcl_binding_upload(hc_lattice *L, const uint8_t *in);
int hcl_download_mask(hc_lattice *L, uint8_t *out);
int hcl_download_tresca(hc_lattice *L, double *out);
int hcl_upload_solidified_mask(hc_lattice *L, const uint8_t *in);
int hcp_type_set_solidify(hc_cells *C, int type, double distance_threshold_lu, double shear_threshold);
int hcp_set_solidify_timescale(hc_cells *C, int every);
int hcp_solidify_prepare(hc_cells *C);
int hcp_solidify_flag(hc_cells *C);
int hcp_solidify_flags_download(hc_cells *C, unsigned char *out);
int hcp_solidify_flags_upload(hc_cells *C, const unsigned char *in);
int hcp_solidify_counts(hc_cells *C, long out[3]);
int hc_debug_solidify_block(int threads);
int hc_iterate(hc_lattice *L, hc_cells *C, long *iter, int n, int particle_timescale, int force_limit,
               int deletion_check_every);
int hcp_cell_extents(hc_cells *C, int type, double *ext );
int hcp_cell_extents_begin(hc_cells *C, int type);
int hcp_cell_extents_end(hc_cells *C, int type, double *ext);
size_t hcp_record_doubles(const hc_cells *C, int type);
int hcp_pack_cells(hc_cells *C, int type, const int *slots, int n, double x_shift, double *dev_buf);
int hcp_unpack_cells(hc_cells *C, int type, const int *slots, const long *cell_ids, const int *is_new, int n,
                     const double *dev_buf);
int hcp_remove_cells(hc_cells *C, int type, const int *slots, int n);
int hcp_owned_vertices(hc_cells *C, long *n_owned);

typedef struct hc_preinlet_cells hc_preinlet_cells;
int hcp_preinlet_create(hc_preinlet_cells **out, hc_cells *pre, hc_cells *domain, int axis, int orientation ,
                        double window_lo, double window_hi, const double shift[3], long id_stride);
int hcp_preinlet_create_slab(hc_preinlet_cells **out, hc_cells *pre , hc_cells *domain, int axis, int orientation,
                             double window_lo, double window_hi, const double shift[3], long id_stride);
int hcp_preinlet_set_sink(hc_preinlet_cells *X, int on, double plane);
int hcp_preinlet_apply(hc_preinlet_cells *X, long *n_injected, long *n_removed);
int hcp_preinlet_counts(const hc_preinlet_cells *X, long out[4]);
int hcp_preinlet_destroy(hc_preinlet_cells *X);
int hc_preinlet_iterate(hc_preinlet *F, hc_preinlet_cells *X, long *iter, int n, int particle_timescale, int force_limit,
                        int deletion_check_every, int cells_every);

int hcp_cell_info(hc_cells *C, int type, double *volume, double *area, double *bbox, double *centroid);

#ifdef __cplusplus
}
#endif
#endif
```

Measured before the change: 15760.

## Cache per-cell IBM tile geometry and node lists across spread and interpolate

Adds a per-cell device record holding the tile bounding box, the compacted lattice-node list and per-vertex stencil keys (base index, admissible-corner mask, fluid mask). The spread and interpolate kernels check the record against the current vertex stencils and mask generation, and reuse the cached node list when they agree, skipping the mask-tile load and node compaction. The record is rebuilt when anything differs. The change also marks the dirty flag once per node instead of once per component, and returns early from mechanics when no cell type is due. The cost is extra global memory for the records, a validation pass and atomic counters for reuse and rebuild events.

```diff
diff --git a/hemocell_amd/capi.py b/hemocell_amd/capi.py
--- a/hemocell_amd/capi.py
+++ b/hemocell_amd/capi.py
@@ -72,6 +72,8 @@
     "hc_measure_copy_bandwidth": (C.c_int, [C.c_size_t, C.c_int, c_double_p]),
     "hcl_node_counts": (C.c_int, [VP, c_long_p]),
     "hc_debug_ibm_per_vertex": (C.c_int, [C.c_int]),
+    "hc_debug_ibm_geometry": (C.c_int, [C.c_int]),
+    "hc_debug_ibm_geometry_counts": (C.c_int, [c_long_p, c_long_p]),
     "hc_set_reproducible_spread": (C.c_int, [C.c_int]),
     "hc_debug_force_plane_padding": (C.c_int, [C.c_int]),
     "hcl_create": (C.c_int, [C.POINTER(VP), C.c_int, C.c_int, C.c_int, c_int_p, C.c_double, C.c_int, C.c_int, C.c_int]),
diff --git a/hemocell_amd/csrc/cells.h b/hemocell_amd/csrc/cells.h
--- a/hemocell_amd/csrc/cells.h
+++ b/hemocell_amd/csrc/cells.h
@@ -37,6 +37,8 @@
   bool ntag_pending = false, maybe_tagged = false;
   int del_mode = HC_DELETE_PARTICLE;
   DevBuf<int> d_vert_cell;
+  DevBuf<unsigned int> d_geom;
+  long geom0[8] = {0};
   DevBuf<double> rep[3];
   int rep_enabled = 0, rep_timescale = 1; double rep_const = 0, rep_cutoff = 0;
   int brep_enabled = 0, brep_timescale = 1; double brep_const = 0, brep_cutoff = 0; DevBuf<uint8_t> d_bflag;
@@ -93,6 +95,18 @@
   v.halo_u[0] = L->halo_u_valid ? L->halo_u[0] : nullptr; v.halo_u[1] = L->halo_u_valid ? L->halo_u[1] : nullptr; v.ny_nz = (int)L->plane;
   return v;
 }
+
+constexpr int IBM_NODE_CAP = 1536;
+constexpr int GEOM_HDR = 8;
+inline int geom_list_cap(int nv) { return std::min(IBM_NODE_CAP, 8 * nv); }
+inline long geom_stride(int nv) { return GEOM_HDR + (geom_list_cap(nv) + 1) / 2 + nv; }
+struct GeomView {
+  unsigned int *rec;
+  long stride;
+  int vert0;
+  unsigned int gen;
+};
+GeomView geom_view(hc_cells *C, int t);
 
 __device__ __forceinline__ long pmod(long a, long n) { long r = a % n; return r < 0 ? r + n : r; }
 
diff --git a/hemocell_amd/csrc/cells.hip b/hemocell_amd/csrc/cells.hip
--- a/hemocell_amd/csrc/cells.hip
+++ b/hemocell_amd/csrc/cells.hip
@@ -60,7 +60,7 @@
 
 static void drop_regions(hc_cells *C) {
   for (int d = 0; d < 3; d++) { C->pos[d].reset(); C->vel[d].reset(); C->frc[d].reset(); C->rep[d].reset(); }
-  C->d_tag.reset(); C->d_vdead.reset(); C->d_vert_cell.reset(); C->d_sflag.reset();
+  C->d_tag.reset(); C->d_vdead.reset(); C->d_vert_cell.reset(); C->d_sflag.reset(); C->d_geom.reset();
   C->cap = 0; C->tag_cap = 0;
   for (int t = 0; t < 8; t++) C->capc[t] = 0;
 }
@@ -110,6 +110,9 @@
       cap += C->capc[t] * C->types[t]->host.nv; capcells += C->capc[t];
     }
     C->cap = cap > 0 ? cap : 1;
+    long geom = 0;
+    for (int t = 0; t < C->ntypes; t++) { C->geom0[t] = geom; geom += C->capc[t] * geom_stride(C->types[t]->host.nv); }
+    if ((rc = C->d_geom.reserve((size_t)(geom > 0 ? geom : 1))) != HC_OK) return rc;
     for (int d = 0; d < 3; d++)
       if ((rc = C->pos[d].reserve((size_t)C->cap)) != HC_OK || (rc = C->vel[d].reserve((size_t)C->cap)) != HC_OK || (rc = C->frc[d].reserve((size_t)C->cap)) != HC_OK) return rc;
     if ((rc = C->d_vert_cell.reserve((size_t)C->cap)) != HC_OK) return rc;
@@ -133,6 +136,7 @@
   }
   HC_HIP(hipMemsetAsync(C->d_tag, 0, C->tag_cap * sizeof(int), hc::stream()));
   HC_HIP(hipMemsetAsync(C->d_vdead, 0, (size_t)C->cap, hc::stream()));
+  HC_HIP(hipMemsetAsync(C->d_geom, 0, C->d_geom.cap * sizeof(unsigned int), hc::stream()));
   if (C->d_sflag) HC_HIP(hipMemsetAsync(C->d_sflag, 0, (size_t)C->cap, hc::stream()));
   HC_HIP(hipStreamSynchronize(hc::stream()));
   for (int t = 0; t < C->ntypes; t++) {
diff --git a/hemocell_amd/csrc/common.h b/hemocell_amd/csrc/common.h
--- a/hemocell_amd/csrc/common.h
+++ b/hemocell_amd/csrc/common.h
@@ -219,7 +219,10 @@
   uint8_t fepoch[3];
   hc::DevBuf<uint8_t> wallbrick; int nbx, nby, nbz;
   hc::DevBuf<uint8_t> mask;
-  std::vector<uint8_t> hmask;
+  struct HostMask : std::vector<uint8_t> {
+    unsigned int gen = 0;
+    void assign(size_t n, uint8_t v) { ++gen; std::vector<uint8_t>::assign(n, v); }
+  } hmask;
   double body[3];
   hc::BodyRegions regions;
   double wall_u[4][3];
diff --git a/hemocell_amd/csrc/ibm.hip b/hemocell_amd/csrc/ibm.hip
--- a/hemocell_amd/csrc/ibm.hip
+++ b/hemocell_amd/csrc/ibm.hip
@@ -164,6 +164,8 @@
 
 constexpr int TILE_CAP = 5832;
 constexpr int NODE_CAP = 1536;
+static_assert(NODE_CAP == IBM_NODE_CAP, "the geometry record (cells.h) holds a node list of NODE_CAP entries");
+static_assert(TILE_CAP < (1 << 13), "a tile index must fit the 13 bits the geometry record gives it");
 
 struct Tile { int o[3]; int e[3]; int vol; int ow[3]; float r1, r2; };
 
@@ -231,6 +233,7 @@
 #pragma unroll
   for (int a = 0; a < 3; a++) {
     int l = s_red[a], h = s_red[3 + a];
+#pragma nounroll
     for (int w = 1; w < nw; w++) { l = min(l, s_red[w * 6 + a]); h = max(h, s_red[w * 6 + 3 + a]); }
     t.o[a] = l; t.e[a] = h >= l ? h - l + 1 : 0;
   }
@@ -260,8 +263,17 @@
   return v.mask[(long)(lx + HALO) * v.plane + ly * v.nz + lz];
 }
 
-__device__ __forceinline__ void tile_stencil(const Tile &t, const unsigned char *mt, double px, double py, double pz, const int b[3], VStencil &o) {
+__device__ __forceinline__ unsigned corner_fluid(const Tile &t, const unsigned char *mt, const int b[3]) {
+  if (!mt) return 0xffu;
   const int sy = t.e[2], sx = t.e[1] * t.e[2];
+  const int base = ((b[0] - t.o[0]) * t.e[1] + (b[1] - t.o[1])) * t.e[2] + (b[2] - t.o[2]);
+  unsigned fluid = 0;
+#pragma unroll
+  for (int k = 0; k < 8; k++) if (mt[base + (k >> 2) * sx + ((k >> 1) & 1) * sy + (k & 1)] == 0) fluid |= 1u << k;
+  return fluid;
+}
+
+__device__ __forceinline__ void tile_stencil(const Tile &t, unsigned fluid, double px, double py, double pz, const int b[3], VStencil &o) {
   o.base = ((b[0] - t.o[0]) * t.e[1] + (b[1] - t.o[1])) * t.e[2] + (b[2] - t.o[2]);
   o.adm = 0;
   double total = 0.0;
@@ -273,7 +285,7 @@
       for (int k = 0; k < 2; k++) {
         const int idx = i * 4 + j * 2 + k;
         const double weight = phi2(px - (double)(b[0] + i)) * phi2(py - (double)(b[1] + j)) * phi2(pz - (double)(b[2] + k));
-        const bool adm = (weight != 0.0) && (!mt || mt[o.base + i * sx + j * sy + k] == 0);
+        const bool adm = (weight != 0.0) && ((fluid >> idx) & 1u);
         if (adm) { total += weight; o.adm |= 1u << idx; }
         o.w[idx] = adm ? weight : 0.0;
       }
@@ -308,20 +320,17 @@
   return *s_near == 0;
 }
 
-__device__ __forceinline__ bool cell_prologue(const LatView &v, int nv, long base, const double *px, const double *py, const double *pz,
-                                              const unsigned char *dead, int *s_red, int *s_near, unsigned char *mt, Tile &t, VStencil vs[NVPT] PH_PARAM) {
+struct VLoad { double p[NVPT][3]; int b[NVPT][3]; bool live[NVPT]; };
+
+__device__ __forceinline__ bool cell_prologue(const LatView &v, int nv, const VLoad &L, int *s_red, int *s_near, unsigned char *mt, Tile &t,
+                                              VStencil vs[NVPT], unsigned int *keys PH_PARAM) {
   const int tid = threadIdx.x, nth = blockDim.x;
-  double p[NVPT][3]; int b[NVPT][3]; bool live[NVPT];
   int lo[3] = {0x7fffffff, 0x7fffffff, 0x7fffffff}, hi[3] = {-0x7fffffff, -0x7fffffff, -0x7fffffff};
 #pragma unroll
   for (int j = 0; j < NVPT; j++) {
-    const int i = tid + j * nth;
-    live[j] = i < nv && !(dead && dead[base + i]);
-    if (live[j]) {
-      p[j][0] = px[base + i]; p[j][1] = py[base + i]; p[j][2] = pz[base + i];
-      stencil_base(v, p[j][0], p[j][1], p[j][2], b[j]);
-#pragma unroll
-      for (int a = 0; a < 3; a++) { lo[a] = min(lo[a], b[j][a]); hi[a] = max(hi[a], b[j][a] + 1); }
+    if (L.live[j]) {
+#pragma unroll
+      for (int a = 0; a < 3; a++) { lo[a] = min(lo[a], L.b[j][a]); hi[a] = max(hi[a], L.b[j][a] + 1); }
     }
   }
   block_bbox(lo, hi, s_red, t);
@@ -338,7 +347,13 @@
 #pragma unroll
   for (int j = 0; j < NVPT; j++) {
     vs[j].adm = 0; vs[j].base = 0;
-    if (live[j]) tile_stencil(t, clear ? nullptr : mt, p[j][0], p[j][1], p[j][2], b[j], vs[j]);
+    unsigned key = 0;
+    if (L.live[j]) {
+      const unsigned fluid = corner_fluid(t, clear ? nullptr : mt, L.b[j]);
+      tile_stencil(t, fluid, L.p[j][0], L.p[j][1], L.p[j][2], L.b[j], vs[j]);
+      key = (unsigned)vs[j].base | (vs[j].adm << 13) | (fluid << 21) | (1u << 29);
+    }
+    if (keys && tid + j * nth < nv) keys[tid + j * nth] = key;
   }
   STAMP(4);
   return true;
@@ -372,6 +387,97 @@
   return *s_count;
 }
 
+__device__ unsigned long long g_geom_counts[2];
+
+__device__ __forceinline__ int cell_geometry_any(const LatView &v, const GeomView &g, int cell, int nv, long base, const double *px, const double *py,
+                                                 const double *pz, const unsigned char *dead, int *s_red, int *s_near, int *s_count, unsigned char *mt,
+                                                 unsigned short *slot, unsigned short *list, Tile &t, VStencil vs[NVPT] PH_PARAM) {
+  const int tid = threadIdx.x, nth = blockDim.x;
+  unsigned int *R = g.rec ? g.rec + (long)cell * g.stride : nullptr;
+  unsigned h[GEOM_HDR], key[NVPT];
+#pragma unroll
+  for (int k = 0; k < GEOM_HDR; k++) h[k] = R ? __builtin_amdgcn_readfirstlane(R[k]) : 0u;
+  VLoad L;
+#pragma unroll
+  for (int j = 0; j < NVPT; j++) {
+    const int i = tid + j * nth;
+    L.live[j] = i < nv && !(dead && dead[base + i]);
+    key[j] = (R && i < nv) ? R[g.vert0 + i] : 0u;
+    if (L.live[j]) {
+      L.p[j][0] = px[base + i]; L.p[j][1] = py[base + i]; L.p[j][2] = pz[base + i];
+      stencil_base(v, L.p[j][0], L.p[j][1], L.p[j][2], L.b[j]);
+    }
+  }
+  if (R && h[0] == g.gen && (h[1] >> 31) && nv <= NVPT * nth) {
+#pragma unroll
+    for (int a = 0; a < 3; a++) { t.o[a] = (int)h[2 + a]; t.e[a] = (int)h[5 + a]; }
+    t.vol = t.e[0] * t.e[1] * t.e[2];
+    bool agree = tile_finish(v, t);
+#pragma unroll
+    for (int j = 0; j < NVPT; j++) {
+      const int i = tid + j * nth;
+      vs[j].adm = 0; vs[j].base = 0;
+      if (i >= nv) continue;
+      const bool was_live = (key[j] >> 29) & 1u;
+      if (!L.live[j]) { agree = agree && !was_live; continue; }
+      bool inside = true;
+#pragma unroll
+      for (int a = 0; a < 3; a++) inside = inside && L.b[j][a] >= t.o[a] && L.b[j][a] + 1 < t.o[a] + t.e[a];
+      tile_stencil(t, (key[j] >> 21) & 0xffu, L.p[j][0], L.p[j][1], L.p[j][2], L.b[j], vs[j]);
+      agree = agree && was_live && inside && vs[j].base == (int)(key[j] & 0x1fffu) && vs[j].adm == ((key[j] >> 13) & 0xffu);
+    }
+    const bool wave_agrees = __ballot(!agree) == 0ull;
+    if ((tid & 63) == 0) s_red[tid >> 6] = wave_agrees ? 1 : 0;
+    __syncthreads();
+    bool all = true;
+    for (int w = 0; w < ((nth + 63) >> 6); w++) all = all && s_red[w] != 0;
+    if (all) {
+      const int n = min((int)(h[1] & 0x7fffffffu), min(NODE_CAP, 2 * (g.vert0 - GEOM_HDR)));
+      const unsigned short *gl = reinterpret_cast<const unsigned short *>(R + GEOM_HDR);
+      for (int r = tid; r < n; r += nth) {
+        const unsigned short li = gl[r];
+        list[r] = li;
+        if (li < TILE_CAP) slot[li] = (unsigned short)r;
+      }
+      if (tid == 0) atomicAdd(&g_geom_counts[0], 1ull);
+      __syncthreads();
+      return n;
+    }
+    __syncthreads();
+  }
+  if (tid == 0) atomicAdd(&g_geom_counts[1], 1ull);
+  int n = -1;
+  if (cell_prologue(v, nv, L, s_red, s_near, mt, t, vs, R ? R + g.vert0 : nullptr PH_ARG)) {
+    n = compact_nodes(t, vs, slot, list, s_count);
+    if (n > NODE_CAP) n = -1;
+  }
+  if (R) {
+    if (tid == 0) {
+      R[0] = g.gen; R[1] = n >= 0 ? ((unsigned)n | 0x80000000u) : 0u;
+#pragma unroll
+      for (int a = 0; a < 3; a++) { R[2 + a] = (unsigned)t.o[a]; R[5 + a] = (unsigned)t.e[a]; }
+    }
+    if (n >= 0) {
+      unsigned short *gl = reinterpret_cast<unsigned short *>(R + GEOM_HDR);
+      for (int r = tid; r < n; r += nth) gl[r] = list[r];
+    }
+  }
+  return n;
+}
+
+__device__ __forceinline__ int cell_geometry(const LatView &v, const GeomView &g, int cell, int nv, long base, const double *px, const double *py,
+                                             const double *pz, const unsigned char *dead, int *s_red, int *s_near, int *s_count, unsigned char *mt,
+                                             unsigned short *slot, unsigned short *list, Tile &t, VStencil vs[NVPT] PH_PARAM) {
+  const int n = cell_geometry_any(v, g, cell, nv, base, px, py, pz, dead, s_red, s_near, s_count, mt, slot, list, t, vs PH_ARG);
+#pragma unroll
+  for (int a = 0; a < 3; a++) {
+    t.o[a] = __builtin_amdgcn_readfirstlane(t.o[a]); t.e[a] = __builtin_amdgcn_readfirstlane(t.e[a]); t.ow[a] = __builtin_amdgcn_readfirstlane(t.ow[a]);
+  }
+  t.vol = __builtin_amdgcn_readfirstlane(t.vol);
+  t.r1 = __int_as_float(__builtin_amdgcn_readfirstlane(__float_as_int(t.r1))); t.r2 = __int_as_float(__builtin_amdgcn_readfirstlane(__float_as_int(t.r2)));
+  return __builtin_amdgcn_readfirstlane(n);
+}
+
 __device__ void spread_direct(const LatView &v, int nv, long base, const double *px, const double *py, const double *pz, const double *fx,
                               const double *fy, const double *fz, const double *rx, const double *ry, const double *rz, double *F,
                               const unsigned char *dead) {
@@ -394,7 +500,7 @@
 
 __global__ __launch_bounds__(256) void ibm_spread_cell_kernel(LatView v, int nv, const double *px, const double *py, const double *pz,
                                                               double *fx, double *fy, double *fz, const double *rx, const double *ry, const double *rz,
-                                                              double *F, int limit_on, double f_limit, int xcd_ranges, const int *tag, const unsigned char *vdead) {
+                                                              double *F, int limit_on, double f_limit, int xcd_ranges, const int *tag, const unsigned char *vdead, GeomView geom) {
   __shared__ unsigned short slot[TILE_CAP];
   __shared__ __attribute__((aligned(16))) unsigned char raw[TILE_CAP > 2 * NODE_CAP ? TILE_CAP : 2 * NODE_CAP];
   unsigned char *mt = raw; unsigned short *list = reinterpret_cast<unsigned short *>(raw);
@@ -419,7 +525,8 @@
     }
   }
   Tile t; VStencil vs[NVPT];
-  bool tiled = cell_prologue(v, nv, base, px, py, pz, dead, s_red, &s_near, mt, t, vs PH_ARG);
+  const int n = cell_geometry(v, geom, cell, nv, base, px, py, pz, dead, s_red, &s_near, &s_count, mt, slot, list, t, vs PH_ARG);
+  STAMP(5);
   if (limit_on) {
     if (in_regs) {
 #pragma unroll
@@ -439,9 +546,7 @@
       }
     }
   }
-  const int n = tiled ? compact_nodes(t, vs, slot, list, &s_count) : 0;
-  STAMP(5);
-  if (!tiled || n > NODE_CAP) { spread_direct(v, nv, base, px, py, pz, fx, fy, fz, rx, ry, rz, F, dead); return; }
+  if (n < 0) { spread_direct(v, nv, base, px, py, pz, fx, fy, fz, rx, ry, rz, F, dead); return; }
   const int sy = t.e[2], sx = t.e[1] * t.e[2];
   for (int k = tid; k < 3 * n; k += nth) acc[k] = 0.0;
   __syncthreads();
@@ -464,8 +569,10 @@
     const double val = acc[k];
     if (val != 0.0) {
       const int q = k / 3;
-      int lx, ly, lz; const long node = tile_node(v, t, list[q], lx, ly, lz); v.dirty[node >> 4] = v.epoch;
-      unsafeAtomicAdd(&F[3 * node + (k - 3 * q)], val);
+      const int c = k - 3 * q;
+      int lx, ly, lz; const long node = tile_node(v, t, list[q], lx, ly, lz);
+      if (c == 0 || (acc[k - c] == 0.0 && (c == 1 || acc[k - 1] == 0.0))) v.dirty[node >> 4] = v.epoch;
+      unsafeAtomicAdd(&F[3 * node + c], val);
     }
   }
   STAMP(7);
@@ -474,7 +581,7 @@
 template <bool OPEN = false>
 __global__ __launch_bounds__(256) void ibm_interpolate_cell_kernel(LatView v, Pops<OPEN> pv, int nv, const double *px, const double *py,
                                                                    const double *pz, double *vx, double *vy, double *vz, const int *slots, int xcd_ranges,
-                                                                   const int *tag, const unsigned char *vdead) {
+                                                                   const int *tag, const unsigned char *vdead, GeomView geom) {
   __shared__ unsigned short slot[TILE_CAP];
   __shared__ __attribute__((aligned(16))) unsigned char raw[TILE_CAP > 2 * NODE_CAP ? TILE_CAP : 2 * NODE_CAP];
   unsigned char *mt = raw; unsigned short *list = reinterpret_cast<unsigned short *>(raw);
@@ -488,14 +595,10 @@
   const long base = (long)cell * nv;
   Tile t; VStencil vs[NVPT];
   PH_INIT
-  bool tiled = cell_prologue(v, nv, base, px, py, pz, dead, s_red, &s_near, mt, t, vs PH_ARG);
+  const int n = cell_geometry(v, geom, cell, nv, base, px, py, pz, dead, s_red, &s_near, &s_count, mt, slot, list, t, vs PH_ARG);
+  STAMP(12);
   const int sy = t.e[2], sx = t.e[1] * t.e[2];
-  if (tiled) {
-    if (compact_nodes(t, vs, slot, list, &s_count) > NODE_CAP) tiled = false;
-    STAMP(12);
-  }
-  if (tiled) {
-    const int n = s_count;
+  if (n >= 0) {
     for (int k = tid; k < n; k += nth) {
       int lx, ly, lz;
       const long node = tile_node(v, t, list[k], lx, ly, lz);
@@ -556,6 +659,20 @@
 
 static int g_ibm_per_vertex = 0;
 extern "C" int hc_debug_ibm_per_vertex(int on) { g_ibm_per_vertex = on; return HC_OK; }
+static int g_ibm_geometry = 1;
+extern "C" int hc_debug_ibm_geometry(int on) { g_ibm_geometry = on != 0; return HC_OK; }
+extern "C" int hc_debug_ibm_geometry_counts(long *reused, long *rebuilt) {
+  unsigned long long h[2];
+  HC_HIP(hipDeviceSynchronize());
+  HC_HIP(hipMemcpyFromSymbol(h, HIP_SYMBOL(g_geom_counts), sizeof(h)));
+  if (reused) *reused = (long)h[0];
+  if (rebuilt) *rebuilt = (long)h[1];
+  return HC_OK;
+}
+GeomView hcc::geom_view(hc_cells *C, int t) {
+  const int nv = C->types[t]->host.nv;
+  return GeomView{g_ibm_geometry ? C->d_geom + C->geom0[t] : nullptr, geom_stride(nv), GEOM_HDR + (geom_list_cap(nv) + 1) / 2, C->L->hmask.gen};
+}
 static int g_reproducible = -1;
 static bool reproducible() {
   if (g_reproducible < 0) { const char *e = std::getenv("HEMOCELL_REPRODUCIBLE_SPREAD"); g_reproducible = (e && *e && *e != '0') ? 1 : 0; }
@@ -642,7 +759,7 @@
                          a.r[0], a.r[1], a.r[2], C->L->force[C->L->fcur], force_limit, C->P.f_limit, a.vert_cell, a.tag_all, a.dead);
     else
       hipLaunchKernelGGL(ibm_spread_cell_kernel, dim3((unsigned)C->ncells[t]), dim3(nv > 128 ? 256 : 128), 0, hc::stream(), v, nv, a.p[0], a.p[1], a.p[2],
-                         a.f[0], a.f[1], a.f[2], a.r[0], a.r[1], a.r[2], C->L->force[C->L->fcur], force_limit, C->P.f_limit, 1, a.tag, a.dead);
+                         a.f[0], a.f[1], a.f[2], a.r[0], a.r[1], a.r[2], C->L->force[C->L->fcur], force_limit, C->P.f_limit, 1, a.tag, a.dead, geom_view(C, t));
     HC_HIP(hipGetLastError());
   }
   return HC_OK;
@@ -666,7 +783,7 @@
                      a.vert_cell, a.tag_all, a.dead);
     else
       HC_LAUNCH_POPS(ibm_interpolate_cell_kernel, dim3((unsigned)C->ncells[t]), dim3(nv > 128 ? 256 : 128), v, pv, nv, a.p[0], a.p[1], a.p[2], a.v[0], a.v[1], a.v[2],
-                     (const int *)nullptr, 1, a.tag, a.dead);
+                     (const int *)nullptr, 1, a.tag, a.dead, geom_view(C, t));
     HC_HIP(hipGetLastError());
   }
   return HC_OK;
@@ -722,7 +839,7 @@
   const TypeArrays a = vert_arrays(C, type);
   const int nv = C->types[type]->host.nv;
   HC_LAUNCH_POPS(ibm_interpolate_cell_kernel, dim3((unsigned)n), dim3(nv > 128 ? 256 : 128), v, pv, nv, a.p[0], a.p[1], a.p[2], a.v[0], a.v[1], a.v[2],
-                 (const int *)d_slots, 0, a.tag, a.dead);
+                 (const int *)d_slots, 0, a.tag, a.dead, geom_view(C, type));
   HC_HIP(hipGetLastError());
   return HC_OK;
 }
diff --git a/hemocell_amd/csrc/mechanics.hip b/hemocell_amd/csrc/mechanics.hip
--- a/hemocell_amd/csrc/mechanics.hip
+++ b/hemocell_amd/csrc/mechanics.hip
@@ -388,6 +388,9 @@
 int hcp_mechanics(hc_cells *C, long iter, int forced) {
   HC_REQUIRE(C, "hcp_mechanics: null pointer");
   int rc = sync_to_device(C); if (rc != HC_OK) return rc;
+  bool due = false;
+  for (int t = 0; t < C->ntypes; t++) due = due || iter % C->timescale[t] == 0 || forced;
+  if (!due) return HC_OK;
   hc::ProfScope prof(hc::PK_MECH);
   for (int t = 0; t < C->ntypes; t++) {
     if (!(iter % C->timescale[t] == 0 || forced)) continue;
diff --git a/hemocell_amd/csrc/solidify.hip b/hemocell_amd/csrc/solidify.hip
--- a/hemocell_amd/csrc/solidify.hip
+++ b/hemocell_amd/csrc/solidify.hip
@@ -224,6 +224,7 @@
     HC_HIP(hipGetLastError());
   }
   C->maybe_tagged = true;
+  L->hmask.gen++;
   return HC_OK;
 }
 
@@ -342,6 +343,7 @@
   HC_HIP(hipMemcpyAsync(d, pad.data(), L->npad, hipMemcpyHostToDevice, hc::stream()));
   hipLaunchKernelGGL(add_walls_kernel, dim3((unsigned)((L->npad + 255) / 256)), dim3(256), 0, hc::stream(), make_view(L), (long)L->npad, (const uint8_t *)d.p, L->mask.p, L->wallbrick.p);
   HC_HIP(hipGetLastError());
+  L->hmask.gen++;
   HC_HIP(hipMemcpyAsync(L->hmask.data(), L->mask, L->npad, hipMemcpyDeviceToHost, hc::stream()));
   HC_HIP(hipStreamSynchronize(hc::stream()));
   return HC_OK;
diff --git a/hemocell_amd/host.py b/hemocell_amd/host.py
--- a/hemocell_amd/host.py
+++ b/hemocell_amd/host.py
@@ -65,6 +65,16 @@
 def ensure_init():
     if not _initialised:
         init(0)
+
+
+def set_ibm_geometry_records(on=True):
+    check(capi.lib().hc_debug_ibm_geometry(int(bool(on))))
+
+
+def ibm_geometry_counts():
+    r, b = C.c_long(), C.c_long()
+    check(capi.lib().hc_debug_ibm_geometry_counts(C.byref(r), C.byref(b)))
+    return r.value, b.value
 
 
 def base_parameters(dx=5e-7, dt=1e-7, nuP=1.1e-6, rhoP=1025.0, kBT=4.100531391e-21):
diff --git a/include/hemocell_amd.h b/include/hemocell_amd.h
--- a/include/hemocell_amd.h
+++ b/include/hemocell_amd.h
@@ -36,6 +36,8 @@
 int hc_measure_copy_bandwidth(size_t bytes, int repeats, double *gbytes_per_s);
 int hc_set_reproducible_spread(int on);
 int hc_debug_ibm_per_vertex(int on);
+int hc_debug_ibm_geometry(int on);
+int hc_debug_ibm_geometry_counts(long *reused, long *rebuilt);
 int hc_debug_force_plane_padding(int on);
 
 #define HC_TRANSPORT_NONE 0
```

Result: no change. 15900, median of 6 (+0.9%).
